# Artessay/RAGraph

Hardware: AMD Instinct MI355X
Metric: retrieved-queries/sec (RAGraph_node forward: GCN encode + cosine/top-k retrieval + 3-hop propagate + decode) (higher is better)
Workload: dtype f32 (exact results; candidates pre-filtered on bf16 / int8 MFMA with proven bounds)

## Files before the change

### include/ragraph_hip.h

```cpp
#ifndef RAGRAPH_HIP_H
#define RAGRAPH_HIP_H

#include <stddef.h>
#include <stdint.h>

#ifdef __cplusplus
extern "C" {
#endif

#define RAGRAPH_ABI_VERSION 1

#define RAGRAPH_OK 0
#define RAGRAPH_EINVAL (-1)
#define RAGRAPH_EUNSUPPORTED (-2)
#define RAGRAPH_EWORKSPACE (-3)
#define RAGRAPH_EDEVICE (-4)

#define RAGRAPH_ACT_NONE 0
#define RAGRAPH_ACT_RELU 1
#define RAGRAPH_ACT_PRELU 2
#define RAGRAPH_ACT_LEAKY 3
#define RAGRAPH_ACT_ELU 4

int ragraph_abi_version(void);
const char* ragraph_last_error(void);
int ragraph_device_check(void);

int ragraph_normalize_rows_f32(const float* X, int64_t n, int D, float* out, void* stream);

#define RAGRAPH_TOPK_MAX 64
size_t ragraph_topk_cosine_workspace_bytes(int64_t B, int64_t N, int D, int k);
int ragraph_topk_cosine_f32(const float* Q, int64_t B, const float* Kn, int64_t N, int D, int k, int64_t idx_base,
                            float* out_scores, int64_t* out_idx, void* ws, size_t ws_bytes, void* stream);

int ragraph_pack_keys_f32(const float* Kn, int64_t N, int D, float* Kp, void* stream);
int ragraph_topk_cosine_bank_f32(const float* Q, int64_t B, const float* Kn, const float* Kp, int64_t N, int D, int k,
                                 int64_t idx_base, float* out_scores, int64_t* out_idx, void* ws, size_t ws_bytes,
                                 void* stream);

size_t ragraph_topk_cosine_mix_workspace_bytes(int64_t B, int64_t N, int D, int A, int k);
int ragraph_topk_cosine_mix_f32(const float* Q, int64_t B, const float* Kn, int64_t N, int D, const float* Pq,
                                const float* Pn, int A, float w_struct, float w_sem, int k, int64_t idx_base,
                                float* out_scores, int64_t* out_idx, void* ws, size_t ws_bytes, void* stream);

int64_t ragraph_keys_bf16_rows(int64_t N);
int ragraph_keys_to_bf16(const float* Kn, int64_t N, int D, uint16_t* Kb, void* stream);
int ragraph_topk_cosine_filtered_cap(int k);
size_t ragraph_topk_cosine_filtered_workspace_bytes(int64_t B, int64_t N, int D, int k);
size_t ragraph_topk_cosine_filtered_stats_offset(size_t ws_bytes);
int ragraph_topk_cosine_filtered_plan(int64_t B, int64_t N, int D, int k, int64_t plan[7]);
int ragraph_topk_cosine_filtered_i8_levels(int64_t B, int64_t N, int D, int k);
int ragraph_topk_cosine_filtered_max_i8_levels(int n);
float ragraph_topk_cosine_filtered_set_prior(float theta_prior);
int ragraph_topk_cosine_filtered_f32(const float* Q, int64_t B, const float* Kn, const float* Kp, const uint16_t* Kb,
                                     int64_t N, int D, int k, int64_t idx_base, float* out_scores, int64_t* out_idx,
                                     int* overflow, int64_t* overflow_idx, void* ws, size_t ws_bytes, void* stream);

typedef void (*ragraph_exchange_fn)(void* ctx, int phase);
int ragraph_verify_merged_prior_f32(const float* merged_scores, int64_t R, int k, float prior, int speculative,
                                    const int* stats_words, const int* overflow, float* out5, void* stream);
int ragraph_topk_cosine_filtered_sharded_speculates(int64_t B, int64_t plan_N, int D, int k, int n_shards);
size_t ragraph_topk_cosine_filtered_sharded_workspace_bytes(int64_t B, int64_t plan_N, int D, int k, int n_shards);
int ragraph_topk_cosine_filtered_sharded_f32(const float* Q, int64_t B, const float* Kn, const float* Kp, const uint16_t* Kb,
                                             int64_t N, int D, int k, int64_t idx_base, float* out_scores, int64_t* out_idx,
                                             int* overflow, int64_t* overflow_idx, void* ws, size_t ws_bytes, void* stream,
                                             int64_t plan_N, float* theta, ragraph_exchange_fn exchange, void* ctx,
                                             int n_shards);

int ragraph_topk_cosine_small_ok(int64_t B, int64_t N, int D, int k);
size_t ragraph_topk_cosine_small_state_bytes(void);
int64_t ragraph_topk_cosine_small_prefix_keys(int64_t B, int64_t N, int D, int* i8);
size_t ragraph_topk_cosine_small_workspace_bytes(int64_t B, int D, int k);
int ragraph_topk_cosine_small_f32(const float* Q, int64_t B, const float* Kn, const uint16_t* Kb, int64_t N, int D, int k,
                                  int64_t idx_base, float* out_scores, int64_t* out_idx, int* overflow, int* state, void* ws,
                                  size_t ws_bytes, void* stream);

int ragraph_topk_cosine_fused_ok(int64_t B, int64_t N, int D, int k);
size_t ragraph_topk_cosine_fused_workspace_bytes(int64_t B, int64_t N, int D, int k);
int ragraph_topk_cosine_fused_f32(const float* Q, int64_t B, const float* Kn, const uint16_t* Kb, int64_t N, int D, int k,
                                  int64_t idx_base, float* out_scores, int64_t* out_idx, int* tickets, void* ws,
                                  size_t ws_bytes, void* stream);

int ragraph_theta_sharpen_f32(const float* gathered, int G, int64_t B, int m, int k, float* theta, void* stream);

typedef struct ragraph_filter_profile ragraph_filter_profile;
ragraph_filter_profile* ragraph_filter_profile_create(void);
void ragraph_filter_profile_destroy(ragraph_filter_profile* p);
ragraph_filter_profile* ragraph_filter_profile_attach(ragraph_filter_profile* p);
float ragraph_filter_profile_last_ms(ragraph_filter_profile* p);
int ragraph_filter_profile_levels(ragraph_filter_profile* p, float* ms_host, int* i8_host, int64_t* keys_host);

int ragraph_topk_merge_f32(const float* scores, const int64_t* idx, int G, int64_t B, int k, float* out_scores,
                           int64_t* out_idx, void* stream);

size_t ragraph_dedup_rows_workspace_bytes(int64_t N);
int ragraph_dedup_rows_f32(const float* Kn, int64_t N, int D, int64_t* stats, int64_t* uniq_row, int32_t* group_ptr,
                           int32_t* members, void* ws, size_t ws_bytes, void* stream);
int ragraph_topk_expand_groups_f32(const float* scores_u, const int64_t* idx_u, int ku, int64_t idx_base_u,
                                   const int32_t* group_ptr, const int32_t* members, int64_t U, int64_t B, int k,
                                   int64_t idx_base, float* out_scores, int64_t* out_idx, void* stream);

int ragraph_gather_rows_f32(const float* V, int64_t N, int D, const int64_t* idx, int64_t M, int64_t idx_base,
                            float* out, void* stream);

int ragraph_gather_reduce_f32(const float* V, int D, const float* L, int C, int64_t N, const int64_t* idx, int64_t B,
                              int k, int64_t idx_base, float v_scale, float* sum_V, float* mean_L, void* stream);

int ragraph_gather_reduce_mix_f32(const float* V, int D, const float* L, int C, int64_t N, const int64_t* idx, int64_t B,
                                  int k, int64_t idx_base, float v_scale, const float* A, float wa, float wb, float* out,
                                  float* mean_L, void* stream);

int ragraph_linear_f32(const float* X, int64_t M, int K, const float* W, int64_t N, const float* bias, int act,
                       float alpha, float* Y, void* stream);

size_t ragraph_linear_tn_workspace_bytes(int64_t n, int M, int N);
int ragraph_linear_tn_f32(const float* A, const float* B, int64_t n, int M, int N, float* C, void* ws, size_t ws_bytes,
                          void* stream);

int ragraph_spmm_csr_f32(const int64_t* rowptr, const int32_t* col, const float* val, int64_t n, const float* X, int D,
                         const float* bias, int act, float alpha, float beta, const float* Y_in, float* Y,
                         void* stream);
size_t ragraph_sparse_workspace_bytes(int64_t nnz, int D);
int ragraph_spmm_csr_ws_f32(const int64_t* rowptr, const int32_t* col, const float* val, int64_t n, const float* X, int D,
                            const float* bias, int act, float alpha, float beta, const float* Y_in, float* Y, int64_t nnz,
                            void* ws, size_t ws_bytes, void* stream);
size_t ragraph_spmm_csr_rows_workspace_bytes(int64_t nnz, int64_t R, int D);
int ragraph_spmm_csr_rows_f32(const int64_t* rowptr, const int32_t* col, const float* val, int64_t n, const float* X, int D,
                              const int64_t* rows, int64_t R, float* Y, int64_t nnz, void* ws, size_t ws_bytes,
                              void* stream);
size_t ragraph_csr_rows_offsets_workspace_bytes(int64_t R);
int ragraph_csr_rows_offsets_i64(const int64_t* rowptr, int64_t n, const int64_t* rows, int64_t R, int64_t* off, void* ws,
                                 size_t ws_bytes, void* stream);
int ragraph_csr_rows_edges_f32(const int64_t* rowptr, const int32_t* col, const float* val, const int64_t* rows, int64_t R,
                               const int64_t* off, int64_t E, int64_t* out_col, int64_t* out_r, float* out_val,
                               void* stream);
int ragraph_spmm_csr_prelu_dev_f32(const int64_t* rowptr, const int32_t* col, const float* val, int64_t n, const float* X,
                                   int D, const float* bias, const float* alpha, float* Y, float* Z, int64_t nnz, void* ws,
                                   size_t ws_bytes, void* stream);
int ragraph_act_grad_prelu_dev_f32(const float* z, const float* gy, int64_t n, const float* alpha, float* gz,
                                   float* alpha_terms, void* stream);

size_t ragraph_radix_sort_workspace_bytes(int64_t n, int val_bytes);
int ragraph_radix_sort_u64(const uint64_t* keys_in, uint64_t* keys_out, const void* vals_in, void* vals_out, int val_bytes,
                           int64_t n, int bits, void* ws, size_t ws_bytes, void* stream);
size_t ragraph_scan_workspace_bytes(int64_t n);
int ragraph_scan_sum_i32(const int* in, int* out, int64_t n, int inclusive, void* ws, size_t ws_bytes, void* stream);

size_t ragraph_coo_to_csr_workspace_bytes(int64_t E, int64_t n);
int ragraph_coo_to_csr_i64(const int64_t* row, const int64_t* col, int64_t E, int64_t n, int sort_cols, int64_t* rowptr,
                           int64_t* perm, int32_t* out_col, void* ws, size_t ws_bytes, void* stream);
int ragraph_csr_row_ids_i64(const int64_t* rowptr, int64_t n, int64_t nnz, int64_t* rows, void* stream);

size_t ragraph_mask_positions_workspace_bytes(int64_t E);
int ragraph_mask_positions_i64(const unsigned char* mask, int64_t E, int64_t* pos, int64_t* count, void* ws, size_t ws_bytes,
                               void* stream);

int ragraph_spmm_csr_panels_f32(const int64_t* rowptr, const int32_t* col, const float* val, int64_t n, const float* X,
                                int64_t x_rows, int x_panels, int D, int act, float alpha, float* Y, int y_panels, void* stream);

int ragraph_spmm_linear_f32(const int64_t* rowptr, const int32_t* col, const float* val, int64_t M, const float* X, int K,
                            const float* W, int64_t N, const float* bias, int act, float alpha, float* Y, void* stream);

int ragraph_spmm_csr_tiled_f32(const int* wp, const int* col3, const float* val3, const unsigned short* row3, int RG, int C,
                               int64_t n, const float* X, int64_t x_rows, int x_panels, int D, int act, float alpha, float* Y,
                               int y_panels, void* stream);

int ragraph_csr_row_normalize_f32(const int64_t* rowptr, const float* val, int64_t n, float* val_out, void* stream);

int ragraph_segment_softmax_f32(const int64_t* rowptr, const float* x, int64_t n, float* out, void* stream);
int ragraph_segment_softmax_ws_f32(const int64_t* rowptr, const float* x, int64_t n, int64_t nnz, float* out, void* ws,
                                   size_t ws_bytes, void* stream);

int ragraph_axpby_f32(const float* a, float wa, const float* b, float wb, int64_t n, float* out, void* stream);

int ragraph_fuse_decode_f32(const float* query, const float* rag, int64_t n, int D, float wq, float wr, const float* W1,
                            const float* b1, int H, float slope, const float* W2, const float* b2, int C,
                            const float* rag_label, float lambda, float* out, void* stream);

int ragraph_softmax_mix_f32(const float* logits, const float* rag_label, int64_t B, int C, float lambda, int log_mode,
                            float* out, void* stream);

int ragraph_segment_reduce_f32(const float* X, int D, const int64_t* seg_ptr, int64_t G, const float* w, int mean_mode,
                               float* out, void* stream);

int ragraph_proto_cosine_f32(const float* emb, int64_t G, int D, const float* proto, int C, int mode, float* out,
                             void* stream);

int ragraph_sigmoid_gate_f32(const float* x, const float* z, int64_t n, float* out, void* stream);

int ragraph_time_rescale_f32(const int64_t* t, int64_t n, float t_min, float t_max, float* out, void* stream);

int ragraph_topk_rows_f32(const float* S, int64_t B, int64_t N, int64_t ld, int k, float* out_scores,
                          int64_t* out_idx, void* stream);

int ragraph_topk_select_rows_f32(const float* S, int64_t B, int64_t N, int64_t ld, int64_t k, float* out_kth,
                                 int64_t* out_idx, void* stream);
size_t ragraph_topk_select_rows_workspace_bytes(int64_t B, int64_t N);
int ragraph_topk_select_rows_ws_f32(const float* S, int64_t B, int64_t N, int64_t ld, int64_t k, float* out_kth,
                                    int64_t* out_idx, void* ws, size_t ws_bytes, void* stream);

#define RAGRAPH_TOPK_ORDERED_MAX 4096
size_t ragraph_topk_rows_large_workspace_bytes(int64_t B, int64_t N, int64_t k);
int ragraph_topk_rows_large_f32(const float* S, int64_t B, int64_t N, int64_t ld, int64_t k, float* out_scores,
                                int64_t* out_idx, void* ws, size_t ws_bytes, void* stream);

int ragraph_scatter_fill_f32(float* S, int64_t B, int64_t N, int64_t ld, const int64_t* rowptr, const int64_t* col,
// ... 104 lines not shown
```

### ragraph_amd/_native.py

```python
from __future__ import annotations

import ctypes
import os
import subprocess

import torch

_HERE = os.path.dirname(os.path.abspath(__file__))
CSRC = os.path.join(_HERE, "csrc")
SO_PATH = os.environ.get("RAGRAPH_HIP_SO", os.path.join(CSRC, "libragraph_hip.so"))

OK, EINVAL, EUNSUPPORTED, EWORKSPACE, EDEVICE = 0, -1, -2, -3, -4
ACT_NONE, ACT_RELU, ACT_PRELU, ACT_LEAKY, ACT_ELU = 0, 1, 2, 3, 4
TOPK_MAX = 64
TOPK_ORDERED_MAX = 4096
POSITION_CODES_LDS_MAX = 40000
POSITION_CODES_LONG_ROW = 512

_vp, _i64, _i32, _f32, _sz = ctypes.c_void_p, ctypes.c_int64, ctypes.c_int, ctypes.c_float, ctypes.c_size_t

SIGNATURES = {
    "ragraph_abi_version": (_i32, []),
    "ragraph_last_error": (ctypes.c_char_p, []),
    "ragraph_device_check": (_i32, []),
    "ragraph_normalize_rows_f32": (_i32, [_vp, _i64, _i32, _vp, _vp]),
    "ragraph_topk_cosine_workspace_bytes": (_sz, [_i64, _i64, _i32, _i32]),
    "ragraph_topk_cosine_f32": (_i32, [_vp, _i64, _vp, _i64, _i32, _i32, _i64, _vp, _vp, _vp, _sz, _vp]),
    "ragraph_pack_keys_f32": (_i32, [_vp, _i64, _i32, _vp, _vp]),
    "ragraph_keys_bf16_rows": (_i64, [_i64]),
    "ragraph_keys_to_bf16": (_i32, [_vp, _i64, _i32, _vp, _vp]),
    "ragraph_filter_profile_create": (_vp, []),
    "ragraph_filter_profile_destroy": (None, [_vp]),
    "ragraph_filter_profile_attach": (_vp, [_vp]),
    "ragraph_filter_profile_last_ms": (ctypes.c_float, [_vp]),
    "ragraph_topk_cosine_filtered_set_prior": (ctypes.c_float, [_f32]),
    "ragraph_filter_profile_levels": (_i32, [_vp, _vp, _vp, _vp]),
    "ragraph_topk_cosine_filtered_cap": (_i32, [_i32]),
    "ragraph_topk_cosine_filtered_workspace_bytes": (_sz, [_i64, _i64, _i32, _i32]),
    "ragraph_topk_cosine_filtered_stats_offset": (_sz, [_sz]),
    "ragraph_topk_cosine_filtered_sharded_workspace_bytes": (_sz, [_i64, _i64, _i32, _i32, _i32]),
    "ragraph_topk_cosine_filtered_plan": (_i32, [_i64, _i64, _i32, _i32, _vp]),
    "ragraph_topk_cosine_filtered_i8_levels": (_i32, [_i64, _i64, _i32, _i32]),
    "ragraph_topk_cosine_filtered_sharded_speculates": (_i32, [_i64, _i64, _i32, _i32, _i32]),
    "ragraph_verify_merged_prior_f32": (_i32, [_vp, _i64, _i32, _f32, _i32, _vp, _vp, _vp, _vp]),
    "ragraph_topk_cosine_filtered_max_i8_levels": (_i32, [_i32]),
    "ragraph_topk_cosine_filtered_f32": (_i32, [_vp, _i64, _vp, _vp, _vp, _i64, _i32, _i32, _i64, _vp, _vp, _vp, _vp, _vp,
                                                _sz, _vp]),
    "ragraph_topk_cosine_filtered_sharded_f32": (_i32, [_vp, _i64, _vp, _vp, _vp, _i64, _i32, _i32, _i64, _vp, _vp, _vp, _vp,
                                                        _vp, _sz, _vp, _i64, _vp, _vp, _vp, _i32]),
    "ragraph_topk_cosine_small_ok": (_i32, [_i64, _i64, _i32, _i32]),
    "ragraph_topk_cosine_small_state_bytes": (_sz, []),
    "ragraph_topk_cosine_small_prefix_keys": (_i64, [_i64, _i64, _i32, _vp]),
    "ragraph_topk_cosine_small_workspace_bytes": (_sz, [_i64, _i32, _i32]),
    "ragraph_topk_cosine_small_f32": (_i32, [_vp, _i64, _vp, _vp, _i64, _i32, _i32, _i64, _vp, _vp, _vp, _vp, _vp, _sz, _vp]),
    "ragraph_topk_cosine_fused_ok": (_i32, [_i64, _i64, _i32, _i32]),
    "ragraph_topk_cosine_fused_workspace_bytes": (_sz, [_i64, _i64, _i32, _i32]),
    "ragraph_topk_cosine_fused_f32": (_i32, [_vp, _i64, _vp, _vp, _i64, _i32, _i32, _i64, _vp, _vp, _vp, _vp, _sz, _vp]),
    "ragraph_theta_sharpen_f32": (_i32, [_vp, _i32, _i64, _i32, _i32, _vp, _vp]),
    "ragraph_topk_cosine_bank_f32": (_i32, [_vp, _i64, _vp, _vp, _i64, _i32, _i32, _i64, _vp, _vp, _vp, _sz, _vp]),
    "ragraph_topk_cosine_mix_workspace_bytes": (_sz, [_i64, _i64, _i32, _i32, _i32]),
    "ragraph_topk_cosine_mix_f32": (_i32, [_vp, _i64, _vp, _i64, _i32, _vp, _vp, _i32, _f32, _f32, _i32, _i64, _vp, _vp, _vp,
                                          _sz, _vp]),
    "ragraph_topk_merge_f32": (_i32, [_vp, _vp, _i32, _i64, _i32, _vp, _vp, _vp]),
    "ragraph_dedup_rows_workspace_bytes": (_sz, [_i64]),
    "ragraph_dedup_rows_f32": (_i32, [_vp, _i64, _i32, _vp, _vp, _vp, _vp, _vp, _sz, _vp]),
    "ragraph_topk_expand_groups_f32": (_i32, [_vp, _vp, _i32, _i64, _vp, _vp, _i64, _i64, _i32, _i64, _vp, _vp, _vp]),
    "ragraph_gather_rows_f32": (_i32, [_vp, _i64, _i32, _vp, _i64, _i64, _vp, _vp]),
    "ragraph_gather_reduce_f32": (_i32, [_vp, _i32, _vp, _i32, _i64, _vp, _i64, _i32, _i64, _f32, _vp, _vp, _vp]),
    "ragraph_gather_reduce_mix_f32": (_i32, [_vp, _i32, _vp, _i32, _i64, _vp, _i64, _i32, _i64, _f32, _vp, _f32, _f32, _vp, _vp, _vp]),
    "ragraph_linear_f32": (_i32, [_vp, _i64, _i32, _vp, _i64, _vp, _i32, _f32, _vp, _vp]),
    "ragraph_linear_tn_workspace_bytes": (_sz, [_i64, _i32, _i32]),
    "ragraph_linear_tn_f32": (_i32, [_vp, _vp, _i64, _i32, _i32, _vp, _vp, _sz, _vp]),
    "ragraph_spmm_csr_f32": (_i32, [_vp, _vp, _vp, _i64, _vp, _i32, _vp, _i32, _f32, _f32, _vp, _vp, _vp]),
    "ragraph_radix_sort_workspace_bytes": (_sz, [_i64, _i32]),
    "ragraph_radix_sort_u64": (_i32, [_vp, _vp, _vp, _vp, _i32, _i64, _i32, _vp, _sz, _vp]),
    "ragraph_scan_workspace_bytes": (_sz, [_i64]),
    "ragraph_scan_sum_i32": (_i32, [_vp, _vp, _i64, _i32, _vp, _sz, _vp]),
    "ragraph_coo_to_csr_workspace_bytes": (_sz, [_i64, _i64]),
    "ragraph_coo_to_csr_i64": (_i32, [_vp, _vp, _i64, _i64, _i32, _vp, _vp, _vp, _vp, _sz, _vp]),
    "ragraph_csr_row_ids_i64": (_i32, [_vp, _i64, _i64, _vp, _vp]),
    "ragraph_mask_positions_workspace_bytes": (_sz, [_i64]),
    "ragraph_mask_positions_i64": (_i32, [_vp, _i64, _vp, _vp, _vp, _sz, _vp]),
    "ragraph_spmm_csr_panels_f32": (_i32, [_vp, _vp, _vp, _i64, _vp, _i64, _i32, _i32, _i32, _f32, _vp, _i32, _vp]),
    "ragraph_spmm_linear_f32": (_i32, [_vp, _vp, _vp, _i64, _vp, _i32, _vp, _i64, _vp, _i32, _f32, _vp, _vp]),
    "ragraph_spmm_csr_tiled_f32": (_i32, [_vp, _vp, _vp, _vp, _i32, _i32, _i64, _vp, _i64, _i32, _i32, _i32, _f32, _vp, _i32, _vp]),
    "ragraph_csr_row_normalize_f32": (_i32, [_vp, _vp, _i64, _vp, _vp]),
    "ragraph_segment_softmax_f32": (_i32, [_vp, _vp, _i64, _vp, _vp]),
    "ragraph_segment_softmax_ws_f32": (_i32, [_vp, _vp, _i64, _i64, _vp, _vp, _sz, _vp]),
    "ragraph_sparse_workspace_bytes": (_sz, [_i64, _i32]),
    "ragraph_spmm_csr_ws_f32": (_i32, [_vp, _vp, _vp, _i64, _vp, _i32, _vp, _i32, _f32, _f32, _vp, _vp, _i64, _vp, _sz,
                                       _vp]),
    "ragraph_spmm_csr_rows_workspace_bytes": (_sz, [_i64, _i64, _i32]),
    "ragraph_spmm_csr_rows_f32": (_i32, [_vp, _vp, _vp, _i64, _vp, _i32, _vp, _i64, _vp, _i64, _vp, _sz, _vp]),
    "ragraph_csr_rows_offsets_workspace_bytes": (_sz, [_i64]),
    "ragraph_csr_rows_offsets_i64": (_i32, [_vp, _i64, _vp, _i64, _vp, _vp, _sz, _vp]),
    "ragraph_csr_rows_edges_f32": (_i32, [_vp, _vp, _vp, _vp, _i64, _vp, _i64, _vp, _vp, _vp, _vp]),
    "ragraph_axpby_f32": (_i32, [_vp, _f32, _vp, _f32, _i64, _vp, _vp]),
    "ragraph_softmax_mix_f32": (_i32, [_vp, _vp, _i64, _i32, _f32, _i32, _vp, _vp]),
    "ragraph_fuse_decode_f32": (_i32, [_vp, _vp, _i64, _i32, _f32, _f32, _vp, _vp, _i32, _f32, _vp, _vp, _i32, _vp, _f32,
                                       _vp, _vp]),
    "ragraph_segment_reduce_f32": (_i32, [_vp, _i32, _vp, _i64, _vp, _i32, _vp, _vp]),
    "ragraph_proto_cosine_f32": (_i32, [_vp, _i64, _i32, _vp, _i32, _i32, _vp, _vp]),
    "ragraph_sigmoid_gate_f32": (_i32, [_vp, _vp, _i64, _vp, _vp]),
    "ragraph_time_rescale_f32": (_i32, [_vp, _i64, _f32, _f32, _vp, _vp]),
    "ragraph_topk_rows_f32": (_i32, [_vp, _i64, _i64, _i64, _i32, _vp, _vp, _vp]),
    "ragraph_topk_select_rows_f32": (_i32, [_vp, _i64, _i64, _i64, _i64, _vp, _vp, _vp]),
    "ragraph_topk_select_rows_workspace_bytes": (_sz, [_i64, _i64]),
    "ragraph_topk_select_rows_ws_f32": (_i32, [_vp, _i64, _i64, _i64, _i64, _vp, _vp, _vp, _sz, _vp]),
    "ragraph_topk_rows_large_workspace_bytes": (_sz, [_i64, _i64, _i64]),
    "ragraph_topk_rows_large_f32": (_i32, [_vp, _i64, _i64, _i64, _i64, _vp, _vp, _vp, _sz, _vp]),
    "ragraph_scatter_fill_f32": (_i32, [_vp, _i64, _i64, _i64, _vp, _vp, _f32, _vp]),
    "ragraph_floyd_warshall_f32": (_i32, [_vp, _i32, _vp, _vp]),
    "ragraph_position_code_f32": (_i32, [_vp, _i32, _vp, _i32, _f32, _vp, _vp]),
    "ragraph_position_codes_csr_f32": (_i32, [_vp, _vp, _vp, _i64, _vp, _i32, _f32, _vp, _vp, _vp]),
    "ragraph_position_codes_csr_global_workspace_bytes": (_sz, [_i64, _i32]),
    "ragraph_position_codes_csr_global_f32": (_i32, [_vp, _vp, _vp, _i64, _vp, _i32, _f32, _vp, _vp, _i32, _i32, _vp, _vp, _sz,
                                                     _vp]),
    "ragraph_act_grad_f32": (_i32, [_vp, _vp, _i64, _i32, _f32, _vp, _vp, _vp]),
    "ragraph_spmm_csr_prelu_dev_f32": (_i32, [_vp, _vp, _vp, _i64, _vp, _i32, _vp, _vp, _vp, _vp, _i64, _vp, _sz, _vp]),
    "ragraph_act_grad_prelu_dev_f32": (_i32, [_vp, _vp, _i64, _vp, _vp, _vp, _vp]),
    "ragraph_sigmoid_gate_grad_f32": (_i32, [_vp, _vp, _vp, _i64, _vp, _vp, _vp]),
    "ragraph_softmax_grad_f32": (_i32, [_vp, _vp, _i64, _i32, _f32, _vp, _vp]),
    "ragraph_mul_cols_f32": (_i32, [_vp, _vp, _i64, _i32, _vp, _vp]),
    "ragraph_mul_cols_act_f32": (_i32, [_vp, _vp, _i64, _i32, _i32, _f32, _vp, _vp]),
    "ragraph_mul_f32": (_i32, [_vp, _vp, _i64, _vp, _vp]),
    "ragraph_proto_cosine_grad_f32": (_i32, [_vp, _i64, _i32, _vp, _i32, _i32, _vp, _vp, _vp, _vp]),
    "ragraph_proto_cosine_grad_proto_workspace_bytes": (_sz, [_i64, _i32, _i32]),
    "ragraph_proto_cosine_grad_proto_f32": (_i32, [_vp, _i64, _i32, _vp, _i32, _i32, _vp, _vp, _vp, _vp, _sz, _vp]),
    "ragraph_axpby_dev_f32": (_i32, [_vp, _vp, _vp, _i32, _i32, _i64, _vp, _vp]),
    "ragraph_ingest_workspace_bytes": (_sz, [_i64, _i64]),
    "ragraph_csr_sym_normalized_f32": (_i32, [_vp, _vp, _i64, _i64, _vp, _vp, _vp, _vp, _vp, _sz, _vp]),
    "ragraph_binorm_edges_f32": (_i32, [_vp, _vp, _vp, _i64, _i64, _i64, _vp, _vp, _vp, _vp, _vp, _sz, _vp]),
    "ragraph_pagerank_workspace_bytes": (_sz, [_i64, _i64]),
    "ragraph_pagerank_f32": (_i32, [_vp, _vp, _vp, _vp, _vp, _vp, _i64, _i64, _f32, _f32, _i32, _vp, _vp, _vp, _sz, _vp]),
    "ragraph_sample_prob_f32": (_i32, [_vp, _vp, _vp, _i64, _f32, _f32, _vp, _vp]),
    "ragraph_csr_row_sums_f32": (_i32, [_vp, _vp, _i64, _vp, _vp]),
    "ragraph_position_codes_batch_f32": (_i32, [_vp, _i64, _i32, _vp, _i32, _f32, _vp, _vp, _vp]),
    "ragraph_topk_dot_masked_workspace_bytes": (_sz, [_i64, _i64, _i32, _i32, _i64]),
    "ragraph_topk_dot_masked_f32": (_i32, [_vp, _i64, _vp, _i64, _vp, _i64, _i32, _i32, _vp, _vp, _i64, _f32, _vp, _vp, _vp,
                                          _sz, _vp]),
    "ragraph_rank_metrics_workspace_bytes": (_sz, [_i64, _i32, _i64]),
    "ragraph_rank_metrics_f64": (_i32, [_vp, _i64, _i32, _vp, _vp, _vp, _i32, _i64, _vp, _vp, _sz, _vp]),
    "ragraph_lp_workspace_bytes": (_sz, []),
    "ragraph_lp_sample_i64": (_i32, [_vp, _vp, _i64, _i64, _i32, _vp, _vp, _vp, _sz, _vp]),
    "ragraph_lp_compare_loss_fwd_f32": (_i32, [_vp, _i64, _i32, _vp, _i32, _f32, _vp, _vp, _vp, _vp, _vp, _vp, _vp, _sz, _vp]),
    "ragraph_lp_combine_f32": (_i32, [_vp, _vp, _vp, _vp, _vp, _f32, _i64, _i32, _vp, _vp]),
    "ragraph_edge_hist_check_i64": (_i32, [_vp, _vp, _i64, _i64, _i64, _vp, _sz, _vp]),
    "ragraph_edge_neg_sample_i64": (_i32, [_vp, _vp, _i64, _i64, _vp, _i64, _i32, _i32, _vp, _vp, _vp, _sz, _vp]),
    "ragraph_noise_rows_i64": (_i32, [_vp, _vp, _i64, _i64, _i32, _i64, _vp, _i64, _vp]),
    "ragraph_gather_reduce_noisy_f32": (_i32, [_vp, _i32, _vp, _i32, _i64, _vp, _i64, _i32, _i64, _f32, _vp, _vp, _i64, _i32, _i64,
                                               _vp, _f32, _f32, _vp, _vp, _vp]),
    "ragraph_add_normal_noise_f32": (_i32, [_vp, _i64, _i64, _i32, _f32, _vp, _vp, _i64, _vp, _vp]),
    "ragraph_edge_rewrite_workspace_bytes": (_sz, [_i64]),
    "ragraph_edge_rewrite_csr": (_i32, [_vp, _vp, _vp, _i64, _i64, _vp, _vp, _vp, _vp, _i64, _vp, _sz, _vp]),
    "ragraph_multinomial_segments_workspace_bytes": (_sz, [_i64]),
    "ragraph_multinomial_segments_i64": (_i32, [_vp, _vp, _i64, _vp, _i64, _i32, _vp, _vp, _sz, _vp]),
    "ragraph_csr_induced_blocks_f32": (_i32, [_vp, _vp, _vp, _i64, _i64, _vp, _i64, _i32, _vp, _vp]),
    "ragraph_blocks_to_csr_workspace_bytes": (_sz, [_i64, _i32]),
    "ragraph_blocks_to_csr_f32": (_i32, [_vp, _i64, _i32, _vp, _vp, _vp, _vp, _vp, _sz, _vp]),
    "ragraph_augment_features_f32": (_i32, [_vp, _i64, _i32, _vp, _f32, _f32, _vp, _vp, _vp, _i64, _vp, _vp]),
}


class RagraphNativeError(RuntimeError):
    """The HIP library is missing, has no usable device, or a call returned an error code."""


_lib = None


def build(verbose: bool = False) -> str:
    cmd = ["make", "-C", CSRC, "-j4"]
    if not verbose:
        cmd.append("-s")
    subprocess.check_call(cmd)
    return SO_PATH


def lib() -> ctypes.CDLL:
    global _lib
    if _lib is None:
        if not os.path.exists(SO_PATH):
            raise RagraphNativeError(
                f"{SO_PATH} not found: build it with `python -c 'import __graft_entry__ as g; g.build()'` "
                "(ragraph_amd has no CPU fallback)")
        cdll = ctypes.CDLL(SO_PATH)
        for name, (res, args) in SIGNATURES.items():
            fn = getattr(cdll, name)
# ... 22 lines not shown
```

### ragraph_amd/csrc/filter_common.h

```cpp
#pragma once
#include "common.h"
#include <climits>

namespace ragraph {

typedef __bf16 bf16x8 __attribute__((ext_vector_type(8)));

constexpr float FILTER_EPS_SLACK = 0.000244140625f;

constexpr int FILTER_STAGE_BYTES = 32 * 1024;
constexpr int FILTER_PAD_KEYS = 256;

__host__ __device__ constexpr int64_t filter_block_offset(int64_t subtile, int D, int t, int h) {
  return (subtile * (D / 16) + 2 * t + h) * 1024;
}

__host__ __device__ constexpr int64_t filter_i8_block_offset(int64_t subtile, int D, int t, int h) {
  return (subtile * (D / 32) + 2 * t + h) * 1024;
}
__host__ __device__ constexpr int filter_i8_granule_keys(int D) { return FILTER_STAGE_BYTES / D; }
__host__ __device__ constexpr int64_t filter_pad_keys(int64_t n) { return (n + FILTER_PAD_KEYS - 1) / FILTER_PAD_KEYS * FILTER_PAD_KEYS; }
struct FilterI8View {
  const signed char* K8;
  const unsigned* tail8;
  const float* gmax;
  const unsigned* cls;
  int64_t granules;
};
inline int64_t filter_i8_granules(int64_t N, int D) {
  const int gk = filter_i8_granule_keys(D);
  return (filter_pad_keys(N) + gk - 1) / gk;
}
inline size_t filter_i8_table_bytes(int64_t N, int D) {
  const int64_t g = filter_i8_granules(N, D);
  return (size_t)((g * 4 + 15) / 16 * 16) + (size_t)((g + 31) / 32 * 4) + 16;
}
inline FilterI8View filter_i8_view(const uint16_t* Kb, int64_t N, int D) {
  const int64_t npad = filter_pad_keys(N);
  FilterI8View v;
  v.K8 = reinterpret_cast<const signed char*>(Kb + (npad + 1) * D);
  v.tail8 = reinterpret_cast<const unsigned*>(v.K8 + npad * D);
  v.granules = filter_i8_granules(N, D);
  v.gmax = reinterpret_cast<const float*>(reinterpret_cast<const char*>(v.tail8) + (size_t)D * 2);
  v.cls = reinterpret_cast<const unsigned*>(reinterpret_cast<const char*>(v.gmax) + (v.granules * 4 + 15) / 16 * 16);
  return v;
}

__device__ __forceinline__ int quantize_i8(float x, float inv_scale) {
  return (int)fminf(fmaxf(__builtin_rintf(__fmul_rn(x, inv_scale)), -127.f), 127.f);
}

int filter_thread_i8_cap();
float filter_thread_prior();
int launch_overflow_fixup(int D, const float* Qn, const float* Kn, int64_t N, int k, int64_t idx_base, const int* count,
                          const int* list, float* out_s, int64_t* out_i, int* done, float* part_s, int64_t* part_i, int64_t B,
                          void* stream);

__device__ __forceinline__ int f2ord(float f) {
  const int b = __float_as_int(f);
  return b >= 0 ? b : b ^ 0x7FFFFFFF;
}
__device__ __forceinline__ float ord2f(int o) { return __int_as_float(o >= 0 ? o : o ^ 0x7FFFFFFF); }

struct FilterThr {
  const float* theta;
  const float* prev_scores;
  const int* gmax;
  const float* eq;
  const unsigned* max_kerr2;
  int k, ngroups;
  int ablate;
  const float* eq8;
  const float* qscale;
  const unsigned* tail8;
  const unsigned* cls8;
  const unsigned char* flag;
};

__device__ __forceinline__ float filter_eps(const FilterThr& t, int64_t q) {
  const float ek = sqrtf(__uint_as_float(*t.max_kerr2));
  const float e = t.eq[q];
  return fmaf(fmaf(e, ek, e + ek), 1.0009765625f, FILTER_EPS_SLACK);
}

__device__ __forceinline__ float filter_theta(const FilterThr& t, int64_t q) {
  if (t.theta) return t.theta[q];
  if (t.gmax) {
    int m = t.gmax[q * t.ngroups];
    for (int g = 1; g < t.ngroups; ++g) m = min(m, t.gmax[q * t.ngroups + g]);
    return __fsub_rn(ord2f(m), filter_eps(t, q));
  }
  return t.prev_scores[q * t.k + t.k - 1];
}

__device__ __forceinline__ float filter_threshold(const FilterThr& t, int64_t q) {
  const unsigned char fl = t.flag ? t.flag[q] : 0;
  const float thr = __fsub_rn(filter_theta(t, q), filter_eps(t, q));
  return (t.ablate == 1 || fl) ? __builtin_huge_valf() : thr;
}

__device__ __forceinline__ int filter_threshold_i8_of(float theta, float e, float ek, float sc) {
  const float eps = fmaf(fmaf(e, ek, e + ek), 1.0009765625f, FILTER_EPS_SLACK);
  if (!(sc > 0.f)) return INT_MIN;
  const float x = __fsub_rn(theta, eps) / sc;
  if (!(x > -8.4e6f)) return INT_MIN;
  if (x > 8.4e6f) return INT_MAX;
  return (int)floorf(x) - 2;
}
__device__ __forceinline__ int filter_threshold_i8_at(const FilterThr& t, int64_t q, float theta, int heavy) {
  return filter_threshold_i8_of(theta, t.eq8[q], sqrtf(__uint_as_float(t.tail8[heavy ? 3 : 0])),
                                t.qscale[q] * __uint_as_float(t.tail8[heavy ? 4 : 1]));
}
__device__ __forceinline__ int filter_threshold_i8(const FilterThr& t, int64_t q, int heavy) {
  const unsigned char fl = t.flag ? t.flag[q] : 0;
  const int thr = filter_threshold_i8_at(t, q, filter_theta(t, q), heavy);
  return (t.ablate == 1 || fl) ? INT_MAX : thr;
}
__device__ __forceinline__ int filter_i8_class(const unsigned* cls, int64_t granule) {
  return (int)((cls[granule >> 5] >> (granule & 31)) & 1u);
}

constexpr int FILTER_COUNT_STRIDE = 32;
constexpr int FILTER_TICKET_SLOT = 16;
__host__ __device__ constexpr int filter_count_stride(int64_t B) { return B < 2048 ? FILTER_COUNT_STRIDE : 1; }

struct DirectArgs {
  const uint16_t* Qb;
  const uint16_t* Kb;
  int64_t B, key0, key1;
  FilterThr thr;
  int* count;
  int* cand;
  int cap;
  int nsub;
  int* gmax_out;
  int bound_groups;
  int scored;
  int i8;
};
template <int D>
int launch_filter_direct(const DirectArgs& a, hipStream_t st);

}
```

### ragraph_amd/csrc/filter_ring.h

```cpp

#ifdef RG_RING_STAMPS
__device__ unsigned long long g_ring_t[2][2][8];
__device__ unsigned long long g_ring_span[2][2];
__device__ unsigned long long g_ring_max[2][8];
#define RG_RSTAMP(i_)                                                                                     \
  if (threadIdx.x == 0 && first_seg) {                                                                    \
    const unsigned long long now_ = wall_clock64();                                                       \
    if (blockIdx.x == 0 || blockIdx.x == gridDim.x - 1) g_ring_t[BOUND][blockIdx.x != 0][i_] = now_;      \
    if ((i_) == 0) atomicMin(&g_ring_span[BOUND][0], now_);                                               \
    else atomicMax(&g_ring_max[BOUND][i_], now_ - rs_prev);                                               \
    rs_prev = now_;                                                                                       \
  }
static void ring_stamps_report(bool BOUND, bool I8) {
  (void)hipDeviceSynchronize();
  unsigned long long t[2][2][8];
  (void)hipMemcpyFromSymbol(t, HIP_SYMBOL(g_ring_t), sizeof(t));
  for (int b = 0; b < 2; ++b)
    fprintf(stderr, "[ring stamps, %s%s launch, %s workgroup, 10 ns ticks] operands %lld thresholds %lld ring primed %lld stages %lld "
            "flush %lld (entered %lld after workgroup 0)\n", BOUND ? "bound" : "filter", I8 ? " int8" : "", b ? "last" : "first",
            (long long)(t[BOUND][b][1] - t[BOUND][b][0]), (long long)(t[BOUND][b][2] - t[BOUND][b][1]),
            (long long)(t[BOUND][b][3] - t[BOUND][b][2]), (long long)(t[BOUND][b][4] - t[BOUND][b][3]),
            (long long)(t[BOUND][b][5] - t[BOUND][b][4]), (long long)(t[BOUND][b][0] - t[BOUND][0][0]));
  unsigned long long span[2][2], mx[2][8];
  (void)hipMemcpyFromSymbol(span, HIP_SYMBOL(g_ring_span), sizeof(span));
  (void)hipMemcpyFromSymbol(mx, HIP_SYMBOL(g_ring_max), sizeof(mx));
  fprintf(stderr, "[ring stamps, all workgroups] first entry to last exit %lld; longest first-segment phases: operands %lld thresholds %lld "
          "ring primed %lld stages %lld flush %lld\n", (long long)(span[BOUND][1] - span[BOUND][0]), (long long)mx[BOUND][1],
          (long long)mx[BOUND][2], (long long)mx[BOUND][3], (long long)mx[BOUND][4], (long long)mx[BOUND][5]);
  unsigned long long init_span[2][2] = {{~0ull, 0ull}, {~0ull, 0ull}}, zero[2][8] = {};
  (void)hipMemcpyToSymbol(HIP_SYMBOL(g_ring_span), init_span, sizeof(init_span));
  (void)hipMemcpyToSymbol(HIP_SYMBOL(g_ring_max), zero, sizeof(zero));
}
#else
#define RG_RSTAMP(i_)
static void ring_stamps_report(bool, bool) {}
#endif
#ifdef RG_TOPK_TIMING
__device__ unsigned long long g_filter_timing[8];
#define RG_FT(var_) const unsigned long long var_ = __builtin_amdgcn_s_memtime()
static void ring_timing_report(int prof_slot, int D) {
  (void)hipDeviceSynchronize();
  unsigned long long t[8];
  (void)hipMemcpyFromSymbol(t, HIP_SYMBOL(g_filter_timing), sizeof(t));
  const double n = (double)t[5];
  if (n > 0)
    fprintf(stderr, "[filter timing] slot %d D=%d wave-stages=%.0f ticks/stage: wait_full %.1f compute %.1f signal+vmcnt "
            "%.1f wait_free %.1f dma_issue %.1f total %.1f; flushes in the loop: %.0f, %.1f ticks each = %.1f per stage\n",
            prof_slot, D, n, t[0] / n, t[1] / n, t[2] / n, t[3] / n, t[4] / n, (t[0] + t[1] + t[2] + t[3] + t[4]) / n, (double)t[7],
            t[7] ? (double)t[6] / (double)t[7] : 0.0, t[6] / n);
  unsigned long long zero[8] = {0, 0, 0, 0, 0, 0, 0, 0};
  (void)hipMemcpyToSymbol(HIP_SYMBOL(g_filter_timing), zero, sizeof(zero));
}
#else
#define RG_FT(var_)
static void ring_timing_report(int, int) {}
#endif

#ifndef RG_RING_FOLD
#define RG_RING_FOLD 1
#endif
template <int D, int QW, bool BOUND = false, bool I8 = false, bool SCORED = false, bool PIPE = false>
__global__ void __launch_bounds__(512, 2) topk_filter_kernel(FilterParams p) {
  using C = FilterCfg<I8 ? D / 2 : D>;
  static_assert(!PIPE || (I8 && !BOUND && C::KSTEPS >= QW / 16 + 2), "PIPE: int8 filter levels, one step per query group + 2");
  static_assert(!(I8 && BOUND), "the bound pass runs on the bf16 copy");
  static_assert(I8 || !SCORED, "scored lists carry the int8 levels' integer sums");
  static_assert(QW == 32 || QW == 64 || QW == 96 || QW == 128, "two, four, six or eight query groups of 16 per wave");
  constexpr int QT = C::WAVES * QW;
  constexpr int NG = QW / 16;
  constexpr bool FOLD = RG_RING_FOLD && I8 && !PIPE && !BOUND && D == 64;
  extern __shared__ float4 fsmem4[];
  char* smem = reinterpret_cast<char*>(fsmem4);
  unsigned* full = reinterpret_cast<unsigned*>(smem + C::SLOTS * C::STAGE_BYTES);
  unsigned* freec = full + C::SLOTS;
  const unsigned lds_base = (unsigned)(size_t)(lds_void_f*)smem;

  const int tid = threadIdx.x;
  const int lane = tid & 63;
  const int wave = __builtin_amdgcn_readfirstlane(tid >> 6);
  const int j = lane & 15, g = lane >> 4;

  unsigned voff[C::DMAS];
#pragma unroll
  for (int i = 0; i < C::DMAS; ++i) voff[i] = (unsigned)(i * 1024 + lane * 16);
  auto dma_stage = [&](int64_t stage_abs, int slot) {
    const uint64_t goff = (uint64_t)stage_abs * C::STAGE_BYTES + (uint64_t)(C::DMAS * wave * 1024);
    const char* gbase = reinterpret_cast<const char*>(p.Kb) +
                        (((uint64_t)(unsigned)__builtin_amdgcn_readfirstlane((int)(goff >> 32)) << 32) |
                         (uint64_t)(unsigned)__builtin_amdgcn_readfirstlane((int)(unsigned)goff));
#pragma unroll
    for (int i = 0; i < C::DMAS; ++i) {
      const unsigned dst = lds_base + (unsigned)(slot * C::STAGE_BYTES + (C::DMAS * wave + i) * 1024);
      unsigned keep;
      asm volatile(
          "s_mov_b32 %0, m0\n\ts_mov_b32 m0, %2\n\ts_nop 0\n\tglobal_load_lds_dwordx4 %1, %3\n\ts_mov_b32 m0, %0"
          : "=&s"(keep)
          : "v"(voff[i]), "s"(dst), "s"(gbase)
          : "memory");
    }
  };
  const unsigned apos = lds_base + (unsigned)lane * 16u;

  const int x = p.xcd_map ? (int)(blockIdx.x & 7) : 0;
  const int64_t nq = p.xcd_map ? ((p.qtiles - x + 7) >> 3) : p.qtiles;
  const int64_t nq0 = p.xcd_map ? ((p.qtiles + 7) >> 3) : p.qtiles;
  SegmentWalker walker(nq, p.nstages_total, p.wgs_per_group, p.lb_min, 0, p.depth[nq != nq0],
                       p.xcd_map ? (int)(blockIdx.x >> 3) : (int)blockIdx.x);
  Segment seg;
  [[maybe_unused]] bool first_seg = true;
#ifdef RG_RING_STAMPS
  unsigned long long rs_prev = 0;
#endif
  RG_RSTAMP(0);
  while (walker.next(seg)) {
    const int64_t qtile = p.xcd_map ? x + 8 * seg.tile : seg.tile;
    const int64_t q_lo = qtile * QT + wave * QW + j;
    const int64_t st0 = seg.st0;
    const int nstages = (int)(seg.st1 - seg.st0);

    bf16x8 bq[I8 ? 1 : NG][I8 ? 1 : C::KS32];
    i32x4 bqi[I8 ? NG : 1][I8 ? C::KS32 : 1];
    constexpr int TB = C::KS32 < 4 ? C::KS32 : 4;
    if constexpr (I8) {
      if (p.Qb) {
        const int64_t qg0 = (qtile * QT + wave * QW) >> 4;
        const int64_t ngroups16 = ((p.B + 31) / 32 * 32) >> 4;
#pragma unroll
        for (int gq = 0; gq < NG; ++gq) {
          const bool have = qg0 + gq < ngroups16;
          const i32x4* src = reinterpret_cast<const i32x4*>(p.Qb) + ((qg0 + gq) * C::KS32) * 64 + lane;
#pragma unroll
          for (int t = 0; t < C::KS32; ++t) {
            i32x4 z = {0, 0, 0, 0};
            bqi[gq][t] = have ? src[t * 64] : z;
          }
        }
      } else
#pragma unroll
      for (int gq = 0; gq < NG; ++gq) {
        const int64_t qq = q_lo + 16 * gq;
        const int64_t qr = qq < p.B ? qq : p.B - 1;
        const float sq = p.thr.qscale[qr];
        const float inv_sq = sq > 0.f ? 1.f / sq : 0.f;
        const float* r0 = p.Qn + qr * D + 16 * g;
#pragma unroll
        for (int t = 0; t < C::KS32; ++t) {
          float4 u[4];
#pragma unroll
          for (int c = 0; c < 4; ++c) u[c] = *reinterpret_cast<const float4*>(r0 + 64 * t + 4 * c);
#pragma unroll
          for (int c = 0; c < 4; ++c) {
            unsigned w = 0u;
            if (sq > 0.f)
              w = ((unsigned)quantize_i8(u[c].x, inv_sq) & 0xFFu) | (((unsigned)quantize_i8(u[c].y, inv_sq) & 0xFFu) << 8) |
                  (((unsigned)quantize_i8(u[c].z, inv_sq) & 0xFFu) << 16) | (((unsigned)quantize_i8(u[c].w, inv_sq) & 0xFFu) << 24);
            bqi[gq][t][c] = (int)w;
          }
          asm volatile("" : "+v"(bqi[gq][t]));
        }
        asm volatile("" ::: "memory");
      }
    } else if (p.Qb) {
      const int64_t qg0 = (qtile * QT + wave * QW) >> 4;
      const int64_t ngroups16 = ((p.B + 31) / 32 * 32) >> 4;
#pragma unroll
      for (int gq = 0; gq < NG; ++gq) {
        const bool have = qg0 + gq < ngroups16;
        const bf16x8* src = reinterpret_cast<const bf16x8*>(p.Qb) + ((qg0 + gq) * C::KS32) * 64 + lane;
#pragma unroll
        for (int t = 0; t < C::KS32; ++t) {
          bf16x8 z;
#pragma unroll
          for (int e = 0; e < 8; ++e) z[e] = (__bf16)0.f;
          bq[gq][t] = have ? src[t * 64] : z;
        }
      }
    } else
#pragma unroll
    for (int gq = 0; gq < NG; ++gq) {
      const int64_t qq = q_lo + 16 * gq;
      const float* r0 = p.Qn + (qq < p.B ? qq : p.B - 1) * D + 8 * g;
#pragma unroll
      for (int t0 = 0; t0 < C::KS32; t0 += TB) {
#pragma unroll
        for (int t = t0; t < t0 + TB; ++t) {
          const float4 u0 = *reinterpret_cast<const float4*>(r0 + 32 * t), u1 = *reinterpret_cast<const float4*>(r0 + 32 * t + 4);
          bq[gq][t][0] = (__bf16)u0.x; bq[gq][t][1] = (__bf16)u0.y; bq[gq][t][2] = (__bf16)u0.z; bq[gq][t][3] = (__bf16)u0.w;
          bq[gq][t][4] = (__bf16)u1.x; bq[gq][t][5] = (__bf16)u1.y; bq[gq][t][6] = (__bf16)u1.z; bq[gq][t][7] = (__bf16)u1.w;
        }
#pragma unroll
        for (int t = t0; t < t0 + TB; ++t) asm volatile("" : "+v"(bq[gq][t]));
        asm volatile("" ::: "memory");
      }
    }
    RG_RSTAMP(1);
    float thr[NG];
    int thr8[NG], thr8h[NG];
#pragma unroll
    for (int gq = 0; gq < NG; ++gq) {
      thr[gq] = (!BOUND && !I8 && q_lo + 16 * gq < p.B) ? filter_threshold(p.thr, q_lo + 16 * gq) : __builtin_huge_valf();
      thr8[gq] = (I8 && q_lo + 16 * gq < p.B) ? filter_threshold_i8(p.thr, q_lo + 16 * gq, 0) : INT_MAX;
      thr8h[gq] = (I8 && q_lo + 16 * gq < p.B) ? filter_threshold_i8(p.thr, q_lo + 16 * gq, 1) : INT_MAX;
    }
    float gm[NG];
#pragma unroll
    for (int gq = 0; gq < NG; ++gq) gm[gq] = RG_NEG_INF;
    int grp = 0;
    int64_t grp_end = 0;
    auto group_of = [&](int64_t t) { return (int)(t * p.ngroups / p.nstages_total); };
    auto flush_max = [&]() {
#pragma unroll
      for (int gq = 0; gq < NG; ++gq) {
        float v = gm[gq];
        v = fmaxf(v, __shfl_xor(v, 16));
        v = fmaxf(v, __shfl_xor(v, 32));
        if (g == 0 && q_lo + 16 * gq < p.B) atomicMax(p.gmax + (q_lo + 16 * gq) * p.ngroups + grp, f2ord(v));
        gm[gq] = RG_NEG_INF;
      }
    };
    if constexpr (BOUND) {
      grp = group_of(st0);
      grp_end = ((int64_t)(grp + 1) * p.nstages_total + p.ngroups - 1) / p.ngroups;
    }
// ... 434 lines not shown
```

### ragraph_amd/csrc/filter_schedule.h

```cpp

constexpr int FILTER_MAX_LEVELS = 3;
static int64_t filter_round_up(int64_t n) { return (n + FILTER_PAD_KEYS - 1) / FILTER_PAD_KEYS * FILTER_PAD_KEYS; }

struct FilterSchedule {
  int64_t bound_keys;
  int64_t n0;
  int slab0;
  int nlev;
  int64_t ends[FILTER_MAX_LEVELS];
  int i8_levels;
};

constexpr int64_t FILTER_SLAB_MAX_B = 16384;
constexpr int64_t FILTER_QB_MAX_B = 262144;
constexpr int64_t FILTER_SLAB_MAX_SCORES = (int64_t)1 << 26;

struct FilterEnv {
  int i8;
  int scored;
  int pipe;
  int partner_lead;
  int i8_qw;
  int scored_shards;
  int spec_two_shards;
};
static int filter_env_int(const char* name, int dflt) {
  const char* e = getenv(name);
  return e ? atoi(e) : dflt;
}
static FilterEnv filter_env() {
  static const int scored_shards = filter_env_int("RAGRAPH_FILTER_SCORED_SHARDS", 2);
  static const int spec_two_shards = filter_env_int("RAGRAPH_FILTER_SPEC_SHARDS_TWO_LEVELS", 2);
  return {filter_env_int("RAGRAPH_FILTER_I8", -1), filter_env_int("RAGRAPH_FILTER_SCORED", -1), filter_env_int("RAGRAPH_FILTER_PIPE", 1),
          filter_env_int("RAGRAPH_FILTER_PARTNER_LEAD", 1), filter_env_int("RAGRAPH_FILTER_I8_QW", 0), scored_shards, spec_two_shards};
}

static bool filter_scored_lists(int64_t B, int D, int k, const FilterEnv& env) {
  if (B < 65) return false;
  if (env.scored >= 0) return env.scored != 0;
  return D == 256 && k <= 16;
}

static int rescore_slices(int64_t B, int k) {
  int S = B <= 16 ? 8 : (B <= 32 ? 4 : (B <= 64 ? 2 : 1));
  while (S > 1 && S * k > 256) S >>= 1;
  return S;
}
constexpr int FILTER_LIST_CAP = 2048;
static int filter_cap(int64_t B, int k) { return FILTER_LIST_CAP * (B <= 64 ? rescore_slices(B, k) : 1); }

constexpr int64_t FILTER_BOUND_MIN_KEYS = 8192;

static int filter_bound_parts(int k, int64_t bound_keys, int D, int64_t B = 1 << 20, int n_shards = 1) {
  if (B <= 64) return k;
  int64_t g = 4 * (int64_t)k;
  if (g > 128) g = 128;
  if (n_shards > 1) g = (g + n_shards - 1) / n_shards;
  const int64_t avail = bound_keys == INT64_MAX ? g : bound_keys / (FILTER_STAGE_BYTES / (2 * D));
  if (g > avail) g = avail;
  return (int)(g < k ? k : g);
}
static double filter_bound_eff(int k, int parts) {
  if (parts >= 4 * k || parts >= 128) return 1.2;
  if (parts >= 2 * k) return 1.5;
  return log((double)k) + 1.0;
}

static void filter_align_ends(FilterSchedule& sc, int D) {
  if (D != 64) return;
  for (int l = 0; l + 1 < sc.nlev; ++l) {
    const int64_t e = sc.ends[l] / 512 * 512;
    if (e >= 512 && (l == 0 || e > sc.ends[l - 1])) sc.ends[l] = e;
  }
  if (sc.bound_keys > sc.ends[0]) sc.bound_keys = sc.ends[0] / FILTER_PAD_KEYS * FILTER_PAD_KEYS;
}

struct FilterShape {
  int64_t B, N, plan_N;
  int D, k, n_shards;
  bool exchange;
  float prior;
  int i8_cap;
  bool exact_level0;
  FilterEnv env;
  int cus;
};

static FilterSchedule filter_schedule(const FilterShape& in) {
  const int64_t B = in.B, N = in.plan_N;
  const int D = in.D, k = in.k, n_shards = in.exchange ? in.n_shards : 1, cus = in.cus;
  const FilterEnv& env = in.env;
  FilterSchedule sc{};
  const int cap = 2048;
  const bool scored = (n_shards == 1 || n_shards <= env.scored_shards) && B >= 2048 && filter_scored_lists(B, D, k, env);
  constexpr double scored_cand = 0.6;
  const bool bound = N >= FILTER_BOUND_MIN_KEYS;
  const bool i8_ok = (D == 64 || D == 128 || D == 256) && B > 256 &&
                     (N * n_shards >= 65536 || (D == 256 && B >= 2048 && N * n_shards >= 32768));
  const bool mid_i8 = i8_ok && N * n_shards < 65536;
  static const bool i8_direct_env = [] { const char* e = getenv("RAGRAPH_FILTER_I8_DIRECT"); return !e || atoi(e) != 0; }();
  static const bool i8_direct_d64 = [] { const char* e = getenv("RAGRAPH_FILTER_I8_DIRECT_D64"); return !e || atoi(e) != 0; }();
  const bool i8_direct = (D == 128 || D == 256 || (D == 64 && i8_direct_d64)) && B <= 256 && N * n_shards >= 65536 && i8_direct_env;
  const double eff_div = filter_bound_eff(k, B <= 64 ? k : 4 * k);
  auto prefix_for = [&](int64_t n0) {
    int64_t nA = filter_round_up((int64_t)((double)n0 * eff_div));
    const int parts = filter_bound_parts(k, nA, D, B);
    if (parts < 4 * k && parts < 128) nA = filter_round_up((int64_t)((double)n0 * filter_bound_eff(k, parts)));
    return nA;
  };
  if (B > FILTER_SLAB_MAX_B || N < 4 * 4096) {
    static const int64_t n0div = [] { const char* e = getenv("RAGRAPH_FILTER_N0DIV"); return e ? (int64_t)atoll(e) : (int64_t)64; }();
    int64_t n0 = N * n_shards / n0div;
    if (n0 < 4096) n0 = 4096;
    int64_t nA = bound ? prefix_for(n0) : 0;
    if (n_shards > 1) {
      n0 /= n_shards;
      nA = filter_round_up(nA / n_shards);
      const int64_t min_keys = filter_round_up((int64_t)k * (FILTER_STAGE_BYTES / (2 * D)));
      if (nA < min_keys) nA = min_keys;
    }
    if (n0 > N) n0 = N;
    if (n0 < k) n0 = k < N ? k : N;
    if (bound) {
      if (nA > N / 4) nA = N / 4 / FILTER_PAD_KEYS * FILTER_PAD_KEYS;
      sc.bound_keys = nA;
    }
    sc.n0 = n0;
    sc.slab0 = 0;
    sc.nlev = 0;
    int64_t prev = n0;
    int64_t fracs[2] = {32, 4};
    int nfr = 2;
    if (const char* fe = getenv("RAGRAPH_FILTER_FRACS")) {
      long long a = 0, b = 0;
      nfr = sscanf(fe, "%lld,%lld", &a, &b);
      if (nfr < 1 || a < 2) nfr = 0;
      fracs[0] = a;
      fracs[1] = b;
      if (nfr == 2 && b < 2) nfr = 1;
    }
    for (int fi = 0; fi < nfr; ++fi) {
      const int64_t frac = fracs[fi];
      int64_t e = filter_round_up(N / frac);
      if (e < 4 * prev) e = filter_round_up(4 * prev);
      if (e * 2 >= N) break;
      sc.ends[sc.nlev++] = e;
      prev = e;
    }
    sc.ends[sc.nlev++] = N;
    if (sc.bound_keys > sc.ends[0]) sc.bound_keys = sc.ends[0] / FILTER_PAD_KEYS * FILTER_PAD_KEYS;
    if (sc.bound_keys / (FILTER_STAGE_BYTES / (2 * D)) < k) sc.bound_keys = 0;
    sc.i8_levels = i8_ok && B >= 1024 ? (scored ? 3 : 2) : 0;
    filter_align_ends(sc, D);
    return sc;
  }
  double best = 1e30;
  int64_t best_n0 = 4096, best_nA = 0;
  int best_L = FILTER_MAX_LEVELS, best_i8 = 0;
  static const int64_t force_n0 = [] { const char* e = getenv("RAGRAPH_FILTER_FORCE_N0"); return e ? (int64_t)atoll(e) : (int64_t)0; }();
  static const int force_L = [] { const char* e = getenv("RAGRAPH_FILTER_FORCE_L"); return e ? atoi(e) : 0; }();
  const int stage_keys = FILTER_STAGE_BYTES / (2 * D);
  const double tiles = (double)((B + 511) / 512);
  for (int64_t n0 = 4096; n0 * 4 <= N; n0 *= 2) {
    if (force_n0 > 0 && n0 != force_n0) continue;
    double first;
    int64_t nA = 0;
    if (bound) {
      nA = prefix_for(n0);
      if (nA * 4 > N) break;
      if (B <= 256)
        first = 6.0 + (double)nA * 2.0 * D / 5.0e6 * (1.0 + (double)B / 320.0);
      else
        first = 35.0 + (double)nA * 2.0 * D / 3.0e6 + tiles * (double)(nA / stage_keys) * 3.1 / 256.0;
    } else {
      if (B * n0 > FILTER_SLAB_MAX_SCORES) break;
      first = 30.0 + (double)B * (double)n0 * (2.0 * D / 1.0e8 + 4.0 / 3.0e6);
    }
    for (int L = 1; L <= FILTER_MAX_LEVELS; ++L) {
      if (force_L > 0 && L != force_L) continue;
      const double r = pow((double)N / (double)n0, 1.0 / L);
      if (1.3 * k * r > cap / 2 && !(force_n0 > 0 && force_L > 0)) continue;
      if (B <= 256) {
        for (int q8 = i8_direct ? 1 : 0; q8 <= (i8_direct ? 1 : 0); ++q8) {
          const double cands = 1.3 * k * r * (q8 ? 3.0 : 1.0);
          if (cands > cap * (q8 ? rescore_slices(B, k) : 1) / 2 && !(force_n0 > 0 && force_L > 0)) continue;
          const double cost = first + L * (25.0 + (double)B * cands * (q8 ? 2.0e-3 : 0.5e-3)) + (L - 1) * (q8 ? 30.0 : 15.0)
                              - (q8 ? 32.0 + 0.08 * (double)B : 0.0);
          if (cost < best) {
            best = cost;
            best_n0 = n0;
            best_nA = nA;
            best_L = L;
            best_i8 = q8 ? L : 0;
          }
        }
        continue;
      }
      const double per_cand = 0.18e-3 + 0.22e-3 * (B <= 1024 ? 1.0 : 1024.0 / (double)B);
      static const double i8_candf = [] { const char* e = getenv("RAGRAPH_FILTER_I8_CANDF"); return e ? atof(e) : 2.0; }();
      for (int i8 = 0; i8 <= (i8_ok && !mid_i8 ? (L < 2 || scored ? L : 2) : 0); ++i8) {
        double cost = first, e_prev = 0.0, e = (double)n0;
        bool fits = true;
        for (int l = 0; l < L; ++l) {
          e = l + 1 == L ? (double)N : e * r;
          const bool q8 = l >= L - i8;
          const double cands = 1.3 * k * r * (q8 ? i8_candf : 1.0);
          if (cands > cap / 2 && !(force_n0 > 0 && force_L > 0)) fits = false;
          cost += 60.0 + (e - e_prev) * (double)B * 2.0 * D / (q8 ? 2.4e9 : 1.25e9) +
                  (double)B * cands * per_cand * (q8 && scored ? scored_cand : 1.0);
          e_prev = e;
        }
        if (fits && cost < best) {
          best = cost;
          best_n0 = n0;
          best_nA = nA;
          best_L = L;
          best_i8 = i8;
        }
      }
    }
  }
  sc.bound_keys = bound ? (best_nA ? best_nA : prefix_for(4096)) : 0;
  if (bound && B > 128 && B <= 256 && n_shards == 1) {
    const int64_t round_keys = (int64_t)8 * cus * (16384 / (2 * D));
    int64_t r = (sc.bound_keys + round_keys / 2) / round_keys;
    if (r < 1) r = 1;
    if (r * round_keys * 4 <= N && r * round_keys >= (int64_t)k * 4 * (FILTER_STAGE_BYTES / (2 * D))) sc.bound_keys = r * round_keys;
  }
  sc.n0 = best_n0;
  sc.i8_levels = mid_i8 ? best_L : best_i8;
  sc.slab0 = 1;
  sc.nlev = 0;
  const double r = pow((double)N / (double)best_n0, 1.0 / best_L);
  double e = (double)best_n0;
  for (int l = 0; l + 1 < best_L; ++l) {
    e *= r;
    const int64_t ei = filter_round_up((int64_t)e);
    if (ei * 2 >= N) break;
    sc.ends[sc.nlev++] = ei;
  }
  sc.ends[sc.nlev++] = N;
  if (sc.bound_keys > sc.ends[0]) sc.bound_keys = sc.ends[0] / FILTER_PAD_KEYS * FILTER_PAD_KEYS;
  if (sc.bound_keys / stage_keys < k) sc.bound_keys = 0;
  if (sc.bound_keys == 0 && B * sc.n0 > FILTER_SLAB_MAX_SCORES) sc.slab0 = 0;
  filter_align_ends(sc, D);
  return sc;
}

static int filter_i8_levels(const FilterSchedule& sc, int64_t B, int i8_cap, const FilterEnv& env) {
  if (B <= 256) {
    if (i8_cap == 0 || sc.i8_levels == 0) return 0;
    return sc.nlev;
  }
  if (env.i8 >= 0) return env.i8 < sc.nlev ? env.i8 : sc.nlev;
  if (i8_cap == 0) return 0;
  int n = sc.i8_levels < sc.nlev ? sc.i8_levels : sc.nlev;
  if (i8_cap > 0 && n > i8_cap) n = i8_cap;
  return n;
}

enum FilterLevel0 {
  FILTER_L0_NONE,
  FILTER_L0_BOUND,
  FILTER_L0_SLAB,
  FILTER_L0_TILE
};
struct FilterLevel {
  int64_t key0, key1;
  bool int8, scored;
};
struct FilterCall {
  int cap;
  bool scored_slots;
  bool exact_participant;
  bool spec;
  FilterLevel0 level0;
  size_t level0_bytes;
  int64_t n0, bound_keys;
  int parts;
  int nlev, i8_levels;
  FilterLevel level[FILTER_MAX_LEVELS];
  bool bf16_image;
  int first_phase;
};

static void filter_drop_first_level(FilterSchedule& sc) {
  for (int l = 0; l + 1 < sc.nlev; ++l) sc.ends[l] = sc.ends[l + 1];
  --sc.nlev;
  if (sc.i8_levels > sc.nlev) sc.i8_levels = sc.nlev;
}

static FilterCall filter_call_plan(const FilterShape& in, FilterSchedule sc) {
  const int64_t B = in.B, N = in.N, plan_N = in.plan_N;
  const int D = in.D, k = in.k, ns = in.exchange ? in.n_shards : 1;
  const int stage_keys = FILTER_STAGE_BYTES / (2 * D);
  FilterCall c{};
  c.cap = filter_cap(B, k);
  c.scored_slots = filter_scored_lists(B, D, k, in.env);
  const bool prior_ok = in.prior == in.prior && in.prior > -2.f && in.prior < 2.f;
  const int spec_two = in.env.spec_two_shards;
  auto drop_first_level_under_prior = [&] {
    if ((sc.nlev == 2 && B <= 4096) || (in.exchange && sc.nlev == 3 && spec_two > 0 && in.n_shards >= spec_two))
      filter_drop_first_level(sc);
  };
  if (in.exchange) {
    c.spec = prior_ok && sc.bound_keys > 0;
    if (c.spec) drop_first_level_under_prior();
    if (plan_N - N > 1024) {
      int64_t prev = 0;
      for (int l = 0; l + 1 < sc.nlev; ++l) {
        int64_t e = (int64_t)((double)sc.ends[l] * (double)N / (double)plan_N) / 512 * 512;
        if (e < prev + 512 || e + 512 > N) c.exact_participant = true;
        sc.ends[l] = e;
        prev = e;
      }
      sc.bound_keys = (int64_t)((double)sc.bound_keys * (double)N / (double)plan_N) / FILTER_PAD_KEYS * FILTER_PAD_KEYS;
      if (sc.nlev > 1 && sc.bound_keys > sc.ends[0]) sc.bound_keys = sc.ends[0];
      if (sc.bound_keys / stage_keys < (int64_t)filter_bound_parts(k, sc.bound_keys, D, B, in.n_shards)) sc.bound_keys = 0;
      if (sc.n0 > N) sc.n0 = N;
      if (N < 16384 || N * 8 < plan_N) c.exact_participant = true;
    }
  }
  c.first_phase = c.spec ? 1 : 0;
  c.nlev = sc.nlev;
  if (c.exact_participant) return c;
  sc.ends[sc.nlev - 1] = N;
  if (sc.bound_keys > N / 2 || in.exact_level0) {
    sc.bound_keys = 0;
    if (sc.n0 > N) sc.n0 = N;
  }
  if (in.exchange && in.n_shards > 1 && sc.bound_keys > 0 && B <= FILTER_SLAB_MAX_B && plan_N >= 4 * 4096) {
    const int64_t min_keys = filter_round_up((int64_t)k * stage_keys);
    const int64_t bk = filter_round_up(sc.bound_keys / in.n_shards);
    sc.bound_keys = bk < min_keys ? (min_keys < sc.bound_keys ? min_keys : sc.bound_keys) : bk;
  }
  if (!in.exchange) {
    c.spec = prior_ok && sc.bound_keys > 0 && N == plan_N;
    if (c.spec) drop_first_level_under_prior();
  }
  const bool bound = sc.bound_keys > 0 && !c.spec;
  c.level0 = c.spec ? FILTER_L0_NONE : (bound ? FILTER_L0_BOUND : (sc.slab0 ? FILTER_L0_SLAB : FILTER_L0_TILE));
  c.level0_bytes = sc.bound_keys > 0 ? 0
                   : sc.slab0        ? align_up((size_t)(B < FILTER_SLAB_MAX_B ? B : FILTER_SLAB_MAX_B) * (size_t)sc.n0 * sizeof(float), 256)
                                     : ragraph_topk_cosine_workspace_bytes(B, sc.n0, D, k);
  c.n0 = sc.n0;
  c.bound_keys = sc.bound_keys;
  c.parts = bound ? filter_bound_parts(k, sc.bound_keys, D, B, ns) : k;
  c.nlev = sc.nlev;
  c.i8_levels = filter_i8_levels(sc, B, in.i8_cap, in.env);
  c.bf16_image = B <= FILTER_QB_MAX_B && (B <= 256 || bound || c.nlev > c.i8_levels);
  for (int l = 0; l < c.nlev; ++l) {
    FilterLevel& lv = c.level[l];
    lv.key0 = l ? sc.ends[l - 1] : 0;
    lv.key1 = sc.ends[l];
    lv.int8 = l >= c.nlev - c.i8_levels;
    lv.scored = lv.int8 && (!in.exchange || in.n_shards <= in.env.scored_shards) && c.scored_slots;
  }
  return c;
}
```

### ragraph_amd/csrc/filter_verify_fixup.h

```cpp

__global__ void __launch_bounds__(256) filter_verify_prior_kernel(const float* __restrict__ out_s, int64_t B, int k, float prior,
                                                                  int speculative, const unsigned char* __restrict__ flag,
                                                                  int* __restrict__ overflow, int* __restrict__ overflow_list,
                                                                  int* __restrict__ stats) {
  const int64_t q = (int64_t)blockIdx.x * 256 + threadIdx.x;
  int lo = INT_MAX, hi = INT_MIN, failed = 0;
  if (q < B && flag[q] != 2) {
    const float kth = out_s[q * k + k - 1];
    if (speculative && flag[q] == 0 && !(kth >= prior)) {
      overflow_list[atomicAdd(overflow, 1)] = (int)q;
      failed = 1;
    } else if (kth > RG_NEG_INF) {
      lo = hi = f2ord(kth);
    }
  }
#pragma unroll
  for (int off = 32; off >= 1; off >>= 1) {
    lo = min(lo, __shfl_xor(lo, off));
    hi = max(hi, __shfl_xor(hi, off));
    failed += __shfl_xor(failed, off);
  }
  __shared__ int red[3][4];
  const int w = threadIdx.x >> 6;
  if ((threadIdx.x & 63) == 0) {
    red[0][w] = lo;
    red[1][w] = hi;
    red[2][w] = failed;
  }
  __syncthreads();
  if (threadIdx.x == 0 && stats) {
    lo = min(min(red[0][0], red[0][1]), min(red[0][2], red[0][3]));
    hi = max(max(red[1][0], red[1][1]), max(red[1][2], red[1][3]));
    failed = red[2][0] + red[2][1] + red[2][2] + red[2][3];
    if (lo != INT_MAX) atomicMin(stats + 18, lo);
    if (hi != INT_MIN) atomicMax(stats + 19, hi);
    if (failed) atomicAdd(stats + 17, failed);
  }
}

__global__ void __launch_bounds__(256) verify_merged_prior_kernel(const float* __restrict__ s, int64_t R, int k, float prior,
                                                                  int speculative, const int* __restrict__ words,
                                                                  const int* __restrict__ overflow, float* __restrict__ out) {
  __shared__ float red[3][4];
  float miss = 0.f, neg_lo = RG_NEG_INF, hi = RG_NEG_INF;
  for (int64_t q = threadIdx.x; q < R; q += 256) {
    const float top = s[q * k], kth = s[q * k + k - 1];
    const bool zero = top == 0.f && kth == 0.f;
    const bool ok = zero || !speculative || kth >= prior;
    if (!ok) miss += 1.f;
    else if (!zero && kth > RG_NEG_INF) {
      neg_lo = fmaxf(neg_lo, -kth);
      hi = fmaxf(hi, kth);
    }
  }
#pragma unroll
  for (int off = 32; off >= 1; off >>= 1) {
    miss += __shfl_xor(miss, off);
    neg_lo = fmaxf(neg_lo, __shfl_xor(neg_lo, off));
    hi = fmaxf(hi, __shfl_xor(hi, off));
  }
  const int w = threadIdx.x >> 6;
  if ((threadIdx.x & 63) == 0) {
    red[0][w] = miss;
    red[1][w] = neg_lo;
    red[2][w] = hi;
  }
  __syncthreads();
  if (threadIdx.x == 0) {
    out[0] = red[0][0] + red[0][1] + red[0][2] + red[0][3];
    out[1] = fmaxf(fmaxf(red[1][0], red[1][1]), fmaxf(red[1][2], red[1][3]));
    out[2] = fmaxf(fmaxf(red[2][0], red[2][1]), fmaxf(red[2][2], red[2][3]));
    float cand = -1.f;
    if (words && words[0] == FILTER_STATS_MAGIC) {
      cand = 0.f;
      for (int l = 0; l < 3; ++l)
        if (words[5 + l] > 0) cand += (float)words[2 + l] / (float)words[5 + l];
    }
    out[3] = cand;
    out[4] = overflow ? (float)*overflow : 0.f;
  }
}

template <int D>
__global__ void __launch_bounds__(256) topk_overflow_fixup_kernel(const float* __restrict__ Qn, const float* __restrict__ Kn,
                                                                  int64_t N, int k, int64_t idx_base,
                                                                  const int* __restrict__ overflow,
                                                                  const int* __restrict__ overflow_list,
                                                                  int64_t* __restrict__ overflow_idx_out,
                                                                  float* __restrict__ out_s, int64_t* __restrict__ out_i,
                                                                  int* __restrict__ done, float* __restrict__ part_s,
                                                                  int64_t* __restrict__ part_i, int64_t B,
                                                                  const unsigned char* __restrict__ flag,
                                                                  int* __restrict__ stats) {
  __shared__ float4 qs[D / 4];
  __shared__ __attribute__((aligned(16))) float tile[4][64 * RESCORE_LD];
  __shared__ float ps[4][32];
  __shared__ int64_t pi[4][32];
  __shared__ int ticket_s;
  const int n_over = *overflow;
  if (stats && blockIdx.x == 0 && threadIdx.x == 0) stats[20] = n_over;
  if (stats && stats[16] == 0) {
    int lo = INT_MAX, hi = INT_MIN;
    for (int64_t q = (int64_t)blockIdx.x * 256 + threadIdx.x; q < B; q += (int64_t)gridDim.x * 256) {
      const float kth = flag[q] != 0 ? RG_NEG_INF : out_s[q * k + k - 1];
      if (kth > RG_NEG_INF) {
        lo = min(lo, f2ord(kth));
        hi = max(hi, f2ord(kth));
      }
    }
#pragma unroll
    for (int off = 32; off >= 1; off >>= 1) {
      lo = min(lo, __shfl_xor(lo, off));
      hi = max(hi, __shfl_xor(hi, off));
    }
    if ((threadIdx.x & 63) == 0) {
      if (lo != INT_MAX) atomicMin(stats + 18, lo);
      if (hi != INT_MIN) atomicMax(stats + 19, hi);
    }
  }
  if (n_over <= 0) return;
  int SL = 1;
  if (n_over <= FILTER_FIX_MAX_Q)
    while (SL < FILTER_FIX_SLICES && 2 * SL * n_over <= (int)gridDim.x) SL *= 2;
  const int64_t chunk = ((N + SL - 1) / SL + 63) / 64 * 64;
  const int lane = threadIdx.x & 63, w = threadIdx.x >> 6;
  for (int64_t item = blockIdx.x; item < (int64_t)n_over * SL; item += gridDim.x) {
    const int o = (int)(item / SL), sl = (int)(item % SL);
    const int64_t b = overflow_list[o];
    if (overflow_idx_out && threadIdx.x == 0 && sl == 0) overflow_idx_out[o] = b;
    __syncthreads();
    if (threadIdx.x < D / 4) qs[threadIdx.x] = reinterpret_cast<const float4*>(Qn + b * D)[threadIdx.x];
    __syncthreads();
    if (SL == 1) {
      exact_scan_query<D>(qs, Kn, N, k, idx_base, tile, ps, pi, out_s + b * k, out_i + b * k);
      continue;
    }
    const int64_t lo = sl * chunk, hi = lo + chunk < N ? lo + chunk : N;
    float* my_s = part_s + ((int64_t)o * SL + sl) * 32;
    int64_t* my_i = part_i + ((int64_t)o * SL + sl) * 32;
    if (lo < hi) {
      exact_scan_query<D>(qs, Kn + lo * D, hi - lo, k, lo, tile, ps, pi, my_s, my_i);
    } else if (threadIdx.x < k) {
      my_s[threadIdx.x] = RG_NEG_INF;
      my_i[threadIdx.x] = INT64_MAX;
    }
    __threadfence();
    __syncthreads();
    if (threadIdx.x == 0) ticket_s = atomicAdd(done + o, 1);
    __syncthreads();
    if (ticket_s != SL - 1) continue;
    __threadfence();
    if (w == 0) {
      float s8[8];
      int id8[8];
#pragma unroll
      for (int u = 0; u < 8; ++u) {
        const int e = lane + 64 * u;
        s8[u] = RG_NEG_INF;
        id8[u] = INT_MAX;
        if (e < SL * k) {
          const int64_t at = ((int64_t)o * SL + e / k) * 32 + e % k;
          const int64_t pv = __builtin_nontemporal_load(part_i + at);
          if (pv < INT_MAX) {
            s8[u] = __builtin_nontemporal_load(part_s + at);
            id8[u] = (int)pv;
          }
        }
      }
      wave_select<8>(s8, id8, k, lane, idx_base, out_s + b * k, out_i + b * k);
    }
  }
}
```

### ragraph_amd/csrc/topk_filter.hip

```cpp
#include "filter_common.h"
#include "rescore_common.h"
#include <new>
#include "segment_plan.h"
#include <cmath>
#include <type_traits>

namespace ragraph {

typedef __attribute__((address_space(3))) void lds_void_f;
typedef int i32x4 __attribute__((ext_vector_type(4)));

template <int D_>
struct FilterCfg {
  static constexpr int D = D_;
  static constexpr int WAVES = 8, THREADS = 512;
  static constexpr int ROW_BYTES = D * 2;
  static constexpr int CR = D / 8;
  static constexpr int KSTEPS = D / 16;
  static constexpr int KS32 = D / 32;
  static constexpr int STAGE_BYTES = FILTER_STAGE_BYTES;
  static constexpr int STAGE_KEYS = STAGE_BYTES / ROW_BYTES;
  static constexpr int SUBS = STAGE_KEYS / 32;
  static constexpr int NSTEP = SUBS * KSTEPS;
  static constexpr int SLOTS = 4;
  static constexpr int DMAS = STAGE_BYTES / 1024 / WAVES;
  static constexpr int RPI = 1024 / ROW_BYTES;
  static constexpr int CAND_BUF = 480;
  static constexpr size_t LDS_BYTES = (size_t)SLOTS * STAGE_BYTES + 64 + (size_t)WAVES * CAND_BUF * 8;
};
static_assert(FilterCfg<256>::NSTEP == 32 && FilterCfg<128>::NSTEP == 32 && FilterCfg<64>::NSTEP == 32, "32 steps per stage");

struct FilterParams {
  const float* Qn;
  const uint16_t* Kb;
  FilterThr thr;
  int* count;
  int cstride;
  const uint16_t* Qb;
  int* cand;
  int64_t B, N;
  int cap;
  int64_t stage_base;
  int64_t qtiles, nstages_total;
  int xcd_map, wgs_per_group, lb_min, depth[2];
  int partner_lead;
  int* gmax;
  int ngroups;
};

__device__ __forceinline__ void fring_wait(unsigned* ctr, unsigned target) {
  while (__hip_atomic_load(ctr, __ATOMIC_ACQUIRE, __HIP_MEMORY_SCOPE_WORKGROUP) < target) __builtin_amdgcn_s_sleep(1);
}
#ifndef RG_RING_RELAXED
#define RG_RING_RELAXED 1
#endif
__device__ __forceinline__ void fring_signal(unsigned* ctr, int lane) {
  asm volatile("" ::: "memory");
  if (lane == 0) __hip_atomic_fetch_add(ctr, 1u, RG_RING_RELAXED ? __ATOMIC_RELAXED : __ATOMIC_RELEASE, __HIP_MEMORY_SCOPE_WORKGROUP);
}

#include "filter_copies.h"

#include "filter_prepare.h"

#include "filter_ring.h"

#include "filter_rescore.h"

#include "filter_verify_fixup.h"

static int filter_device_cus() { return device_cus_multiple_of_8(); }

}

using namespace ragraph;

struct ragraph_filter_profile {
  hipEvent_t ev[2 * 4];
  int have, bound;
  int i8[4];
  int64_t keys[4];
};
static thread_local ragraph_filter_profile* t_prof = nullptr;
extern "C" ragraph_filter_profile* ragraph_filter_profile_create(void) {
  ragraph_filter_profile* p = new (std::nothrow) ragraph_filter_profile();
  if (!p) {
    set_error("profile: out of memory");
    return nullptr;
  }
  for (int i = 0; i < 2 * 4; ++i)
    if (hipEventCreate(&p->ev[i]) != hipSuccess) {
      for (int j = 0; j < i; ++j) (void)hipEventDestroy(p->ev[j]);
      delete p;
      set_error("profile: cannot create events");
      return nullptr;
    }
  return p;
}
extern "C" void ragraph_filter_profile_destroy(ragraph_filter_profile* p) {
  if (!p) return;
  if (t_prof == p) t_prof = nullptr;
  for (int i = 0; i < 2 * 4; ++i) (void)hipEventDestroy(p->ev[i]);
  delete p;
}
extern "C" ragraph_filter_profile* ragraph_filter_profile_attach(ragraph_filter_profile* p) {
  ragraph_filter_profile* old = t_prof;
  t_prof = p;
  if (p) p->have = p->bound = 0;
  return old;
}
extern "C" float ragraph_filter_profile_last_ms(ragraph_filter_profile* p) {
  if (!p || !p->have) return -1.f;
  float total = 0.f;
  if (p->bound) {
    float ms = 0.f;
    if (hipEventSynchronize(p->ev[7]) != hipSuccess || hipEventElapsedTime(&ms, p->ev[6], p->ev[7]) != hipSuccess) return -1.f;
    total += ms;
  }
  for (int l = 0; l < p->have; ++l) {
    float ms = 0.f;
    if (hipEventSynchronize(p->ev[2 * l + 1]) != hipSuccess || hipEventElapsedTime(&ms, p->ev[2 * l], p->ev[2 * l + 1]) != hipSuccess)
      return -1.f;
    total += ms;
  }
  return total;
}

extern "C" int ragraph_filter_profile_levels(ragraph_filter_profile* p, float* ms_host, int* i8_host, int64_t* keys_host) {
  RG_REQUIRE(p && ms_host && i8_host && keys_host, RAGRAPH_EINVAL, "profile: null pointer");
  for (int s_ = 0; s_ < 4; ++s_) {
    ms_host[s_] = -1.f;
    i8_host[s_] = p->i8[s_];
    keys_host[s_] = p->keys[s_];
    const bool have = s_ == 3 ? p->bound != 0 : s_ < p->have;
    if (!have) continue;
    float ms = 0.f;
    if (hipEventSynchronize(p->ev[2 * s_ + 1]) == hipSuccess && hipEventElapsedTime(&ms, p->ev[2 * s_], p->ev[2 * s_ + 1]) == hipSuccess)
      ms_host[s_] = ms;
  }
  return RAGRAPH_OK;
}

#include "filter_schedule.h"

static thread_local int t_max_i8_levels = -1;
static thread_local float t_prior = __builtin_nanf("");
extern "C" float ragraph_topk_cosine_filtered_set_prior(float theta_prior) {
  const float old = t_prior;
  t_prior = theta_prior;
  return old;
}
extern "C" int ragraph_topk_cosine_filtered_max_i8_levels(int n) {
  const int old = t_max_i8_levels;
  t_max_i8_levels = n < 0 ? -1 : n;
  return old;
}
int ragraph::filter_thread_i8_cap() { return t_max_i8_levels; }
float ragraph::filter_thread_prior() { return t_prior; }
int ragraph::launch_overflow_fixup(int D, const float* Qn, const float* Kn, int64_t N, int k, int64_t idx_base, const int* count,
                                   const int* list, float* out_s, int64_t* out_i, int* done, float* part_s, int64_t* part_i,
                                   int64_t B, void* stream) {
  hipStream_t st = as_stream(stream);
#define RG_FIX(D_)                                                                                                          \
  hipLaunchKernelGGL(topk_overflow_fixup_kernel<D_>, dim3(256), dim3(256), 0, st, Qn, Kn, N, k, idx_base, count, list,       \
                     (int64_t*)nullptr, out_s, out_i, done, part_s, part_i, B, (const unsigned char*)nullptr, (int*)nullptr)
  if (D == 256) RG_FIX(256);
  else if (D == 128) RG_FIX(128);
  else RG_FIX(64);
#undef RG_FIX
  RG_CHECK_LAUNCH("overflow fixup");
  return RAGRAPH_OK;
}

static bool filter_dim_ok(int D) { return D == 64 || D == 128 || D == 256; }

extern "C" int ragraph_keys_to_bf16(const float* Kn, int64_t N, int D, uint16_t* Kb, void* stream) {
  RG_REQUIRE(Kn && Kb, RAGRAPH_EINVAL, "keys_to_bf16: null pointer");
  RG_REQUIRE(N >= 1, RAGRAPH_EINVAL, "keys_to_bf16: N=%lld must be >= 1", (long long)N);
  RG_REQUIRE(filter_dim_ok(D), RAGRAPH_EUNSUPPORTED, "keys_to_bf16: D=%d not in {64,128,256}", D);
  RG_REQUIRE(aligned16(Kn) && aligned16(Kb), RAGRAPH_EINVAL, "keys_to_bf16: pointers must be 16-B aligned");
  const int64_t npad = filter_round_up(N);
  unsigned* tail = reinterpret_cast<unsigned*>(Kb + npad * D);
  hipStream_t st = as_stream(stream);
  if (hipMemsetAsync(tail, 0, (size_t)D * sizeof(uint16_t), st) != hipSuccess) {
    set_error("keys_to_bf16: memset failed");
    return RAGRAPH_EDEVICE;
  }
  const dim3 grid((unsigned)cdiv(npad * (D / 8), 256));
  if (D == 256) hipLaunchKernelGGL(keys_to_bf16_kernel<256>, grid, dim3(256), 0, st, Kn, N, npad, Kb, tail);
  else if (D == 128) hipLaunchKernelGGL(keys_to_bf16_kernel<128>, grid, dim3(256), 0, st, Kn, N, npad, Kb, tail);
  else hipLaunchKernelGGL(keys_to_bf16_kernel<64>, grid, dim3(256), 0, st, Kn, N, npad, Kb, tail);
  RG_CHECK_LAUNCH("keys_to_bf16");
  const FilterI8View v8 = filter_i8_view(Kb, N, D);
  signed char* Kb8 = const_cast<signed char*>(v8.K8);
  unsigned* tail8 = const_cast<unsigned*>(v8.tail8);
  if (hipMemsetAsync(tail8, 0, (size_t)D * sizeof(uint16_t) + filter_i8_table_bytes(N, D), st) != hipSuccess) {
    set_error("keys_to_bf16: memset failed");
    return RAGRAPH_EDEVICE;
  }
  float* gmax = const_cast<float*>(v8.gmax);
  unsigned* cls = const_cast<unsigned*>(v8.cls);
  const dim3 gridg((unsigned)v8.granules);
  if (D == 256) hipLaunchKernelGGL(i8_granule_absmax_kernel<256>, gridg, dim3(256), 0, st, Kn, N, gmax, tail8);
  else if (D == 128) hipLaunchKernelGGL(i8_granule_absmax_kernel<128>, gridg, dim3(256), 0, st, Kn, N, gmax, tail8);
  else hipLaunchKernelGGL(i8_granule_absmax_kernel<64>, gridg, dim3(256), 0, st, Kn, N, gmax, tail8);
  static const float lambda = [] {
    const char* e = getenv("RAGRAPH_I8_ONE_SCALE");
    if (e && e[0] == '1') return 0.f;
    const char* l = getenv("RAGRAPH_I8_CUT_LAMBDA");
    return l ? (float)atof(l) : 60.f;
  }();
  hipLaunchKernelGGL(i8_cut_kernel, dim3(1), dim3(1024), 0, st, gmax, v8.granules, D, lambda, tail8);
  const dim3 grid8((unsigned)cdiv(npad * (D / 16), 256));
  if (D == 256) hipLaunchKernelGGL(keys_to_i8_kernel<256>, grid8, dim3(256), 0, st, Kn, N, npad, Kb8, tail8, gmax, cls);
  else if (D == 128) hipLaunchKernelGGL(keys_to_i8_kernel<128>, grid8, dim3(256), 0, st, Kn, N, npad, Kb8, tail8, gmax, cls);
  else hipLaunchKernelGGL(keys_to_i8_kernel<64>, grid8, dim3(256), 0, st, Kn, N, npad, Kb8, tail8, gmax, cls);
  RG_CHECK_LAUNCH("keys_to_bf16(int8 copy)");
  return RAGRAPH_OK;
}

constexpr int64_t FILTER_COPY_SLACK_ROWS = 256;
extern "C" int64_t ragraph_keys_bf16_rows(int64_t N) {
  if (N < 1) return 0;
  const int64_t npad = filter_round_up(N);
  return npad + 1 + npad / 2 + 1 + (npad / 4096 + 8) + FILTER_COPY_SLACK_ROWS;
}

extern "C" int ragraph_topk_cosine_filtered_cap(int k) { return FILTER_LIST_CAP; }

constexpr size_t FILTER_STATS_BYTES = 256;
extern "C" size_t ragraph_topk_cosine_filtered_stats_offset(size_t ws_bytes) {
  return ws_bytes < FILTER_STATS_INTS * sizeof(int) ? 0 : (ws_bytes - FILTER_STATS_INTS * sizeof(int)) & ~(size_t)15;
}

struct FilterWs {
  float* Qn;
  uint16_t* Qb;
  float* eq;
  int* count;
  unsigned char* flag;
  int* cand;
  int* gmax;
  float* theta;
  int* overflow_list;
  int* fix_done;
  float* fix_s;
  int64_t* fix_i;
  float* part_s;
  int* part_i;
  float* eq8;
  float* qscale;
  signed char* Qb8;
};

static size_t filter_ws_carve(char* w, const FilterShape& in, const FilterCall& c, FilterWs* out) {
  const int64_t B = in.B;
  const int D = in.D, k = in.k;
  size_t off = 0;
  auto take = [&](size_t bytes) {
    char* ptr = w ? w + off : nullptr;
    off += align_up(bytes, 256);
    return ptr;
  };
  FilterWs f;
  f.Qn = reinterpret_cast<float*>(take((size_t)B * D * sizeof(float)));
  f.Qb = B <= FILTER_QB_MAX_B ? reinterpret_cast<uint16_t*>(take((size_t)((B + 31) / 32 * 32) * D * sizeof(uint16_t))) : nullptr;
  f.eq = reinterpret_cast<float*>(take((size_t)B * sizeof(float)));
  f.count = reinterpret_cast<int*>(take((size_t)B * filter_count_stride(B) * sizeof(int)));
  f.flag = reinterpret_cast<unsigned char*>(take((size_t)B));
  f.cand = reinterpret_cast<int*>(take((size_t)B * c.cap * (c.scored_slots ? sizeof(int2) : sizeof(int))));
  f.gmax = reinterpret_cast<int*>(take((size_t)B * filter_bound_parts(k, INT64_MAX, 256) * sizeof(int)));
  f.theta = reinterpret_cast<float*>(take((size_t)B * sizeof(float)));
  f.overflow_list = reinterpret_cast<int*>(take((size_t)B * sizeof(int)));
  f.fix_done = reinterpret_cast<int*>(take((size_t)FILTER_FIX_MAX_Q * sizeof(int)));
  f.fix_s = reinterpret_cast<float*>(take((size_t)FILTER_FIX_MAX_Q * FILTER_FIX_SLICES * 32 * sizeof(float)));
  f.fix_i = reinterpret_cast<int64_t*>(take((size_t)FILTER_FIX_MAX_Q * FILTER_FIX_SLICES * 32 * sizeof(int64_t)));
  f.part_s = B <= 64 ? reinterpret_cast<float*>(take((size_t)B * 8 * k * sizeof(float))) : nullptr;
  f.part_i = B <= 64 ? reinterpret_cast<int*>(take((size_t)B * 8 * k * sizeof(int))) : nullptr;
  f.eq8 = reinterpret_cast<float*>(take((size_t)B * sizeof(float)));
  f.qscale = reinterpret_cast<float*>(take((size_t)B * sizeof(float)));
  f.Qb8 = B <= FILTER_QB_MAX_B ? reinterpret_cast<signed char*>(take((size_t)((B + 31) / 32 * 32) * D)) : nullptr;
  if (out) *out = f;
  return off;
}

static int filter_shape_code(int64_t B, int64_t N, int D, int k) {
  if (!filter_dim_ok(D)) return RAGRAPH_EUNSUPPORTED;
  return B >= 1 && N >= 1 && k >= 1 && k <= 32 && k <= N ? RAGRAPH_OK : RAGRAPH_EINVAL;
}
#define RG_REQUIRE_FILTER_SHAPE(who, B, N, D, k)                                                                      \
  do {                                                                                                                \
    const int code__ = filter_shape_code(B, N, D, k);                                                                 \
    RG_REQUIRE(code__ != RAGRAPH_EUNSUPPORTED, RAGRAPH_EUNSUPPORTED, who ": D=%d not in {64,128,256}", D);           \
    RG_REQUIRE(code__ == RAGRAPH_OK, RAGRAPH_EINVAL, who ": bad B/N/k");                                              \
  } while (0)

static FilterShape filter_query_shape(int64_t B, int64_t N, int D, int k, int n_shards, bool exchange) {
  return {B, N, N, D, k, n_shards, exchange, __builtin_nanf(""), -1, false, filter_env(), filter_device_cus()};
}

static size_t filter_workspace_bytes(FilterShape in, const FilterSchedule& sc) {
  const FilterCall planned = filter_call_plan(in, sc);
  in.exact_level0 = true;
  const FilterCall exact0 = filter_call_plan(in, sc);
  return (planned.level0_bytes > exact0.level0_bytes ? planned.level0_bytes : exact0.level0_bytes) +
         filter_ws_carve(nullptr, in, planned, nullptr) + FILTER_STATS_BYTES;
}
static size_t filter_workspace_bytes(int64_t B, int64_t N, int D, int k, int n_shards) {
  if (B < 1 || N < 1 || k < 1 || n_shards < 1 || !filter_dim_ok(D)) return 0;
  const FilterShape in = filter_query_shape(B, N, D, k, n_shards, n_shards > 1);
  return filter_workspace_bytes(in, filter_schedule(in));
}

extern "C" size_t ragraph_topk_cosine_filtered_workspace_bytes(int64_t B, int64_t N, int D, int k) {
  return filter_workspace_bytes(B, N, D, k, 1);
}
extern "C" size_t ragraph_topk_cosine_filtered_sharded_workspace_bytes(int64_t B, int64_t plan_N, int D, int k, int n_shards) {
  if (!filter_dim_ok(D)) return 0;
  const size_t a = filter_workspace_bytes(B, plan_N, D, k, n_shards), b = filter_workspace_bytes(B, plan_N, D, k, 1);
  const size_t c = ragraph_topk_cosine_workspace_bytes(B, plan_N, D, k);
  const size_t ab = a > b ? a : b;
  return ab > c ? ab : c;
}

extern "C" int ragraph_topk_cosine_filtered_i8_levels(int64_t B, int64_t N, int D, int k) {
  if (filter_shape_code(B, N, D, k) != RAGRAPH_OK) return 0;
  FilterShape in = filter_query_shape(B, N, D, k, 1, false);
  in.i8_cap = t_max_i8_levels;
  return filter_call_plan(in, filter_schedule(in)).i8_levels;
}

extern "C" int ragraph_topk_cosine_filtered_plan(int64_t B, int64_t N, int D, int k, int64_t plan[7]) {
  RG_REQUIRE(plan, RAGRAPH_EINVAL, "topk_cosine_filtered_plan: null pointer");
  RG_REQUIRE_FILTER_SHAPE("topk_cosine_filtered_plan", B, N, D, k);
  const FilterShape in = filter_query_shape(B, N, D, k, 1, false);
  const FilterCall c = filter_call_plan(in, filter_schedule(in));
  plan[0] = c.n0;
  plan[1] = c.level0 == FILTER_L0_BOUND ? 2 : (c.level0 == FILTER_L0_SLAB ? 1 : 0);
  plan[2] = c.nlev;
  for (int l = 0; l < FILTER_MAX_LEVELS; ++l) plan[3 + l] = l < c.nlev ? c.level[l].key1 : 0;
  plan[6] = c.bound_keys;
  return c.nlev;
}

extern "C" int ragraph_topk_cosine_filtered_sharded_speculates(int64_t B, int64_t plan_N, int D, int k, int n_shards) {
  if (filter_shape_code(B, plan_N, D, k) != RAGRAPH_OK || n_shards < 1) return 0;
  FilterShape in = filter_query_shape(B, plan_N, D, k, n_shards, true);
  in.prior = 0.f;
  return filter_call_plan(in, filter_schedule(in)).spec ? 1 : 0;
}

template <int D, int QW, bool BOUND, bool I8 = false, bool SCORED = false, bool PIPE = false>
static int launch_ring(FilterParams p, int64_t B, int CUS, int prof_slot, hipStream_t st) {
  using C = FilterCfg<I8 ? D / 2 : D>;
  p.qtiles = cdiv(B, (int64_t)C::WAVES * QW);
  p.xcd_map = p.qtiles >= 64 ? 1 : 0;
  p.wgs_per_group = CUS / (p.xcd_map ? 8 : 1);
  {
    const int64_t per_wg = p.qtiles * p.nstages_total / CUS;
    p.lb_min = per_wg >= 16 ? 8 : (per_wg >= 8 ? 4 : (per_wg >= 3 ? 2 : 1));
  }
  const int64_t nq0 = p.xcd_map ? (p.qtiles + 7) / 8 : p.qtiles;
  for (int v = 0; v < 2; ++v) {
    const int64_t nq = nq0 - v;
    p.depth[v] = 0;
    if (nq < 1 || (v == 1 && (!p.xcd_map || p.qtiles % 8 == 0))) continue;
    p.depth[v] = SegmentWalker::choose_depth(nq, p.nstages_total, p.wgs_per_group, p.lb_min, 0).depth;
    if (p.qtiles * p.nstages_total / CUS < 16) p.depth[v] = 0;
  }
  static DeviceOnce lds_once;
  if (hipError_t e = raise_dynamic_lds(lds_once, &topk_filter_kernel<D, QW, BOUND, I8, SCORED, PIPE>, (int)C::LDS_BYTES); e != hipSuccess) {
    set_error("topk_cosine_filtered: cannot raise dynamic LDS limit: %s", hipGetErrorString(e));
    return RAGRAPH_EDEVICE;
  }
  if (t_prof) (void)hipEventRecord(t_prof->ev[2 * prof_slot], st);
  hipLaunchKernelGGL((topk_filter_kernel<D, QW, BOUND, I8, SCORED, PIPE>), dim3((unsigned)CUS), dim3(C::THREADS), C::LDS_BYTES, st, p);
  if (t_prof) (void)hipEventRecord(t_prof->ev[2 * prof_slot + 1], st);
  RG_CHECK_LAUNCH("topk_cosine_filtered(filter)");
  ring_stamps_report(BOUND, I8);
  ring_timing_report(prof_slot, D);
  return RAGRAPH_OK;
}

struct PassVariant {
  bool direct;
  int qw;
  bool bound, i8, scored, pipe;
};
static PassVariant filter_pass_variant(int D, int64_t B, int64_t key0, int64_t key1, bool bound, bool int8, bool scored, int cus,
                                       const FilterEnv& env) {
  PassVariant v{};
  v.qw = 64;
  v.bound = bound;
  v.i8 = int8;
  v.scored = int8 && scored;
  if (B <= 256) {
    v.direct = true;
    return v;
  }
  const int64_t nstages = cdiv(key1 - key0, FILTER_STAGE_BYTES / ((int8 ? 1 : 2) * D));
  auto long_stream = [&](int64_t tile) { return cdiv(B, tile) * nstages >= 32 * (int64_t)cus; };
  if (!int8) {
    if (!bound && D == 64 && B >= 1024 && long_stream(1024)) v.qw = 128;
    return v;
  }
  const int64_t pad64 = cdiv(B, (int64_t)512) * 512 - B;
  auto fits = [&](int64_t tile) {
    return long_stream(tile) && (cdiv(B, tile) * tile - B - pad64) * 50 <= B;
  };
  const int qw = env.i8_qw ? env.i8_qw : (D == 64 && fits(1024) ? 128 : (fits(768) ? 96 : 64));
  const bool long128 = qw == 128 && long_stream(1024), long96 = qw == 96 && long_stream(768);
  if (D == 256 && ((env.pipe == 1 && !long128 && !long96) || env.pipe == 2)) v.pipe = true;
  else v.qw = long128 ? 128 : (long96 ? 96 : 64);
  return v;
}

template <int D>
static int launch_ring_variant(const PassVariant& v, const FilterParams& p, int64_t B, int cus, int prof_slot, hipStream_t st) {
  RG_REQUIRE(!v.direct && (v.qw == 64 || (v.i8 ? !v.pipe && (v.qw == 96 || v.qw == 128) : D == 64 && !v.bound && v.qw == 128)) &&
             (!v.pipe || (D == 256 && v.i8)), RAGRAPH_EINVAL, "topk_cosine_filtered: no ring kernel for D=%d qw=%d bound=%d int8=%d pipe=%d",
             D, v.qw, (int)v.bound, (int)v.i8, (int)v.pipe);
  if (v.bound) return launch_ring<D, 64, true>(p, B, cus, prof_slot, st);
  if (!v.i8) {
    if constexpr (D == 64)
      if (v.qw == 128) return launch_ring<D, 128, false>(p, B, cus, prof_slot, st);
    return launch_ring<D, 64, false>(p, B, cus, prof_slot, st);
  }
  if constexpr (D == 256)
    if (v.pipe)
      return v.scored ? launch_ring<D, 64, false, true, true, true>(p, B, cus, prof_slot, st)
                      : launch_ring<D, 64, false, true, false, true>(p, B, cus, prof_slot, st);
#define RG_RING_I8(QW_) \
  return v.scored ? launch_ring<D, QW_, false, true, true>(p, B, cus, prof_slot, st) : launch_ring<D, QW_, false, true>(p, B, cus, prof_slot, st)
  if (v.qw == 128) RG_RING_I8(128);
  if (v.qw == 96) RG_RING_I8(96);
  RG_RING_I8(64);
#undef RG_RING_I8
}

template <int D>
static int run_pass(const FilterWs& f, const uint16_t* Kb, const signed char* Kb8, int64_t B, int64_t key0, int64_t key1,
                    const FilterThr& thr, int cap, int bound_groups, bool int8, bool scored, const FilterEnv& env, int cus,
                    int prof_slot, hipStream_t st) {
  const PassVariant v = filter_pass_variant(D, B, key0, key1, bound_groups > 0, int8, scored, cus, env);
  const uint16_t* keys = v.i8 ? reinterpret_cast<const uint16_t*>(Kb8) : Kb;
  const uint16_t* Qimg = v.i8 ? reinterpret_cast<const uint16_t*>(f.Qb8) : f.Qb;
  if (v.direct) {
    DirectArgs a{};
    a.Qb = Qimg;
    a.Kb = keys;
    a.i8 = v.i8;
    a.scored = v.scored;
    a.B = B;
    a.key0 = key0;
    a.key1 = key1;
    a.thr = thr;
    a.count = f.count;
    a.cand = f.cand;
    a.cap = cap;
    a.nsub = rescore_slices(B, thr.k);
    a.gmax_out = f.gmax;
    a.bound_groups = bound_groups;
    if (t_prof) (void)hipEventRecord(t_prof->ev[2 * prof_slot], st);
    const int rc = launch_filter_direct<D>(a, st);
    if (t_prof) (void)hipEventRecord(t_prof->ev[2 * prof_slot + 1], st);
    return rc;
  }
  const int stage_keys = FILTER_STAGE_BYTES / ((v.i8 ? 1 : 2) * D);
  RG_REQUIRE(!v.i8 || key0 % stage_keys == 0, RAGRAPH_EINVAL, "topk_cosine_filtered: an int8 level must start at a whole stage "
             "(key %lld, %d keys per stage)", (long long)key0, stage_keys);
  FilterParams p{};
  p.Qn = f.Qn;
  p.Kb = keys;
  p.thr = thr;
  p.count = f.count;
  p.cstride = filter_count_stride(B);
  p.Qb = Qimg;
  p.cand = f.cand;
  p.gmax = bound_groups > 0 ? f.gmax : nullptr;
  p.ngroups = bound_groups;
  p.B = B;
  p.N = key1;
  p.cap = cap;
  p.stage_base = key0 / stage_keys;
  p.nstages_total = cdiv(key1 - key0, stage_keys);
  p.partner_lead = env.partner_lead;
  return launch_ring_variant<D>(v, p, B, cus, prof_slot, st);
}

enum RescoreKind {
  RESCORE_SCORED_SMALL,
  RESCORE_SCORED,
  RESCORE_WIDE_SLICED,
  RESCORE_WIDE_COOP,
  RESCORE_WIDE,
  RESCORE_COOP_FEW,
  RESCORE_COOP
};
static RescoreKind rescore_kind(int64_t B, int k, bool scored, bool few) {
  if (scored) return B >= 8192 ? RESCORE_SCORED_SMALL : RESCORE_SCORED;
  if (B < 2048) return rescore_slices(B, k) > 1 ? RESCORE_WIDE_SLICED : (B <= 256 ? RESCORE_WIDE_COOP : RESCORE_WIDE);
  return few ? RESCORE_COOP_FEW : RESCORE_COOP;
}

template <int D>
static int run_rescore(const FilterWs& f, const float* Kn, int64_t N, int64_t B, int cap, int k, int64_t idx_base, int merge,
                       int final_level, float* out_scores, int64_t* out_idx, int* overflow, RescoreKind kind, const FilterThr& thr,
                       int* cstat, hipStream_t st) {
  const float* ps = merge ? out_scores : nullptr;
  const int64_t* pi = merge ? out_idx : nullptr;
  const int cs = filter_count_stride(B);
  const int64_t scan_n = 0;
#define RG_SCORED(SMALL_)                                                                                                        \
  hipLaunchKernelGGL((topk_rescore_scored_kernel<D, SMALL_>), dim3((unsigned)cdiv(B, 2)), dim3(128), 0, st, f.Qn, Kn, f.count,    \
                     reinterpret_cast<const int2*>(f.cand), B, cap, cs, k, idx_base, ps, pi, final_level, out_scores, out_idx,   \
                     overflow, f.overflow_list, f.flag, scan_n, thr, cstat)
#define RG_WIDE(SLICED_, COOP_, GRID_, PART_S_, PART_I_)                                                                         \
  hipLaunchKernelGGL((topk_rescore_wide_kernel<D, SLICED_, COOP_>), GRID_, dim3(256), 0, st, f.Qn, Kn, f.count, f.cand, B, N,    \
                     cap, cs, k, idx_base, ps, pi, final_level, out_scores, out_idx, overflow, f.overflow_list, f.flag, PART_S_, \
                     PART_I_, cstat)
#define RG_COOP(FEW_)                                                                                                            \
  hipLaunchKernelGGL((topk_rescore_coop_kernel<D, 32, FEW_>), dim3((unsigned)cdiv(B, 2)), dim3(128), 0, st, f.Qn, Kn, f.count,    \
                     f.cand, B, cap, cs, k, idx_base, ps, pi, final_level, out_scores, out_idx, overflow, f.overflow_list,       \
                     f.flag, scan_n, cstat)
  switch (kind) {
    case RESCORE_SCORED_SMALL: RG_SCORED(true); break;
    case RESCORE_SCORED: RG_SCORED(false); break;
    case RESCORE_WIDE_SLICED:
      RG_WIDE(true, true, dim3((unsigned)B, (unsigned)rescore_slices(B, k)), f.part_s, f.part_i);
      wide_timing_report();
      break;
    case RESCORE_WIDE_COOP: RG_WIDE(false, true, dim3((unsigned)B), (float*)nullptr, (int*)nullptr); break;
    case RESCORE_WIDE: RG_WIDE(false, false, dim3((unsigned)B), (float*)nullptr, (int*)nullptr); break;
    case RESCORE_COOP_FEW: RG_COOP(true); break;
    case RESCORE_COOP: RG_COOP(false); break;
  }
#undef RG_SCORED
#undef RG_WIDE
#undef RG_COOP
  RG_CHECK_LAUNCH("topk_cosine_filtered(rescore)");
  return RAGRAPH_OK;
}

struct FilteredArgs {
  const float* Q;
  int64_t B;
  const float *Kn, *Kp;
  const uint16_t* Kb;
  int64_t N;
  int D, k;
  int64_t idx_base;
  float* out_scores;
  int64_t* out_idx;
  int* overflow;
  int64_t* overflow_idx;
  void* ws;
  size_t ws_bytes;
  void* stream;
  int64_t plan_N;
  float* theta;
  ragraph_exchange_fn exchange;
  void* ctx;
  int n_shards;
};

static int launch_theta(FilterThr thr, int64_t B, int first, float* theta, hipStream_t st) {
  thr.gmax = nullptr;
  thr.theta = nullptr;
  hipLaunchKernelGGL(filter_theta_kernel, dim3((unsigned)cdiv(B, 256)), dim3(256), 0, st, thr, B, first, theta);
  RG_CHECK_LAUNCH("topk_cosine_filtered(theta)");
  return RAGRAPH_OK;
}

static int run_exact_participant(const FilteredArgs& a, const FilterCall& c) {
  hipStream_t st = as_stream(a.stream);
  RG_REQUIRE(a.ws_bytes >= ragraph_topk_cosine_workspace_bytes(a.B, a.N, a.D, a.k), RAGRAPH_EWORKSPACE,
             "topk_cosine_filtered: workspace too small for a short shard's exact top-k");
  int rc = ragraph_topk_cosine_bank_f32(a.Q, a.B, a.Kn, a.D == 256 ? a.Kp : nullptr, a.N, a.D, a.k, a.idx_base, a.out_scores,
                                        a.out_idx, a.ws, a.ws_bytes, a.stream);
  if (rc != RAGRAPH_OK) return rc;
  if (hipMemsetAsync(a.overflow, 0, sizeof(int), st) != hipSuccess) {
    set_error("topk_cosine_filtered: memset failed");
    return RAGRAPH_EDEVICE;
  }
  FilterThr t0{};
  t0.prev_scores = a.out_scores;
  t0.k = a.k;
  for (int ph = c.first_phase; ph < c.nlev; ++ph) {
    if ((rc = launch_theta(t0, a.B, ph == c.first_phase, a.theta, st)) != RAGRAPH_OK) return rc;
    a.exchange(a.ctx, ph);
  }
  return RAGRAPH_OK;
}

template <int D>
static int run_filtered(const FilteredArgs& a, const FilterCall& c, const FilterShape& in) {
  hipStream_t st = as_stream(a.stream);
  const int64_t B = a.B, N = a.N;
  const int k = a.k;
  float* const out_scores = a.out_scores;
  int64_t* const out_idx = a.out_idx;
  const bool sharded = a.exchange != nullptr, bound = c.level0 == FILTER_L0_BOUND;
  static const int ablate = [] {
    const char* e = getenv("RAGRAPH_FILTER_ABLATE");
    return e ? atoi(e) : 0;
  }();
  if (t_prof) t_prof->have = t_prof->bound = 0;

  char* w = static_cast<char*>(a.ws);
  FilterWs f;
  const size_t used = c.level0_bytes + filter_ws_carve(w + c.level0_bytes, in, c, &f) + FILTER_STATS_BYTES;
  RG_REQUIRE(used <= a.ws_bytes, RAGRAPH_EWORKSPACE, "topk_cosine_filtered: the schedule of this call needs %zu bytes of workspace, "
             "%zu given", used, a.ws_bytes);
  int* stats = reinterpret_cast<int*>(w + ragraph_topk_cosine_filtered_stats_offset(a.ws_bytes));
  const unsigned* max_kerr2 = reinterpret_cast<const unsigned*>(a.Kb + filter_round_up(N) * D);
  const FilterI8View v8 = filter_i8_view(a.Kb, N, D);

  FilterStatsInit stats_init{};
  stats_init.nlev = c.nlev;
  for (int l = 0; l < c.nlev; ++l) {
    stats_init.i8[l] = c.level[l].int8;
    const int64_t lk = c.level[l].key1 - c.level[l].key0;
    stats_init.keys[l] = lk > INT_MAX ? INT_MAX : (int)lk;
  }
#define RG_PREP(R_)                                                                                                                     \
  hipLaunchKernelGGL((filter_prep_kernel<D, R_>), dim3((unsigned)cdiv(B <= FILTER_QB_MAX_B ? (B + 31) / 32 * 32 : B, 4 * (R_))), dim3(256), 0, st, a.Q, B, \
                     f.Qn, f.eq, f.count, f.flag, a.overflow, bound ? f.gmax : nullptr, c.parts, c.bf16_image ? f.Qb : nullptr,         \
                     filter_count_stride(B), c.i8_levels > 0 ? f.eq8 : nullptr, f.qscale, B <= FILTER_QB_MAX_B ? f.Qb8 : nullptr, f.fix_done, \
                     stats, stats_init, c.spec ? (sharded ? a.theta : f.theta) : nullptr, in.prior)
  if (B >= 8192) RG_PREP(4);
  else RG_PREP(1);
#undef RG_PREP
  RG_CHECK_LAUNCH("topk_cosine_filtered(prepare)");

  FilterThr thr{};
  thr.eq = f.eq;
  thr.max_kerr2 = max_kerr2;
  thr.eq8 = f.eq8;
  thr.qscale = f.qscale;
  thr.tail8 = v8.tail8;
  thr.cls8 = v8.cls;
  thr.flag = f.flag;
  thr.k = k;
  thr.ngroups = c.parts;
  thr.ablate = ablate;
  int rc = RAGRAPH_OK;
  switch (c.level0) {
    case FILTER_L0_NONE: break;
    case FILTER_L0_BOUND:
      rc = run_pass<D>(f, a.Kb, v8.K8, B, 0, c.bound_keys, thr, c.cap, c.parts, false, false, in.env, in.cus, 3, st);
      if (t_prof) {
        t_prof->bound = 1;
        t_prof->i8[3] = 0;
        t_prof->keys[3] = c.bound_keys;
      }
      break;
    case FILTER_L0_SLAB: {
      float* S = reinterpret_cast<float*>(w);
      for (int64_t b0 = 0; b0 < B && rc == RAGRAPH_OK; b0 += FILTER_SLAB_MAX_B) {
        const int64_t nb = B - b0 < FILTER_SLAB_MAX_B ? B - b0 : FILTER_SLAB_MAX_B;
        rc = ragraph_linear_f32(f.Qn + b0 * D, nb, D, a.Kn, c.n0, nullptr, RAGRAPH_ACT_NONE, 0.f, S, a.stream);
        if (rc == RAGRAPH_OK)
          rc = ragraph_topk_rows_f32(S, nb, c.n0, c.n0, k, out_scores + b0 * k, out_idx + b0 * k, a.stream);
      }
      break;
    }
    case FILTER_L0_TILE:
      rc = ragraph_topk_cosine_bank_f32(a.Q, B, a.Kn, D == 256 ? a.Kp : nullptr, c.n0, D, k, 0, out_scores, out_idx, a.ws,
                                        c.level0_bytes, a.stream);
      break;
  }
  if (rc != RAGRAPH_OK) return rc;
  if (sharded && c.spec) {
    thr.theta = a.theta;
  } else if (sharded) {
    thr.gmax = bound ? f.gmax : nullptr;
    thr.prev_scores = out_scores;
    if (bound) {
      hipLaunchKernelGGL(filter_bound_scores_kernel, dim3((unsigned)cdiv(B, 4)), dim3(256), 0, st, thr, B, out_scores, a.theta);
      RG_CHECK_LAUNCH("topk_cosine_filtered(theta)");
    } else if ((rc = launch_theta(thr, B, 1, a.theta, st)) != RAGRAPH_OK) {
      return rc;
    }
    a.exchange(a.ctx, 0);
    thr.theta = a.theta;
  } else if (bound && c.parts > k) {
    thr.gmax = f.gmax;
    hipLaunchKernelGGL(filter_bound_scores_kernel, dim3((unsigned)cdiv(B, 4)), dim3(256), 0, st, thr, B, (float*)nullptr, f.theta);
    RG_CHECK_LAUNCH("topk_cosine_filtered(theta)");
  }

  for (int l = 0; l < c.nlev; ++l) {
    const FilterLevel& lv = c.level[l];
    thr.gmax = (l == 0 && bound && !sharded && c.parts == k) ? f.gmax : nullptr;
    if (!sharded) thr.theta = (c.spec || (l == 0 && bound && c.parts > k)) ? f.theta : nullptr;
    thr.prev_scores = out_scores;
    rc = run_pass<D>(f, a.Kb, v8.K8, B, lv.key0, lv.key1, thr, c.cap, 0, lv.int8, lv.scored, in.env, in.cus, l, st);
    if (t_prof) {
      t_prof->i8[l] = lv.int8;
      t_prof->keys[l] = lv.key1 - lv.key0;
    }
    if (rc != RAGRAPH_OK) return rc;
    if (t_prof) t_prof->have = l + 1;
    rc = run_rescore<D>(f, a.Kn, N, B, c.cap, k, a.idx_base, l > 0, l == c.nlev - 1, out_scores, out_idx, a.overflow,
                        rescore_kind(B, k, lv.scored, sharded && l > 0), thr, stats + 2 + l, st);
    if (rc != RAGRAPH_OK) return rc;
    if (l + 1 == c.nlev) break;
    if (sharded) {
      if ((rc = launch_theta(thr, B, 0, a.theta, st)) != RAGRAPH_OK) return rc;
      a.exchange(a.ctx, 1 + l);
    } else if (c.spec) {
      if ((rc = launch_theta(thr, B, 0, f.theta, st)) != RAGRAPH_OK) return rc;
    }
  }

  if (c.spec && !sharded) {
    hipLaunchKernelGGL(filter_verify_prior_kernel, dim3((unsigned)cdiv(B, 256)), dim3(256), 0, st, out_scores, B, k, in.prior, 1, f.flag,
                       a.overflow, f.overflow_list, stats);
    RG_CHECK_LAUNCH("topk_cosine_filtered(verify)");
  }
  hipLaunchKernelGGL(topk_overflow_fixup_kernel<D>, dim3(256), dim3(256), 0, st, f.Qn, a.Kn, N, k, a.idx_base,
                     a.overflow, f.overflow_list, a.overflow_idx, out_scores, out_idx, f.fix_done, f.fix_s, f.fix_i, B, f.flag,
                     sharded ? nullptr : stats);
  RG_CHECK_LAUNCH("topk_cosine_filtered(overflow fallback)");
  return RAGRAPH_OK;
}

static int filtered_entry(const FilteredArgs& a) {
  const int64_t B = a.B, N = a.N, plan_N = a.plan_N;
  const int D = a.D, k = a.k;
  RG_REQUIRE(a.Q && a.Kn && a.Kb && a.out_scores && a.out_idx && a.overflow && a.ws, RAGRAPH_EINVAL, "topk_cosine_filtered: null pointer");
  RG_REQUIRE(a.n_shards >= 1, RAGRAPH_EINVAL, "topk_cosine_filtered: n_shards=%d", a.n_shards);
  RG_REQUIRE_FILTER_SHAPE("topk_cosine_filtered", B, N, D, k);
  RG_REQUIRE(N < (int64_t)INT_MAX - 1024, RAGRAPH_EUNSUPPORTED, "topk_cosine_filtered: shard rows must fit int32");
  RG_REQUIRE(plan_N >= N && (a.exchange || plan_N - N <= 1024), RAGRAPH_EINVAL, "topk_cosine_filtered: plan_N must be the largest shard's size");
  RG_REQUIRE(!a.exchange || a.theta, RAGRAPH_EINVAL, "topk_cosine_filtered: an exchange needs the theta buffer");
  RG_REQUIRE(aligned16(a.Q) && aligned16(a.Kn) && aligned16(a.Kb) && aligned16(a.ws), RAGRAPH_EINVAL,
             "topk_cosine_filtered: pointers must be 16-B aligned");
  const FilterShape one = filter_query_shape(B, plan_N, D, k, 1, false);
  const FilterSchedule sc_one = filter_schedule(one);
  const size_t need = filter_workspace_bytes(one, sc_one);
  RG_REQUIRE(a.ws_bytes >= need, RAGRAPH_EWORKSPACE, "topk_cosine_filtered: workspace %zu < %zu", a.ws_bytes, need);
  const FilterShape in{B, N, plan_N, D, k, a.n_shards, a.exchange != nullptr, t_prior, t_max_i8_levels, false, one.env, one.cus};
  const FilterCall c = filter_call_plan(in, a.exchange && a.n_shards > 1 ? filter_schedule(in) : sc_one);
  if (c.exact_participant) return run_exact_participant(a, c);
  if (D == 256) return run_filtered<256>(a, c, in);
  if (D == 128) return run_filtered<128>(a, c, in);
  return run_filtered<64>(a, c, in);
}

extern "C" int ragraph_topk_cosine_filtered_f32(const float* Q, int64_t B, const float* Kn, const float* Kp,
                                                const uint16_t* Kb, int64_t N, int D, int k, int64_t idx_base,
                                                float* out_scores, int64_t* out_idx, int* overflow,
                                                int64_t* overflow_idx, void* ws, size_t ws_bytes, void* stream) {
  return filtered_entry({Q, B, Kn, Kp, Kb, N, D, k, idx_base, out_scores, out_idx, overflow, overflow_idx, ws, ws_bytes, stream,
                         N, nullptr, nullptr, nullptr, 1});
}

extern "C" int ragraph_topk_cosine_filtered_sharded_f32(const float* Q, int64_t B, const float* Kn, const float* Kp,
                                                        const uint16_t* Kb, int64_t N, int D, int k, int64_t idx_base,
                                                        float* out_scores, int64_t* out_idx, int* overflow,
                                                        int64_t* overflow_idx, void* ws, size_t ws_bytes, void* stream,
                                                        int64_t plan_N, float* theta, ragraph_exchange_fn exchange,
                                                        void* ctx, int n_shards) {
  return filtered_entry({Q, B, Kn, Kp, Kb, N, D, k, idx_base, out_scores, out_idx, overflow, overflow_idx, ws, ws_bytes, stream,
                         plan_N, theta, exchange, ctx, n_shards});
}

extern "C" int ragraph_verify_merged_prior_f32(const float* merged_scores, int64_t R, int k, float prior, int speculative,
                                               const int* stats_words, const int* overflow, float* out5, void* stream) {
  RG_REQUIRE(out5 && (merged_scores || R == 0), RAGRAPH_EINVAL, "verify_merged_prior: null pointer");
  RG_REQUIRE(R >= 0 && k >= 1, RAGRAPH_EINVAL, "verify_merged_prior: bad R/k");
  hipLaunchKernelGGL(verify_merged_prior_kernel, dim3(1), dim3(256), 0, as_stream(stream), merged_scores, R, k, prior, speculative,
                     stats_words, overflow, out5);
  RG_CHECK_LAUNCH("verify_merged_prior");
  return RAGRAPH_OK;
}

extern "C" int ragraph_theta_sharpen_f32(const float* gathered, int G, int64_t B, int m, int k, float* theta, void* stream) {
  RG_REQUIRE(gathered && theta, RAGRAPH_EINVAL, "theta_sharpen: null pointer");
  RG_REQUIRE(G >= 1 && m >= 1 && k >= 1 && G * m <= 64 && G * m >= k, RAGRAPH_EINVAL,
             "theta_sharpen: need k <= G*m <= 64 (G=%d m=%d k=%d)", G, m, k);
  if (B <= 0) return RAGRAPH_OK;
  if (G * m <= 32 && B >= 4096)
    hipLaunchKernelGGL(theta_sharpen2_kernel, dim3((unsigned)cdiv(B, 8)), dim3(256), 0, as_stream(stream), gathered, G, B, m, k,
                       theta);
  else
    hipLaunchKernelGGL(theta_sharpen_kernel, dim3((unsigned)cdiv(B, 4)), dim3(256), 0, as_stream(stream), gathered, G, B, m, k,
                       theta);
  RG_CHECK_LAUNCH("theta_sharpen");
  return RAGRAPH_OK;
}
```

### ragraph_amd/csrc/topk_filter_direct.hip

```cpp
#include "filter_common.h"
#include <type_traits>

namespace ragraph {

template <int D_>
struct DirectCfg {
  static constexpr int D = D_;
  static constexpr int WAVES = 8, THREADS = 512;
  static constexpr int KSTEPS = D / 16;
  static constexpr int KS32 = D / 32;
  static constexpr int UNIT_BLOCKS = 16;
  static constexpr int SUBS = UNIT_BLOCKS / KSTEPS;
  static constexpr int UNIT_KEYS = 32 * SUBS;
  static constexpr int CAND_BUF = SUBS == 1 ? 256 : (SUBS <= 4 ? 512 : 128 * SUBS + 64);
  static constexpr int GROUP_BYTES = KS32 * 1024;
#ifndef RG_DIRECT_LA
#define RG_DIRECT_LA 4
#endif
  static constexpr int LA = KS32 < RG_DIRECT_LA ? KS32 : RG_DIRECT_LA;
  static constexpr size_t lds_bytes(int groups_in_lds) {
    return (size_t)groups_in_lds * GROUP_BYTES + (size_t)WAVES * CAND_BUF * 8 + 512 * sizeof(float) + WAVES * sizeof(int);
  }
};

struct DirectParams {
  const uint16_t* Qb;
  const uint16_t* Kb;
  int64_t B;
  int64_t unit0, nunits;
  int64_t key_end;
  FilterThr thr;
  int* count;
  int* cand;
  int cap, nsub, subcap;
  int scored;
  int* gmax;
  int ngroups;
  int qgroups;
};

#ifdef RG_DIRECT_TIMING
__device__ unsigned long long g_direct_t[2][2][8];
#define RG_DSTAMP(i_)                                                                       \
  if (threadIdx.x == 0 && (blockIdx.x == 0 || blockIdx.x == gridDim.x - 1))                \
  g_direct_t[BOUND][blockIdx.x != 0][i_] = wall_clock64()
#else
#define RG_DSTAMP(i_)
#endif

typedef int i32x4 __attribute__((ext_vector_type(4)));

template <int D, bool QREG, bool BOUND, bool I8 = false>
__global__ void __launch_bounds__(512, 2) topk_filter_direct_kernel(DirectParams p) {
  using C = DirectCfg<I8 ? D / 2 : D>;
  static_assert(!(I8 && BOUND), "the bound pass runs on the bf16 copy");
  using acc_t = typename std::conditional<I8, i32x4, f32x4>::type;
  RG_DSTAMP(0);
  extern __shared__ float4 dsmem4[];
  char* smem = reinterpret_cast<char*>(dsmem4);
  const int ngl = QREG ? 0 : p.qgroups;
  char* qlds = smem;
  uint2* wbuf_all = reinterpret_cast<uint2*>(smem + (size_t)ngl * C::GROUP_BYTES);
  float* thr_lds = reinterpret_cast<float*>(wbuf_all + C::WAVES * C::CAND_BUF);

  const int tid = threadIdx.x;
  const int lane = tid & 63;
  const int wave = __builtin_amdgcn_readfirstlane(tid >> 6);
  const int j = lane & 15, g = lane >> 4;

  if (tid < (I8 ? 512 : 256)) {
    if constexpr (I8) {
      int t = INT_MAX;
      if ((tid & 255) < p.B) t = filter_threshold_i8(p.thr, tid & 255, tid >> 8);
      thr_lds[tid] = __int_as_float(t);
    } else {
      float t = __builtin_huge_valf();
      if (!BOUND && tid < p.B) t = filter_threshold(p.thr, tid);
      thr_lds[tid] = t;
    }
  }
  if constexpr (!QREG) {
    const int pieces = ngl * C::KS32 * 64;
    for (int i = tid; i < pieces; i += C::THREADS)
      *reinterpret_cast<f32x4*>(qlds + (size_t)i * 16) = reinterpret_cast<const f32x4*>(p.Qb)[i];
  }
  bf16x8 bq[QREG ? C::KSTEPS : 1];
  if constexpr (QREG) {
#pragma unroll
    for (int t = 0; t < C::KSTEPS; ++t) bq[t] = reinterpret_cast<const bf16x8*>(p.Qb)[t * 64 + lane];
  }
  __syncthreads();
  asm volatile("s_waitcnt vmcnt(0) lgkmcnt(0)" ::: "memory");
  RG_DSTAMP(1);

  const int64_t W = (int64_t)gridDim.x * C::WAVES;
  const int64_t gw = (int64_t)blockIdx.x * C::WAVES + wave;
  const int64_t chunk = (p.nunits + W - 1) / W;
  const int64_t ubase = BOUND ? gw * chunk : gw;
  const int64_t ustride = BOUND ? 1 : W;
  const int64_t n_mine = BOUND ? (ubase < p.nunits ? (p.nunits - ubase < chunk ? p.nunits - ubase : chunk) : 0)
                               : (gw < p.nunits ? (p.nunits - gw + W - 1) / W : 0);
  uint2* wbuf = wbuf_all + wave * C::CAND_BUF;
  float* gm_lds = reinterpret_cast<float*>(wbuf);
  int cur_part = -1;
  if constexpr (BOUND) {
#pragma unroll
    for (int e = 0; e < 4; ++e) gm_lds[lane + 64 * e] = RG_NEG_INF;
  }
  auto flush_max = [&]() {
    if (cur_part >= 0) {
#pragma unroll
      for (int e = 0; e < 4; ++e) {
        const int qq = lane + 64 * e;
        const float v = gm_lds[qq];
        if (qq < p.B && v > RG_NEG_INF) atomicMax(p.gmax + (int64_t)qq * p.ngroups + cur_part, f2ord(v));
        gm_lds[qq] = RG_NEG_INF;
      }
    }
  };
  int wcnt = 0;
  const unsigned lane16 = (unsigned)lane * 16u;

  const int sub = (int)(gw & (p.nsub - 1));
  auto flush = [&]() {
    for (int i0 = 0; i0 < wcnt; i0 += 64) {
      const int i = i0 + lane;
      if (i < wcnt) {
        const uint2 e = wbuf[i];
        const int64_t q = I8 ? ((e.y >> 8) & 0xFFu) : (e.y >> 16);
        unsigned mk = I8 ? (e.y & 0xFFu) : (e.y & 0xFFFFu);
        int slot = atomicAdd(p.count + q * FILTER_COUNT_STRIDE + sub, __popc(mk));
        asm volatile("s_waitcnt vmcnt(0)" : "+v"(slot) : : "memory");
        while (mk) {
          const int r = __ffs(mk) - 1;
          mk &= mk - 1;
          if (slot < p.subcap) {
            const int64_t at = q * p.cap + sub * p.subcap + slot;
            const int key = (int)e.x + (r & 3) + 16 * (r >> 2);
            if (I8 && p.scored) reinterpret_cast<int2*>(p.cand)[at] = make_int2(key, (((int)e.y >> 17) * 512) | (int)((e.y >> 16) & 1u));
            else p.cand[at] = key;
          }
          ++slot;
        }
      }
    }
    wcnt = 0;
  };

  f32x4 A0[16], A1[16];
#define RG_DLOAD(buf_, u_)                                                                                         \
  {                                                                                                                \
    const char* ub_ = reinterpret_cast<const char*>(p.Kb) + (uint64_t)(u_) * (C::UNIT_BLOCKS * 1024) + lane16;     \
    _Pragma("unroll") for (int b_ = 0; b_ < 16; ++b_)                                                              \
      buf_[b_] = __builtin_nontemporal_load(reinterpret_cast<const f32x4*>(ub_ + b_ * 1024));                      \
  }
#define RG_DWAIT(cnt_, reg_)

  [[maybe_unused]] int cls_unit = 0;
  auto epilogue = [&](const acc_t (&a)[2], int gq, int64_t unit, int sub, int part) {
#if defined(RG_DIRECT_ABL) && (RG_DIRECT_ABL & 1)
    if (a[0][0] + a[1][3] == 123456) wbuf[0] = make_uint2(1u, 2u);
    return;
#endif
    if constexpr (I8) {
      int m = a[0][0];
#pragma unroll
      for (int r = 1; r < 4; ++r) m = max(m, a[0][r]);
#pragma unroll
      for (int r = 0; r < 4; ++r) m = max(m, a[1][r]);
      const int th = __float_as_int(thr_lds[256 * cls_unit + 16 * gq + j]);
      if (__any(m >= th)) {
        unsigned mk = 0;
        const unsigned tm1 = (unsigned)(max(-(1 << 24), min(1 << 24, th)) - 1);
#pragma unroll
        for (int b = 7; b >= 0; --b) mk = __builtin_amdgcn_alignbit(mk, tm1 - (unsigned)a[b >> 2][b & 3], 31);
        const int64_t key_base = (unit * C::SUBS + sub) * 32 + 4 * g;
        if (key_base + 32 > p.key_end) {
          unsigned vm = 0;
#pragma unroll
          for (int r = 0; r < 8; ++r) vm |= (key_base + (r & 3) + 16 * (r >> 2) < p.key_end) ? (1u << r) : 0u;
          mk &= vm;
        }
        const unsigned long long bal = __ballot(mk != 0);
        if (bal) {
          const int pos = wcnt + (int)__builtin_amdgcn_mbcnt_hi((unsigned)(bal >> 32), __builtin_amdgcn_mbcnt_lo((unsigned)bal, 0u));
          if (mk) wbuf[pos] = make_uint2((unsigned)key_base, mk | ((unsigned)(16 * gq + j) << 8) |
                                                             ((unsigned)((((m + 255) >> 8) << 1) | cls_unit) << 16));
          wcnt += __popcll(bal);
        }
      }
      return;
    }
    float m = (float)a[0][0];
#pragma unroll
    for (int r = 1; r < 4; ++r) m = fmaxf(m, (float)a[0][r]);
#pragma unroll
    for (int r = 0; r < 4; ++r) m = fmaxf(m, (float)a[1][r]);
    if constexpr (BOUND) {
      if (part != cur_part) {
        flush_max();
        cur_part = part;
      }
      m = fmaxf(m, __shfl_xor(m, 16));
      m = fmaxf(m, __shfl_xor(m, 32));
      if (g == 0) gm_lds[16 * gq + j] = fmaxf(gm_lds[16 * gq + j], m);
    } else {
      const float th = thr_lds[16 * gq + j];
      if (__any(m >= th)) {
        unsigned mk = 0;
#pragma unroll
// ... 56 lines not shown
            }
          }
#pragma unroll
        for (int gq = 0; gq < 2; ++gq) epilogue(acc[gq], gq, unit, sub, part_of(sub));
      }
    } else {
      f32x4 fr[C::LA];
#if defined(RG_DIRECT_ABL) && (RG_DIRECT_ABL & 2)
#pragma unroll
      for (int t = 0; t < C::LA; ++t) fr[t] = f32x4{1.f, 2.f, 3.f, 4.f};
#define RG_BREAD(slot_, addr_, blk_) asm volatile("" : "+v"(fr[(slot_) % C::LA]))
#define RG_BWAIT(slot_) asm volatile("" : "+v"(fr[(slot_) % C::LA]))
#else
#define RG_BREAD(slot_, addr_, blk_) \
  asm volatile("ds_read_b128 %0, %1 offset:%2" : "=v"(fr[(slot_) % C::LA]) : "v"(addr_), "n"((blk_) * 1024))
#define RG_BWAIT(slot_) asm volatile("s_waitcnt lgkmcnt(%1)" : "+v"(fr[(slot_) % C::LA]) : "n"(C::LA - 1))
#endif
#pragma unroll
      for (int t = 0; t < C::LA; ++t) RG_BREAD(t, qaddr0, t);
      for (int gq = 0; gq < ngl; ++gq) {
        if constexpr (!BOUND) {
          if (wcnt > C::CAND_BUF - 64 * C::SUBS) flush();
        }
        const unsigned cur = qaddr0 + (unsigned)gq * C::GROUP_BYTES;
        acc_t acc[C::SUBS][2];
#pragma unroll
        for (int sub = 0; sub < C::SUBS; ++sub) acc[sub][0] = acc[sub][1] = acc_t{0, 0, 0, 0};
#define RG_GSTEP(t_)                                                                                            \
  if constexpr ((t_) < C::KS32) {                                                                               \
    RG_BWAIT(t_);                                                                                               \
    {                                                                                                           \
      _Pragma("unroll") for (int sub = 0; sub < C::SUBS; ++sub)                                                 \
        _Pragma("unroll") for (int h = 0; h < 2; ++h) {                                                         \
          if constexpr (I8)                                                                                     \
            acc[sub][h] = __builtin_bit_cast(acc_t, __builtin_amdgcn_mfma_i32_16x16x64_i8(                      \
                __builtin_bit_cast(i32x4, A[(sub * C::KS32 + (t_)) * 2 + h]),                                   \
                __builtin_bit_cast(i32x4, fr[(t_) % C::LA]), __builtin_bit_cast(i32x4, acc[sub][h]), 0, 0, 0)); \
          else                                                                                                  \
            acc[sub][h] = __builtin_bit_cast(acc_t, __builtin_amdgcn_mfma_f32_16x16x32_bf16(                    \
                __builtin_bit_cast(bf16x8, A[(sub * C::KS32 + (t_)) * 2 + h]),                                  \
                __builtin_bit_cast(bf16x8, fr[(t_) % C::LA]), __builtin_bit_cast(f32x4, acc[sub][h]), 0, 0, 0)); \
        }                                                                                                       \
    }                                                                                                           \
    RG_BREAD(t_, cur, (t_) + C::LA);                                                                            \
  }
        RG_GSTEP(0) RG_GSTEP(1) RG_GSTEP(2) RG_GSTEP(3) RG_GSTEP(4) RG_GSTEP(5) RG_GSTEP(6) RG_GSTEP(7)
#undef RG_GSTEP
#pragma unroll
        for (int sub = 0; sub < C::SUBS; ++sub) epilogue(acc[sub], gq, unit, sub, part_of(sub));
      }
#pragma unroll
      for (int t = 0; t < C::LA; ++t) asm volatile("s_waitcnt lgkmcnt(0)" : "+v"(fr[t]));
#undef RG_BWAIT
#undef RG_BREAD
    }
  };

  auto cls_word = [&](int64_t u) -> unsigned {
    if constexpr (I8) return p.thr.cls8[__builtin_amdgcn_readfirstlane((int)(u >> 6))];
    else return 0u;
  };
  if (n_mine > 0) {
    const int64_t u0 = p.unit0 + ubase;
    RG_DLOAD(A0, u0);
    unsigned w0 = cls_word(u0), w1 = 0u;
    int64_t i = 0;
    for (; i + 2 <= n_mine; i += 2) {
      RG_DLOAD(A1, u0 + (i + 1) * ustride);
      w1 = cls_word(u0 + (i + 1) * ustride);
      process(A0, u0 + i * ustride, w0, std::true_type{});
      if (i + 2 < n_mine) {
        RG_DLOAD(A0, u0 + (i + 2) * ustride);
        w0 = cls_word(u0 + (i + 2) * ustride);
        process(A1, u0 + (i + 1) * ustride, w1, std::true_type{});
      } else {
        process(A1, u0 + (i + 1) * ustride, w1, std::false_type{});
      }
    }
    if (i < n_mine) process(A0, u0 + i * ustride, w0, std::false_type{});
  }
  RG_DSTAMP(2);
  if constexpr (BOUND) {
    int* wave_part = reinterpret_cast<int*>(thr_lds + 256);
    if (lane == 0) wave_part[wave] = cur_part;
    __syncthreads();
    if (tid < 256 && tid < p.B) {
      const float* all = reinterpret_cast<const float*>(wbuf_all);
      float m = RG_NEG_INF;
      int part = -1;
      for (int w = 0; w < C::WAVES; ++w) {
        const int pw = wave_part[w];
        if (pw < 0) continue;
        if (pw != part) {
          if (part >= 0 && m > RG_NEG_INF) atomicMax(p.gmax + (int64_t)tid * p.ngroups + part, f2ord(m));
          part = pw;
          m = RG_NEG_INF;
        }
        m = fmaxf(m, all[(size_t)w * C::CAND_BUF * 2 + tid]);
      }
      if (part >= 0 && m > RG_NEG_INF) atomicMax(p.gmax + (int64_t)tid * p.ngroups + part, f2ord(m));
    }
  } else {
    flush();
  }
  RG_DSTAMP(3);
#undef RG_DWAIT
#undef RG_DLOAD
}

template <int D, bool QREG, bool BOUND, bool I8 = false>
static int launch_direct(const DirectParams& p, int grid, size_t lds, hipStream_t st) {
  static DeviceOnce lds_once;
  if (hipError_t e = raise_dynamic_lds(lds_once, &topk_filter_direct_kernel<D, QREG, BOUND, I8>, 160 * 1024); e != hipSuccess) {
    set_error("topk_cosine_filtered(direct): cannot raise dynamic LDS limit: %s", hipGetErrorString(e));
    return RAGRAPH_EDEVICE;
  }
  hipLaunchKernelGGL((topk_filter_direct_kernel<D, QREG, BOUND, I8>), dim3((unsigned)grid), dim3(512), lds, st, p);
  RG_CHECK_LAUNCH("topk_cosine_filtered(direct filter)");
#ifdef RG_DIRECT_TIMING
  {
    (void)hipDeviceSynchronize();
    unsigned long long t[2][2][8];
    (void)hipMemcpyFromSymbol(t, HIP_SYMBOL(g_direct_t), sizeof(t));
    for (int b = 0; b < 2; ++b)
      fprintf(stderr, "[direct timing, %s pass, %s block of %d, 10 ns ticks] prologue %lld units %lld tail %lld (started %lld after block 0)\n",
              BOUND ? "bound" : "filter", b ? "last" : "first", grid, (long long)(t[BOUND][b][1] - t[BOUND][b][0]),
              (long long)(t[BOUND][b][2] - t[BOUND][b][1]), (long long)(t[BOUND][b][3] - t[BOUND][b][2]),
              (long long)(t[BOUND][b][0] - t[BOUND][0][0]));
  }
#endif
  return RAGRAPH_OK;
}

template <int D>
static int launch_filter_direct_i8(const DirectArgs& a, hipStream_t st) {
  using C = DirectCfg<D / 2>;
  RG_REQUIRE(a.B >= 1 && a.B <= 256 && a.bound_groups == 0, RAGRAPH_EINVAL, "filter(direct, int8): bad batch / mode");
  RG_REQUIRE(a.key0 % C::UNIT_KEYS == 0 && a.key1 > a.key0, RAGRAPH_EINVAL, "filter(direct, int8): bad key range");
  DirectParams p{};
  p.Qb = a.Qb;
  p.Kb = a.Kb;
  p.B = a.B;
  p.unit0 = a.key0 / C::UNIT_KEYS;
  p.nunits = cdiv(a.key1 - a.key0, (int64_t)C::UNIT_KEYS);
  p.key_end = a.key1;
  p.thr = a.thr;
  p.count = a.count;
  p.cand = a.cand;
  p.cap = a.cap;
  p.nsub = a.nsub < 1 ? 1 : a.nsub;
  RG_REQUIRE((p.nsub & (p.nsub - 1)) == 0 && p.nsub <= FILTER_COUNT_STRIDE, RAGRAPH_EINVAL, "filter(direct): nsub=%d", p.nsub);
  p.subcap = a.cap / p.nsub;
  p.scored = a.scored;
  p.qgroups = 2 * (int)cdiv(a.B, 32);
  const int cus = device_cus_multiple_of_8();
  int64_t grid = cdiv(p.nunits, (int64_t)C::WAVES);
  if (grid > cus) grid = cus;
  const bool qreg = a.B <= 32;
  const size_t lds = C::lds_bytes(qreg ? 0 : p.qgroups);
  return qreg ? launch_direct<D, true, false, true>(p, (int)grid, lds, st) : launch_direct<D, false, false, true>(p, (int)grid, lds, st);
}

template <int D>
int launch_filter_direct(const DirectArgs& a, hipStream_t st) {
  using C = DirectCfg<D>;
  if (a.i8) return launch_filter_direct_i8<D>(a, st);
  RG_REQUIRE(a.B >= 1 && a.B <= 256, RAGRAPH_EINVAL, "filter(direct): B=%lld not in [1,256]", (long long)a.B);
  RG_REQUIRE(a.key0 % C::UNIT_KEYS == 0 && a.key1 > a.key0, RAGRAPH_EINVAL, "filter(direct): bad key range");
  DirectParams p{};
  p.Qb = a.Qb;
  p.Kb = a.Kb;
  p.B = a.B;
  p.unit0 = a.key0 / C::UNIT_KEYS;
  p.nunits = cdiv(a.key1 - a.key0, (int64_t)C::UNIT_KEYS);
  p.key_end = a.key1;
  p.thr = a.thr;
  p.count = a.count;
  p.cand = a.cand;
  p.cap = a.cap;
  p.nsub = a.nsub < 1 ? 1 : a.nsub;
  RG_REQUIRE((p.nsub & (p.nsub - 1)) == 0 && p.nsub <= FILTER_COUNT_STRIDE, RAGRAPH_EINVAL, "filter(direct): nsub=%d", p.nsub);
  p.subcap = a.cap / p.nsub;
  p.gmax = a.gmax_out;
  p.ngroups = a.bound_groups;
  p.qgroups = 2 * (int)cdiv(a.B, 32);
  const bool bound = a.bound_groups > 0;
  if (bound)
    RG_REQUIRE(p.nunits * C::SUBS >= a.bound_groups, RAGRAPH_EINVAL, "filter(direct): bound range shorter than its parts");
  const int cus = device_cus_multiple_of_8();
  int64_t grid = cdiv(p.nunits, (int64_t)C::WAVES);
  if (grid > cus) grid = cus;
  const bool qreg = a.B <= 32;
  const size_t lds = C::lds_bytes(qreg ? 0 : p.qgroups);
  if (qreg) return bound ? launch_direct<D, true, true>(p, (int)grid, lds, st) : launch_direct<D, true, false>(p, (int)grid, lds, st);
  return bound ? launch_direct<D, false, true>(p, (int)grid, lds, st) : launch_direct<D, false, false>(p, (int)grid, lds, st);
}

template int launch_filter_direct<64>(const DirectArgs&, hipStream_t);
template int launch_filter_direct<128>(const DirectArgs&, hipStream_t);
template int launch_filter_direct<256>(const DirectArgs&, hipStream_t);

}
```

### ragraph_amd/kernels.py

```python
from __future__ import annotations

import ctypes
import os

import torch

from . import _native as N
from ._native import ACT_ELU, ACT_LEAKY, ACT_NONE, ACT_PRELU, ACT_RELU, RagraphNativeError

_device_ok = False


def _ready():
    global _device_ok
    if not _device_ok:
        N.require_device()
        _device_ok = True
    return N.lib()


def _f32c(t: torch.Tensor, name: str) -> torch.Tensor:
    if not isinstance(t, torch.Tensor) or not t.is_cuda:
        raise RagraphNativeError(f"{name}: expected a ROCm device tensor (ragraph_amd has no CPU fallback)")
    if t.dtype != torch.float32:
# ... 37 lines not shown
_ws_cache: dict = {}
_WS_CACHE_MAX = 8


def _workspace(nbytes: int, device) -> torch.Tensor:
    dev = device.index if device.index is not None else torch.cuda.current_device()
    stream = _raw_stream(dev) if _raw_stream is not None else torch.cuda.current_stream(dev).cuda_stream
    key = (dev, stream)
    ws = _ws_cache.pop(key, None)
    if ws is None or ws.numel() < nbytes:
        ws = torch.empty(max(nbytes, 1 << 20), dtype=torch.uint8, device=device)
    _ws_cache[key] = ws
    while len(_ws_cache) > _WS_CACHE_MAX:
        _ws_cache.pop(next(iter(_ws_cache)))
    return ws


def pack_keys(keys_normalized: torch.Tensor) -> torch.Tensor:
    L = _ready()
    kn = _f32c(keys_normalized, "pack_keys.keys")
    out = torch.empty_like(kn)
    if kn.shape[0] == 0:
        return out
    N.check(L.ragraph_pack_keys_f32(kn.data_ptr(), kn.shape[0], kn.shape[1], out.data_ptr(), _stream()), "pack_keys")
    return out


def packed_keys_help(B: int, D: int, k: int) -> bool:
    return B > 128 and D == 256 and k <= 14


FUSED_WIDTHS = (64, 128, 256)


def padded_dim(D: int):
    for w in FUSED_WIDTHS:
        if D <= w:
            return w
    return None


def pad_cols(x: torch.Tensor, width: int) -> torch.Tensor:
    x = _f32c(x, "pad_cols.x")
    if x.shape[1] == width:
        return x
    out = x.new_zeros((x.shape[0], width))
    out[:, :x.shape[1]] = x
    return out


def topk_cosine(q: torch.Tensor, keys_normalized: torch.Tensor, k: int, idx_base: int = 0,
                keys_packed: torch.Tensor | None = None):
    L = _ready()
    q = _f32c(q, "topk_cosine.q")
    kn = _f32c(keys_normalized, "topk_cosine.keys")
    kp = 0
    if keys_packed is not None:
        kpt = _f32c(keys_packed, "topk_cosine.keys_packed")
        if kpt.shape != kn.shape:
            raise RagraphNativeError(f"topk_cosine: keys_packed {tuple(kpt.shape)} != keys {tuple(kn.shape)}")
        kp = kpt.data_ptr()
    if q.dim() != 2 or kn.dim() != 2 or q.shape[1] != kn.shape[1]:
        raise RagraphNativeError(f"topk_cosine: bad shapes {tuple(q.shape)} x {tuple(kn.shape)}")
    B, D = q.shape
    Nk = kn.shape[0]
    scores = torch.empty((B, k), dtype=torch.float32, device=q.device)
    idx = torch.empty((B, k), dtype=torch.int64, device=q.device)
    if B == 0:
        return scores, idx
    nbytes = L.ragraph_topk_cosine_workspace_bytes(B, Nk, D, k)
    ws = _workspace(nbytes, q.device)
    N.check(L.ragraph_topk_cosine_bank_f32(q.data_ptr(), B, kn.data_ptr(), kp, Nk, D, k, idx_base, scores.data_ptr(),
                                           idx.data_ptr(), ws.data_ptr(), ws.numel(), _stream()), "topk_cosine")
    return scores, idx


def topk_cosine_mix_workspace_bytes(B: int, n_keys: int, D: int, A: int, k: int) -> int:
    return int(N.lib().ragraph_topk_cosine_mix_workspace_bytes(B, n_keys, D, A, k))


def topk_cosine_mix(q: torch.Tensor, keys_normalized: torch.Tensor, pos_q: torch.Tensor, pos_normalized: torch.Tensor,
                    w_struct: float, w_sem: float, k: int, idx_base: int = 0):
    L = _ready()
    q = _f32c(q, "topk_cosine_mix.q")
    kn = _f32c(keys_normalized, "topk_cosine_mix.keys")
    pq = _f32c(pos_q, "topk_cosine_mix.pos_q")
    pn = _f32c(pos_normalized, "topk_cosine_mix.pos_normalized")
    if q.dim() != 2 or kn.dim() != 2 or q.shape[1] != kn.shape[1]:
        raise RagraphNativeError(f"topk_cosine_mix: bad shapes {tuple(q.shape)} x {tuple(kn.shape)}")
    if pq.dim() != 2 or pn.dim() != 2 or pq.shape[1] != pn.shape[1] or pq.shape[0] != q.shape[0] or pn.shape[0] != kn.shape[0]:
        raise RagraphNativeError(f"topk_cosine_mix: codes {tuple(pq.shape)} x {tuple(pn.shape)} do not match "
                                 f"{tuple(q.shape)} x {tuple(kn.shape)}")
    B, D = q.shape
    Nk, A = pn.shape
    scores = torch.empty((B, k), dtype=torch.float32, device=q.device)
    idx = torch.empty((B, k), dtype=torch.int64, device=q.device)
    if B == 0:
        return scores, idx
    nbytes = L.ragraph_topk_cosine_mix_workspace_bytes(B, Nk, D, A, k)
    ws = _workspace(nbytes, q.device)
    N.check(L.ragraph_topk_cosine_mix_f32(q.data_ptr(), B, kn.data_ptr(), Nk, D, pq.data_ptr(), pn.data_ptr(), A,
                                          float(w_struct), float(w_sem), k, idx_base, scores.data_ptr(), idx.data_ptr(),
                                          ws.data_ptr(), ws.numel(), _stream()), "topk_cosine_mix")
    return scores, idx


def keys_to_bf16(keys_normalized: torch.Tensor) -> torch.Tensor:
    L = _ready()
    kn = _f32c(keys_normalized, "keys_to_bf16.keys")
    rows = L.ragraph_keys_bf16_rows(kn.shape[0])
    out = torch.empty((rows, kn.shape[1]), dtype=torch.int16, device=kn.device)
    if kn.shape[0]:
        N.check(L.ragraph_keys_to_bf16(kn.data_ptr(), kn.shape[0], kn.shape[1], out.data_ptr(), _stream()), "keys_to_bf16")
    return out


def bank_copy_errors(keys_bf16: torch.Tensor, n_keys: int):
    npad = -(-n_keys // 256) * 256
    t16 = keys_bf16[npad, :2].contiguous().view(torch.float32).cpu()
    t8 = keys_bf16[npad + 1 + npad // 2, :4].contiguous().view(torch.float32).cpu()
    return float(t16[0]) ** 0.5, float(t8[0]) ** 0.5, float(t8[1])


def int8_copy_classes(keys_bf16: torch.Tensor, n_keys: int) -> dict:
    npad = -(-n_keys // 256) * 256
    row = keys_bf16[npad + 1 + npad // 2, :16].contiguous()
    f, i = row.view(torch.float32).cpu(), row.view(torch.int32).cpu()
    return {"err": float(f[0]) ** 0.5, "scale": float(f[1]), "max_abs": float(f[2]), "err_heavy": float(f[3]) ** 0.5,
            "scale_heavy": float(f[4]), "cut": float(f[5]), "heavy_granules": int(i[6]), "granules": int(i[7])}


def filtered_i8_levels(B: int, n_keys: int, D: int, k: int) -> int:
    return N.lib().ragraph_topk_cosine_filtered_i8_levels(B, n_keys, D, k)


def sharded_speculates(B: int, plan_n: int, D: int, k: int, n_shards: int) -> bool:
    return bool(N.lib().ragraph_topk_cosine_filtered_sharded_speculates(B, plan_n, D, k, n_shards))


def verify_merged_prior(merged_scores: torch.Tensor, prior, stats=None, overflow=None) -> torch.Tensor:
    L = _ready()
    ms = _f32c(merged_scores, "verify_merged_prior.scores")
    R, k = ms.shape
    out = torch.empty(5, dtype=torch.float32, device=ms.device)
    N.check(L.ragraph_verify_merged_prior_f32(ms.data_ptr() if R else None, R, k, 0.0 if prior is None else float(prior),
                                              0 if prior is None else 1, stats.data_ptr() if stats is not None else None,
                                              overflow.data_ptr() if overflow is not None else None, out.data_ptr(), _stream()),
            "verify_merged_prior")
    return out


def set_filter_prior(theta_prior) -> float:
    return N.lib().ragraph_topk_cosine_filtered_set_prior(float("nan") if theta_prior is None else float(theta_prior))


def ord2f(v: int) -> float:
    import struct

    v = int(v)
    if v < 0:
        v ^= 0x7FFFFFFF
    return struct.unpack("<f", struct.pack("<i", v))[0]


def set_max_i8_levels(n: int) -> int:
    return N.lib().ragraph_topk_cosine_filtered_max_i8_levels(int(n))


def expected_i8_candidates(B: int, n_keys: int, D: int, k: int) -> float:
    L = N.lib()
    plan = (ctypes.c_int64 * 7)()
    if L.ragraph_topk_cosine_filtered_plan(B, n_keys, D, k, plan) <= 0:
        return 0.0
    nlev = int(plan[2])
    n_i8 = L.ragraph_topk_cosine_filtered_i8_levels(B, n_keys, D, k)
    ends = [max(int(plan[0]), 1)] + [int(plan[3 + l]) for l in range(nlev)]
    return sum(3.9 * k * ends[l + 1] / ends[l] for l in range(nlev) if l >= nlev - n_i8)


def filter_helps(B: int, n_keys: int, D: int, k: int) -> bool:
    if os.environ.get("RAGRAPH_EXACT_FP32") == "1":
        return False
    if D not in (64, 128, 256) or k > 32:
        return False
    if n_keys >= 65536:
        return B >= FILTER_MIN_B
    if n_keys >= 32768:
        return B >= 128
    if n_keys < 8192:
        return False
    if D >= 128:
        return B >= 512
    return B >= (2048 if n_keys >= 16384 else 8192)


FILTER_MIN_B = int(os.environ.get("RAGRAPH_FILTER_MIN_B", "1"))


_EXCHANGE_FN = ctypes.CFUNCTYPE(None, ctypes.c_void_p, ctypes.c_int)

FILTER_STATS = True
FILTER_STATS_MAGIC = 0x52414753


def filter_stats_levels(stats) -> list:
    st = [int(x) for x in stats]
    if len(st) < 16 or st[0] != FILTER_STATS_MAGIC:
        return []
    return [("int8" if st[8 + l] else "bf16", st[11 + l], (st[2 + l] / st[5 + l]) if st[5 + l] else None)
            for l in range(min(st[1], 3))]


def topk_cosine_filtered(q: torch.Tensor, keys_normalized: torch.Tensor, keys_bf16: torch.Tensor, k: int,
                         idx_base: int = 0, keys_packed: torch.Tensor | None = None, exchange=None, plan_n: int = 0,
                         return_stats: bool = False):
    L = _ready()
    q = _f32c(q, "topk_cosine_filtered.q")
    kn = _f32c(keys_normalized, "topk_cosine_filtered.keys")
    B, D = q.shape
    Nk = kn.shape[0]
    if keys_bf16.dtype != torch.int16 or not keys_bf16.is_contiguous() or keys_bf16.shape[1] != D or \
            keys_bf16.shape[0] != L.ragraph_keys_bf16_rows(Nk):
        raise RagraphNativeError("topk_cosine_filtered: keys_bf16 must come from keys_to_bf16(keys_normalized)")
    kp = 0
    if keys_packed is not None:
        kpt = _f32c(keys_packed, "topk_cosine_filtered.keys_packed")
        if kpt.shape != kn.shape:
            raise RagraphNativeError("topk_cosine_filtered: keys_packed shape mismatch")
        kp = kpt.data_ptr()
    scores = torch.empty((B, k), dtype=torch.float32, device=q.device)
    idx = torch.empty((B, k), dtype=torch.int64, device=q.device)
    overflow = torch.empty(1, dtype=torch.int32, device=q.device)
    if exchange is None:
        nbytes = L.ragraph_topk_cosine_filtered_workspace_bytes(B, max(plan_n, Nk), D, k)
    else:
        nbytes = L.ragraph_topk_cosine_filtered_sharded_workspace_bytes(B, max(plan_n, Nk), D, k,
                                                                        int(getattr(exchange, "n_shards", 1)))
    if nbytes == 0:
        raise RagraphNativeError(f"topk_cosine_filtered: unsupported shape B={B} N={Nk} D={D} k={k}")
    ws = _workspace(nbytes, q.device)
    off = L.ragraph_topk_cosine_filtered_stats_offset(ws.numel())
    stats = ws[off:off + 128].view(torch.int32)
    if exchange is None:
        N.check(L.ragraph_topk_cosine_filtered_f32(q.data_ptr(), B, kn.data_ptr(), kp, keys_bf16.data_ptr(), Nk, D, k,
                                                   idx_base, scores.data_ptr(), idx.data_ptr(), overflow.data_ptr(), None,
                                                   ws.data_ptr(), ws.numel(), _stream()),
                "topk_cosine_filtered")
        return (scores, idx, overflow, stats) if return_stats else (scores, idx, overflow)
    theta = torch.empty(B, dtype=torch.float32, device=q.device)
    errors = []

    def _cb(_ctx, phase):
        try:
            exchange(int(phase), theta, scores)
        except BaseException as e:
            errors.append(e)

    cb = _EXCHANGE_FN(_cb)
    rc = L.ragraph_topk_cosine_filtered_sharded_f32(q.data_ptr(), B, kn.data_ptr(), kp, keys_bf16.data_ptr(), Nk, D, k,
                                                    idx_base, scores.data_ptr(), idx.data_ptr(), overflow.data_ptr(), None,
                                                    ws.data_ptr(), ws.numel(), _stream(), max(plan_n, Nk),
                                                    theta.data_ptr(), cb, None, int(getattr(exchange, "n_shards", 1)))
    if errors:
        raise errors[0]
    N.check(rc, "topk_cosine_filtered(sharded)")
    return (scores, idx, overflow, stats) if return_stats else (scores, idx, overflow)


def fused_helps(B: int, n_keys: int, D: int, k: int) -> bool:
    if os.environ.get("RAGRAPH_EXACT_FP32") == "1" or os.environ.get("RAGRAPH_TOPK_FUSED", "1") == "0":
        return False
    if D not in (64, 128, 256) or k > 16 or n_keys < 128 * k:
        return False
    if 2 * n_keys * D > FUSED_MAX_COPY_BYTES or (D >= 128 and n_keys >= 8192):
        return False
    return B * n_keys >= FUSED_MIN_SCORES


FUSED_MAX_COPY_BYTES = int(os.environ.get("RAGRAPH_FUSED_MAX_COPY", str(3 << 20)))
FUSED_MIN_SCORES = int(os.environ.get("RAGRAPH_FUSED_MIN_SCORES", "12000000"))


_fused_tickets: dict = {}


def _tickets(n: int, device) -> torch.Tensor:
    dev = device.index if device.index is not None else torch.cuda.current_device()
    key = (dev, _raw_stream(dev) if _raw_stream is not None else torch.cuda.current_stream(dev).cuda_stream)
    t = _fused_tickets.get(key)
    if t is None or t.numel() < n:
        t = torch.zeros(max(n, 1024), dtype=torch.int32, device=device)
        _fused_tickets[key] = t
    return t


def topk_cosine_fused(q: torch.Tensor, keys_normalized: torch.Tensor, keys_bf16: torch.Tensor, k: int, idx_base: int = 0):
    L = _ready()
    q = _f32c(q, "topk_cosine_fused.q")
    kn = _f32c(keys_normalized, "topk_cosine_fused.keys")
    B, D = q.shape
    Nk = kn.shape[0]
    if keys_bf16.dtype != torch.int16 or not keys_bf16.is_contiguous() or keys_bf16.shape[1] != D or \
            keys_bf16.shape[0] != L.ragraph_keys_bf16_rows(Nk):
        raise RagraphNativeError("topk_cosine_fused: keys_bf16 must come from keys_to_bf16(keys_normalized)")
    scores = torch.empty((B, k), dtype=torch.float32, device=q.device)
    idx = torch.empty((B, k), dtype=torch.int64, device=q.device)
# ... 1257 lines not shown
```

### ragraph_amd/kernels_index.py

```python
from __future__ import annotations

import os

import torch

from ._native import TOPK_MAX


class KeyIndex:

    MAX_FILTERED_BATCH = 262144
    I8_MAX_ERR = 0.02
    OVERFLOW_FRACTION = 1.0 / 64
    I8_MAX_CANDIDATES_BASE = 300.0
    I8_MAX_CANDIDATES_PER_KEY = 1.2e-3
    REPROBE_QUERIES = 1 << 20
    REPROBE_MAX_BATCH = 4096
    SPEC_MIN_BATCH = 17
    SPEC_WARM_CALLS = 2
    SPEC_WARM_QUERIES = 64
    SPEC_MARGIN = 0.5
    SPEC_MIN_MARGIN = 0.01
    SPEC_MAX_CANDIDATES = 1.5
    SPEC_HISTORY = 16
    DEDUP_MIN_ROWS = 2048
    DEDUP_MAX_UNIQUE = 0.9
    DEDUP_MAX_GROUP = 64

    def __init__(self, keys_normalized: torch.Tensor, ops=None, dedup: bool = True):
        if ops is None:
            from . import kernels as ops
        self.ops = ops
        self.dim = int(keys_normalized.shape[1])
        pad = getattr(ops, "padded_dim", None)
        self._width = pad(self.dim) if pad is not None else self.dim
        if self._width is not None and self._width != self.dim:
            keys_normalized = ops.pad_cols(keys_normalized, self._width)
        self.keys_normalized = keys_normalized
        self._packed = None
        self._bf16 = None
        self._filter_off = False
        self._i8_off = False
        self.i8_classes = None
        self._pending = None
        self._i8_ok = None
        self._seen_i8, self._seen_bf16 = [0, 0], [0, 0]
        self._queries = 0
        self._demoted = {"i8": None, "filter": None}
        self._reprobe_after = {"i8": self.REPROBE_QUERIES, "filter": self.REPROBE_QUERIES}
        self._probed_at = {"i8": None, "filter": None}
        self._host_word = self._event = None
        self._overflowed = 0
        self.last_i8_candidates = None
        self._spec = {}
        self.spec_enabled = os.environ.get("RAGRAPH_SPEC", "1") != "0"
        self._notes = 0
        self.last_stats = None
        self.last_prior = None
        self.last_over = None
        self._collapsed = None if dedup else False
        self.duplicate_stats = None

    @property
    def overflowed_queries(self) -> int:
        return self._overflowed + (self._collapsed[0].overflowed_queries if self._collapsed else 0)

    @property
    def search_index(self) -> "KeyIndex":
        return self._collapsed[0] if self._collapsed else self

    def search_rows(self, min_unique: int = 0) -> int:
        if self._collapsed is None:
            self._judge_duplicates()
        if self._collapsed and self._collapsed[0].keys_normalized.shape[0] < min_unique:
            self._collapsed = False
        return int(self.search_index.keys_normalized.shape[0])

    def _judge_duplicates(self):
        kn = self.keys_normalized
        dedup = getattr(self.ops, "dedup_rows", None)
        if dedup is None or kn.shape[0] < self.DEDUP_MIN_ROWS:
            self._collapsed = False
            return
        if kn.is_cuda and torch.cuda.is_current_stream_capturing():
            return
        U, largest, uniq_row, group_ptr, members = dedup(kn)
        self.duplicate_stats = (kn.shape[0], U, largest)
        if U > self.DEDUP_MAX_UNIQUE * kn.shape[0] and largest <= self.DEDUP_MAX_GROUP:
            self._collapsed = False
            return
        unique = self.ops.gather_rows(kn, uniq_row)
        self._collapsed = (KeyIndex(unique, self.ops, dedup=False), group_ptr, members)

    def _poll_overflow(self):
        pend = self._pending
        if pend is None or (torch.cuda.is_available() and torch.cuda.is_current_stream_capturing()):
            return
        if not pend[1].query():
            return
        n_over, B = int(pend[0][0]), pend[2]
        if n_over < 0:
            n_over = int(pend[0][21]) if int(pend[0][1]) == 0x52414753 else 0
        self._pending = None
        words = pend[0][1:].tolist()
        speculative = False
        if len(pend) > 4 and pend[4] and len(words) >= 20 and words[0] == 0x52414753:
            speculative = bool(words[16])
            n_over = self._judge_prior(pend[4], B, words, n_over)
        self._overflowed += n_over
        i8_was_off = self._i8_off
        if pend[3] and pend[0].numel() > 16 and not speculative:
            from .kernels import filter_stats_levels
            i8 = [(keys, c) for dt, keys, c in filter_stats_levels(pend[0][1:17].tolist()) if dt == "int8" and c is not None]
            if i8:
                self.last_i8_candidates = sum(c for _, c in i8)
                if self.last_i8_candidates > self.I8_MAX_CANDIDATES_BASE + self.I8_MAX_CANDIDATES_PER_KEY * sum(kk for kk, _ in i8):
                    self._demote("i8")
        acc = self._seen_i8 if pend[3] else self._seen_bf16
        acc[0] += B
        acc[1] += n_over
        if (B >= 64 and n_over >= 2 and n_over > self.OVERFLOW_FRACTION * B) or (acc[0] >= 8 and 4 * acc[1] > acc[0]):
            if pend[3] and not i8_was_off:
                self._demote("i8")
            else:
                self._demote("filter")
            acc[0] = acc[1] = 0
        elif acc[0] >= 4096:
            acc[0] = acc[1] = 0

    def _judge_prior(self, k: int, B: int, words, n_over: int) -> int:
        st = self._spec_state(k)
        spec, failed, lo, hi = words[16], words[17], words[18], words[19]
        lists_over = max(n_over - failed, 0)
        cand = None
        if any(words[5 + l] for l in range(3)):
            cand = sum(words[2 + l] / words[5 + l] for l in range(min(words[1], 3)) if words[5 + l])
        if lists_over:
            st["hist"], st["queries"] = [], 0
        elif lo != 0x7FFFFFFF and hi != -0x80000000 and B - failed > 0:
            from .kernels import ord2f
            st["hist"].append((ord2f(lo), ord2f(hi)))
            del st["hist"][:-self.SPEC_HISTORY]
            st["queries"] += B
        if not spec:
            if cand is not None and not lists_over:
                st["cand"] = cand
            return lists_over
        st["used"] += 1
        st["failed"] += failed
        loose = cand is not None and st["cand"] is not None and cand > self.SPEC_MAX_CANDIDATES * max(st["cand"], 32.0)
        if failed or loose or lists_over:
            probed_at = st.get("probed_at")
            if probed_at is not None and self._queries - probed_at < st["after"]:
                st["after"] = min(st["after"] * 4, 1 << 40)
            st["off_at"] = self._queries
            if failed:
                st["hist"] = []
                st["queries"] = 0
        return 0

    def _demote(self, what: str):
        if what == "i8":
            self._i8_off = True
        else:
            self._filter_off = True
        if self._demoted[what] is None:
            probed_at = self._probed_at[what]
            if probed_at is not None and self._queries - probed_at < self._reprobe_after[what]:
                self._reprobe_after[what] = min(self._reprobe_after[what] * 4, 1 << 40)
            else:
                self._reprobe_after[what] = self.REPROBE_QUERIES
            self._demoted[what] = self._queries

    def _maybe_reprobe(self, B: int):
        if B > self.REPROBE_MAX_BATCH:
            return
        for what in ("filter", "i8"):
            at = self._demoted[what]
            if at is not None and self._queries - at >= self._reprobe_after[what]:
                if what == "i8":
                    self._i8_off = False
                    self._seen_i8 = [0, 0]
                else:
                    self._filter_off = False
                    self._seen_bf16 = [0, 0]
                self._demoted[what] = None
                self._probed_at[what] = self._queries
                return

    def _spec_state(self, k: int) -> dict:
        st = self._spec.get(k)
        if st is None:
            st = self._spec[k] = {"hist": [], "queries": 0, "off_at": None, "after": self.REPROBE_QUERIES, "cand": None,
                                  "failed": 0, "used": 0}
        return st

    def _prior_for(self, B: int, k: int, small: bool = False):
        if not self.spec_enabled or (B < self.SPEC_MIN_BATCH and not small) or getattr(self.ops, "set_filter_prior", None) is None:
            return None
        if torch.cuda.is_available() and torch.cuda.is_current_stream_capturing():
            return None
        st = self._spec_state(k)
        if st["off_at"] is not None:
            if self._queries - st["off_at"] < st["after"] or B > self.REPROBE_MAX_BATCH:
                return None
            st["off_at"] = None
            st["probed_at"] = self._queries
        if len(st["hist"]) < self.SPEC_WARM_CALLS or st["queries"] < self.SPEC_WARM_QUERIES:
            return None
        lo = min(h[0] for h in st["hist"])
        hi = max(h[1] for h in st["hist"])
        return lo - max(self.SPEC_MARGIN * (hi - lo), self.SPEC_MIN_MARGIN)

    def _note_overflow(self, over, B: int, had_i8: bool, stats=None, k: int = 0):
        if not over.is_cuda:
            self._overflowed += int(over)
        elif self._pending is None and not torch.cuda.is_current_stream_capturing():
            self._notes += 1
            if B <= 64 and (self._notes & 3) and self.last_prior is not None:
                return
            if self._host_word is None:
                self._host_word = torch.zeros(33, dtype=torch.int32).pin_memory()
                self._event = torch.cuda.Event()
            if stats is not None and stats.numel() >= 32:
                self._host_word[1:33].copy_(stats[:32], non_blocking=True)
                self._host_word[0] = -1
            else:
                self._host_word[:1].copy_(over, non_blocking=True)
                self._host_word[1:].zero_()
                if stats is not None:
                    self._host_word[1:1 + stats.numel()].copy_(stats, non_blocking=True)
            self._event.record()
            self._pending = (self._host_word, self._event, B, had_i8, k)

    def _cap_i8(self):
        cap = getattr(self.ops, "set_max_i8_levels", None)
        if cap is None:
            return None, False
        if self._i8_ok is None and not (torch.cuda.is_available() and torch.cuda.is_current_stream_capturing()):
            c = self.ops.int8_copy_classes(self._bf16, self.keys_normalized.shape[0])
            many_heavy = 4 * c["heavy_granules"] > c["granules"] and c["err_heavy"] > self.I8_MAX_ERR
            self._i8_ok = c["err"] <= self.I8_MAX_ERR and not many_heavy
            self.i8_classes = c
        allowed = bool(self._i8_ok) and not self._i8_off
        cap(-1 if allowed else 0)
        return cap, allowed

    def sharded_speculates(self, B: int, k: int, plan_n: int, n_shards: int) -> bool:
        ops = self.ops
        if self._width is None or getattr(ops, "set_filter_prior", None) is None or getattr(ops, "sharded_speculates", None) is None:
            return False
        fhelps = getattr(ops, "filter_helps", None)
        if fhelps is None or B > self.MAX_FILTERED_BATCH or not fhelps(B, plan_n, self._width, k):
            return False
        return bool(ops.sharded_speculates(B, plan_n, self._width, k, n_shards))

    def topk(self, q: torch.Tensor, k: int, idx_base: int = 0, exchange=None, plan_n: int = 0, prior=None):
        ops, kn = self.ops, self.keys_normalized
        if q.shape[1] != self.dim:
            raise ValueError(f"KeyIndex.topk: queries of {q.shape[1]} columns against a bank of {self.dim}")
        if k > TOPK_MAX and exchange is None:
            if self._width is not None and self._width != self.dim:
                q = ops.pad_cols(q, self._width)
            return ops.topk_cosine(q, kn, k, idx_base=idx_base)
        if self._width is None:
            return ops.topk_cosine(q, kn, k, idx_base=idx_base)
        if self._width != self.dim:
            q = ops.pad_cols(q, self._width)
        B, D = q.shape
        if self._collapsed is None:
            self._judge_duplicates()
        if self._collapsed:
            inner, group_ptr, members = self._collapsed
            U = inner.keys_normalized.shape[0]
            if exchange is None:
                su, iu = inner.topk(q, min(k, U))
                return ops.topk_expand_groups(su, iu, group_ptr, members, k, idx_base=idx_base)
            if U >= k:
                su, iu = inner.topk(q, k, 0, exchange, plan_n, prior)
                return ops.topk_expand_groups(su, iu, group_ptr, members, k, idx_base=idx_base)
            raise RuntimeError("KeyIndex: a collapsed shard of fewer unique rows than k cannot take part in the exchanges; "
                               "ShardedToyGraphBase keeps such a shard uncollapsed (search_rows(min_unique=k))")
        fhelps = getattr(ops, "filter_helps", None)
        if exchange is not None:
            if fhelps is not None and fhelps(B, max(plan_n, kn.shape[0]), D, k) and B <= self.MAX_FILTERED_BATCH:
                if self._bf16 is None:
                    self._bf16 = ops.keys_to_bf16(kn)
                cap, _ = self._cap_i8()
                if prior is not None:
                    ops.set_filter_prior(prior)
                try:
                    if getattr(ops, "FILTER_STATS", False):
                        s, i, self.last_over, self.last_stats = ops.topk_cosine_filtered(
                            q, kn, self._bf16, k, idx_base=idx_base, exchange=exchange, plan_n=plan_n, return_stats=True)
                    else:
                        s, i, self.last_over = ops.topk_cosine_filtered(q, kn, self._bf16, k, idx_base=idx_base,
                                                                        exchange=exchange, plan_n=plan_n)
                finally:
                    if cap is not None:
                        cap(-1)
                    if prior is not None:
                        ops.set_filter_prior(None)
                self.last_prior = prior
                return s, i
            fhelps = None
        self._poll_overflow()
        self._maybe_reprobe(B)
        self._queries += B
        fused = getattr(ops, "fused_helps", None)
        if fused is not None and not self._filter_off and fused(B, kn.shape[0], D, k):
            if self._bf16 is None:
                self._bf16 = ops.keys_to_bf16(kn)
            return ops.topk_cosine_fused(q, kn, self._bf16, k, idx_base=idx_base)
        small = getattr(ops, "small_helps", None)
        if (small is not None and not self._filter_off and small(B, kn.shape[0], D, k)
                and getattr(ops, "small_state_ready", lambda _d: True)(q.device)):
            if self._bf16 is None:
                self._bf16 = ops.keys_to_bf16(kn)
            cap, had_i8 = self._cap_i8()
            stats = None
            prior = self._prior_for(B, k, small=True)
            if prior is not None:
                ops.set_filter_prior(prior)
            try:
                if getattr(ops, "FILTER_STATS", False):
                    s, i, over, stats = ops.topk_cosine_small(q, kn, self._bf16, k, idx_base=idx_base, return_stats=True)
                else:
                    s, i, over = ops.topk_cosine_small(q, kn, self._bf16, k, idx_base=idx_base)
            finally:
                if cap is not None:
                    cap(-1)
                if prior is not None:
                    ops.set_filter_prior(None)
            self.last_prior = prior
            self._note_overflow(over, B, had_i8 and D in (128, 256), stats, k)
            return s, i
        if fhelps is not None and not self._filter_off and fhelps(B, kn.shape[0], D, k):
            if self._bf16 is None:
                self._bf16 = ops.keys_to_bf16(kn)
            if B > self.MAX_FILTERED_BATCH:
                outs = [self.topk(q[b0:b0 + self.MAX_FILTERED_BATCH], k, idx_base)
                        for b0 in range(0, B, self.MAX_FILTERED_BATCH)]
                return torch.cat([o[0] for o in outs]), torch.cat([o[1] for o in outs])
            cap, had_i8 = self._cap_i8()
            had_i8 = had_i8 and ops.filtered_i8_levels(B, kn.shape[0], D, k) > 0
            stats = None
            prior = self._prior_for(B, k)
            if prior is not None:
                ops.set_filter_prior(prior)
            try:
                if getattr(ops, "FILTER_STATS", False):
                    s, i, over, stats = ops.topk_cosine_filtered(q, kn, self._bf16, k, idx_base=idx_base,
                                                                 keys_packed=self._packed, return_stats=True)
                else:
                    s, i, over = ops.topk_cosine_filtered(q, kn, self._bf16, k, idx_base=idx_base, keys_packed=self._packed)
            finally:
                if cap is not None:
                    cap(-1)
                if prior is not None:
                    ops.set_filter_prior(None)
            self.last_prior = prior
            self._note_overflow(over, B, had_i8, stats, k)
            self.last_stats = stats
            return s, i
        helps = getattr(ops, "packed_keys_help", None)
        if helps is not None and helps(B, D, k):
            if self._packed is None:
                self._packed = ops.pack_keys(kn)
            return ops.topk_cosine(q, kn, k, idx_base=idx_base, keys_packed=self._packed)
        return ops.topk_cosine(q, kn, k, idx_base=idx_base)
```

Baseline: 5.002 million.

## Add tight speculative threshold with gated repair pass for soft queries

Adds a second, tighter speculative threshold derived from the history of observed k-th scores, so the filtered top-k can run a single filter level with fewer candidates. Queries whose k-th score falls below the tight threshold are marked soft and cleared. Up to 256 of them are gathered into a small batch and re-run through the filter and rescore using buffers carved from idle list space. If too many queries are soft, a full-batch fallback pass runs, and device-side gates make those kernels exit early when unused. This trades fewer levels and fewer candidates for extra small launches and the risk of costly fallbacks when the margin is wrong.

```diff
diff --git a/include/ragraph_hip.h b/include/ragraph_hip.h
--- a/include/ragraph_hip.h
+++ b/include/ragraph_hip.h
@@ -52,6 +52,7 @@
 int ragraph_topk_cosine_filtered_i8_levels(int64_t B, int64_t N, int D, int k);
 int ragraph_topk_cosine_filtered_max_i8_levels(int n);
 float ragraph_topk_cosine_filtered_set_prior(float theta_prior);
+float ragraph_topk_cosine_filtered_set_tight_prior(float t);
 int ragraph_topk_cosine_filtered_f32(const float* Q, int64_t B, const float* Kn, const float* Kp, const uint16_t* Kb,
                                      int64_t N, int D, int k, int64_t idx_base, float* out_scores, int64_t* out_idx,
                                      int* overflow, int64_t* overflow_idx, void* ws, size_t ws_bytes, void* stream);
diff --git a/ragraph_amd/_native.py b/ragraph_amd/_native.py
--- a/ragraph_amd/_native.py
+++ b/ragraph_amd/_native.py
@@ -34,6 +34,7 @@
     "ragraph_filter_profile_attach": (_vp, [_vp]),
     "ragraph_filter_profile_last_ms": (ctypes.c_float, [_vp]),
     "ragraph_topk_cosine_filtered_set_prior": (ctypes.c_float, [_f32]),
+    "ragraph_topk_cosine_filtered_set_tight_prior": (ctypes.c_float, [_f32]),
     "ragraph_filter_profile_levels": (_i32, [_vp, _vp, _vp, _vp]),
     "ragraph_topk_cosine_filtered_cap": (_i32, [_i32]),
     "ragraph_topk_cosine_filtered_workspace_bytes": (_sz, [_i64, _i64, _i32, _i32]),
diff --git a/ragraph_amd/csrc/filter_common.h b/ragraph_amd/csrc/filter_common.h
--- a/ragraph_amd/csrc/filter_common.h
+++ b/ragraph_amd/csrc/filter_common.h
@@ -124,6 +124,17 @@
 constexpr int FILTER_TICKET_SLOT = 16;
 __host__ __device__ constexpr int filter_count_stride(int64_t B) { return B < 2048 ? FILTER_COUNT_STRIDE : 1; }
 
+constexpr int FILTER_REPAIR_Q = 256;
+struct FilterGate {
+  const int* word;
+  int lo, hi;
+};
+__device__ __forceinline__ bool filter_gate_closed(const FilterGate& g) {
+  if (!g.word) return false;
+  const int n = *g.word;
+  return n < g.lo || n > g.hi;
+}
+
 struct DirectArgs {
   const uint16_t* Qb;
   const uint16_t* Kb;
@@ -136,6 +147,7 @@
   int* gmax_out;
   int bound_groups;
   int scored;
+  FilterGate gate;
   int i8;
 };
 template <int D>
diff --git a/ragraph_amd/csrc/filter_ring.h b/ragraph_amd/csrc/filter_ring.h
--- a/ragraph_amd/csrc/filter_ring.h
+++ b/ragraph_amd/csrc/filter_ring.h
@@ -69,6 +69,7 @@
   constexpr int QT = C::WAVES * QW;
   constexpr int NG = QW / 16;
   constexpr bool FOLD = RG_RING_FOLD && I8 && !PIPE && !BOUND && D == 64;
+  if (filter_gate_closed(p.gate)) return;
   extern __shared__ float4 fsmem4[];
   char* smem = reinterpret_cast<char*>(fsmem4);
   unsigned* full = reinterpret_cast<unsigned*>(smem + C::SLOTS * C::STAGE_BYTES);
diff --git a/ragraph_amd/csrc/filter_schedule.h b/ragraph_amd/csrc/filter_schedule.h
--- a/ragraph_amd/csrc/filter_schedule.h
+++ b/ragraph_amd/csrc/filter_schedule.h
@@ -23,6 +23,7 @@
   int i8_qw;
   int scored_shards;
   int spec_two_shards;
+  int tight_levels;
 };
 static int filter_env_int(const char* name, int dflt) {
   const char* e = getenv(name);
@@ -32,7 +33,8 @@
   static const int scored_shards = filter_env_int("RAGRAPH_FILTER_SCORED_SHARDS", 2);
   static const int spec_two_shards = filter_env_int("RAGRAPH_FILTER_SPEC_SHARDS_TWO_LEVELS", 2);
   return {filter_env_int("RAGRAPH_FILTER_I8", -1), filter_env_int("RAGRAPH_FILTER_SCORED", -1), filter_env_int("RAGRAPH_FILTER_PIPE", 1),
-          filter_env_int("RAGRAPH_FILTER_PARTNER_LEAD", 1), filter_env_int("RAGRAPH_FILTER_I8_QW", 0), scored_shards, spec_two_shards};
+          filter_env_int("RAGRAPH_FILTER_PARTNER_LEAD", 1), filter_env_int("RAGRAPH_FILTER_I8_QW", 0), scored_shards, spec_two_shards,
+          filter_env_int("RAGRAPH_FILTER_TIGHT_LEVELS", 1)};
 }
 
 static bool filter_scored_lists(int64_t B, int D, int k, const FilterEnv& env) {
@@ -84,6 +86,7 @@
   bool exact_level0;
   FilterEnv env;
   int cus;
+  float tight;
 };
 
 static FilterSchedule filter_schedule(const FilterShape& in) {
@@ -282,7 +285,16 @@
   FilterLevel level[FILTER_MAX_LEVELS];
   bool bf16_image;
   int first_phase;
-};
+  bool tight;
+  bool repair_scored;
+  int level_final;
+};
+
+static size_t filter_repair_bytes(int D, int k, size_t slot_bytes) {
+  const size_t q = FILTER_REPAIR_Q;
+  return q * FILTER_LIST_CAP * slot_bytes + 2 * q * D * sizeof(float) + q * D * sizeof(uint16_t) + q * FILTER_COUNT_STRIDE * sizeof(int) +
+         align_up(q * k * sizeof(float), 256) + align_up(q * k * sizeof(int64_t), 256) + 16 * 1024 ;
+}
 
 static void filter_drop_first_level(FilterSchedule& sc) {
   for (int l = 0; l + 1 < sc.nlev; ++l) sc.ends[l] = sc.ends[l + 1];
@@ -338,6 +350,14 @@
     c.spec = prior_ok && sc.bound_keys > 0 && N == plan_N;
     if (c.spec) drop_first_level_under_prior();
   }
+  {
+    const size_t slot = c.scored_slots ? sizeof(int2) : sizeof(int);
+    const size_t idle = align_up((size_t)B * c.cap * slot, 256) + align_up((size_t)B * filter_bound_parts(k, INT64_MAX, 256) * sizeof(int), 256);
+    c.tight = c.spec && !in.exchange && B > 256 && in.tight == in.tight && in.tight > in.prior && in.tight < 2.f &&
+              idle >= filter_repair_bytes(D, k, slot);
+  }
+  if (c.tight)
+    while (sc.nlev > (in.env.tight_levels == 2 ? 2 : 1)) filter_drop_first_level(sc);
   const bool bound = sc.bound_keys > 0 && !c.spec;
   c.level0 = c.spec ? FILTER_L0_NONE : (bound ? FILTER_L0_BOUND : (sc.slab0 ? FILTER_L0_SLAB : FILTER_L0_TILE));
   c.level0_bytes = sc.bound_keys > 0 ? 0
@@ -356,5 +376,7 @@
     lv.int8 = l >= c.nlev - c.i8_levels;
     lv.scored = lv.int8 && (!in.exchange || in.n_shards <= in.env.scored_shards) && c.scored_slots;
   }
+  c.level_final = c.tight ? -1 : c.nlev - 1;
+  c.repair_scored = c.tight && c.level[c.nlev - 1].scored;
   return c;
 }
diff --git a/ragraph_amd/csrc/filter_verify_fixup.h b/ragraph_amd/csrc/filter_verify_fixup.h
--- a/ragraph_amd/csrc/filter_verify_fixup.h
+++ b/ragraph_amd/csrc/filter_verify_fixup.h
@@ -35,6 +35,68 @@
     if (lo != INT_MAX) atomicMin(stats + 18, lo);
     if (hi != INT_MIN) atomicMax(stats + 19, hi);
     if (failed) atomicAdd(stats + 17, failed);
+  }
+}
+
+__global__ void __launch_bounds__(256) filter_tight_verdict_kernel(float* __restrict__ out_s, int64_t* __restrict__ out_i, int64_t B,
+                                                                   int k, float tight, float prior,
+                                                                   const unsigned char* __restrict__ flag, float* __restrict__ theta,
+                                                                   int* __restrict__ list, int* __restrict__ stats) {
+  const int64_t q = (int64_t)blockIdx.x * 256 + threadIdx.x;
+  const int lane = threadIdx.x & 63;
+  if (q == 0) stats[21] = 1;
+  bool soft = false;
+  float kth = RG_NEG_INF;
+  if (q < B) {
+    kth = out_s[q * k + k - 1];
+    soft = flag[q] == 0 && !(kth >= tight);
+    theta[q] = soft ? fmaxf(prior, kth) : __builtin_huge_valf();
+  }
+  const unsigned long long m = __ballot(soft);
+  if (m == 0ull) return;
+  int base = 0;
+  if (lane == 0) base = atomicAdd(stats + 22, __popcll(m));
+  base = __shfl(base, 0);
+  if (!soft) return;
+  const int pos = base + __popcll(m & ((1ull << lane) - 1ull));
+  if (pos < FILTER_REPAIR_Q) list[pos] = (int)q;
+  for (int j = 0; j < k; ++j) {
+    out_s[q * k + j] = RG_NEG_INF;
+    out_i[q * k + j] = INT64_MAX;
+  }
+}
+
+template <int D>
+__global__ void __launch_bounds__(64) filter_repair_gather_kernel(const float* __restrict__ Q, const float* __restrict__ theta,
+                                                                  const int* __restrict__ list, float* __restrict__ Q2,
+                                                                  float* __restrict__ theta2, int* __restrict__ stats) {
+  const int row = blockIdx.x, lane = threadIdx.x;
+  const int n = stats[22];
+  if (row == 0 && lane == 0) stats[23] = n == 0 ? 0 : (n <= FILTER_REPAIR_Q ? 1 : 2);
+  const bool live = n <= FILTER_REPAIR_Q && row < n;
+  const int64_t q = live ? list[row] : 0;
+  float4 v = make_float4(0.f, 0.f, 0.f, 0.f);
+  if (live && lane < D / 4) v = reinterpret_cast<const float4*>(Q + q * D)[lane];
+  if (lane < D / 4) reinterpret_cast<float4*>(Q2 + (int64_t)row * D)[lane] = v;
+  if (lane == 0) theta2[row] = live ? theta[q] : 0.f;
+}
+
+__global__ void __launch_bounds__(64) filter_repair_scatter_kernel(const int* __restrict__ list, const float* __restrict__ s2,
+                                                                   const int64_t* __restrict__ i2,
+                                                                   const unsigned char* __restrict__ flag2, int k,
+                                                                   float* __restrict__ out_s, int64_t* __restrict__ out_i,
+                                                                   unsigned char* __restrict__ flag, const int* __restrict__ stats) {
+  const int row = blockIdx.x, lane = threadIdx.x;
+  const int n = stats[22];
+  if (n < 1 || n > FILTER_REPAIR_Q || row >= n) return;
+  const int64_t q = list[row];
+  if (flag2[row] != 0) {
+    if (lane == 0) flag[q] = 1;
+    return;
+  }
+  if (lane < k) {
+    out_s[q * k + lane] = s2[(int64_t)row * k + lane];
+    out_i[q * k + lane] = i2[(int64_t)row * k + lane];
   }
 }
 
diff --git a/ragraph_amd/csrc/topk_filter.hip b/ragraph_amd/csrc/topk_filter.hip
--- a/ragraph_amd/csrc/topk_filter.hip
+++ b/ragraph_amd/csrc/topk_filter.hip
@@ -46,6 +46,7 @@
   int partner_lead;
   int* gmax;
   int ngroups;
+  FilterGate gate;
 };
 
 __device__ __forceinline__ void fring_wait(unsigned* ctr, unsigned target) {
@@ -153,6 +154,12 @@
 extern "C" int ragraph_topk_cosine_filtered_max_i8_levels(int n) {
   const int old = t_max_i8_levels;
   t_max_i8_levels = n < 0 ? -1 : n;
+  return old;
+}
+static thread_local float t_tight = __builtin_nanf("");
+extern "C" float ragraph_topk_cosine_filtered_set_tight_prior(float t) {
+  const float old = t_tight;
+  t_tight = t;
   return old;
 }
 int ragraph::filter_thread_i8_cap() { return t_max_i8_levels; }
@@ -296,7 +303,13 @@
   } while (0)
 
 static FilterShape filter_query_shape(int64_t B, int64_t N, int D, int k, int n_shards, bool exchange) {
-  return {B, N, N, D, k, n_shards, exchange, __builtin_nanf(""), -1, false, filter_env(), filter_device_cus()};
+  return {B, N, N, D, k, n_shards, exchange, __builtin_nanf(""), -1, false, filter_env(), filter_device_cus(), __builtin_nanf("")};
+}
+static void filter_query_follow_tight(FilterShape& in) {
+  if (t_prior == t_prior && t_tight == t_tight && t_tight > t_prior) {
+    in.prior = t_prior;
+    in.tight = t_tight;
+  }
 }
 
 static size_t filter_workspace_bytes(FilterShape in, const FilterSchedule& sc) {
@@ -327,13 +340,15 @@
   if (filter_shape_code(B, N, D, k) != RAGRAPH_OK) return 0;
   FilterShape in = filter_query_shape(B, N, D, k, 1, false);
   in.i8_cap = t_max_i8_levels;
+  filter_query_follow_tight(in);
   return filter_call_plan(in, filter_schedule(in)).i8_levels;
 }
 
 extern "C" int ragraph_topk_cosine_filtered_plan(int64_t B, int64_t N, int D, int k, int64_t plan[7]) {
   RG_REQUIRE(plan, RAGRAPH_EINVAL, "topk_cosine_filtered_plan: null pointer");
   RG_REQUIRE_FILTER_SHAPE("topk_cosine_filtered_plan", B, N, D, k);
-  const FilterShape in = filter_query_shape(B, N, D, k, 1, false);
+  FilterShape in = filter_query_shape(B, N, D, k, 1, false);
+  filter_query_follow_tight(in);
   const FilterCall c = filter_call_plan(in, filter_schedule(in));
   plan[0] = c.n0;
   plan[1] = c.level0 == FILTER_L0_BOUND ? 2 : (c.level0 == FILTER_L0_SLAB ? 1 : 0);
@@ -373,12 +388,12 @@
     set_error("topk_cosine_filtered: cannot raise dynamic LDS limit: %s", hipGetErrorString(e));
     return RAGRAPH_EDEVICE;
   }
-  if (t_prof) (void)hipEventRecord(t_prof->ev[2 * prof_slot], st);
+  if (t_prof && prof_slot >= 0) (void)hipEventRecord(t_prof->ev[2 * prof_slot], st);
   hipLaunchKernelGGL((topk_filter_kernel<D, QW, BOUND, I8, SCORED, PIPE>), dim3((unsigned)CUS), dim3(C::THREADS), C::LDS_BYTES, st, p);
-  if (t_prof) (void)hipEventRecord(t_prof->ev[2 * prof_slot + 1], st);
+  if (t_prof && prof_slot >= 0) (void)hipEventRecord(t_prof->ev[2 * prof_slot + 1], st);
   RG_CHECK_LAUNCH("topk_cosine_filtered(filter)");
   ring_stamps_report(BOUND, I8);
-  ring_timing_report(prof_slot, D);
+  if (prof_slot >= 0) ring_timing_report(prof_slot, D);
   return RAGRAPH_OK;
 }
 
@@ -441,7 +456,7 @@
 template <int D>
 static int run_pass(const FilterWs& f, const uint16_t* Kb, const signed char* Kb8, int64_t B, int64_t key0, int64_t key1,
                     const FilterThr& thr, int cap, int bound_groups, bool int8, bool scored, const FilterEnv& env, int cus,
-                    int prof_slot, hipStream_t st) {
+                    int prof_slot, hipStream_t st, FilterGate gate = FilterGate{nullptr, 0, 0}) {
   const PassVariant v = filter_pass_variant(D, B, key0, key1, bound_groups > 0, int8, scored, cus, env);
   const uint16_t* keys = v.i8 ? reinterpret_cast<const uint16_t*>(Kb8) : Kb;
   const uint16_t* Qimg = v.i8 ? reinterpret_cast<const uint16_t*>(f.Qb8) : f.Qb;
@@ -461,9 +476,10 @@
     a.nsub = rescore_slices(B, thr.k);
     a.gmax_out = f.gmax;
     a.bound_groups = bound_groups;
-    if (t_prof) (void)hipEventRecord(t_prof->ev[2 * prof_slot], st);
+    a.gate = gate;
+    if (t_prof && prof_slot >= 0) (void)hipEventRecord(t_prof->ev[2 * prof_slot], st);
     const int rc = launch_filter_direct<D>(a, st);
-    if (t_prof) (void)hipEventRecord(t_prof->ev[2 * prof_slot + 1], st);
+    if (t_prof && prof_slot >= 0) (void)hipEventRecord(t_prof->ev[2 * prof_slot + 1], st);
     return rc;
   }
   const int stage_keys = FILTER_STAGE_BYTES / ((v.i8 ? 1 : 2) * D);
@@ -485,6 +501,7 @@
   p.stage_base = key0 / stage_keys;
   p.nstages_total = cdiv(key1 - key0, stage_keys);
   p.partner_lead = env.partner_lead;
+  p.gate = gate;
   return launch_ring_variant<D>(v, p, B, cus, prof_slot, st);
 }
 
@@ -593,6 +610,93 @@
   return RAGRAPH_OK;
 }
 
+struct FilterRepairWs {
+  FilterWs f;
+  int* list;
+  float* Q;
+  float* theta;
+  float* out_s;
+  int64_t* out_i;
+  int* dummy;
+};
+static FilterRepairWs filter_repair_carve(const FilterWs& f, int D, int k, bool int8, size_t slot_bytes) {
+  char* w = reinterpret_cast<char*>(f.cand);
+  size_t off = 0;
+  auto take = [&](size_t bytes) {
+    char* ptr = w + off;
+    off += align_up(bytes, 256);
+    return ptr;
+  };
+  const size_t q = FILTER_REPAIR_Q;
+  FilterRepairWs r{};
+  r.f.cand = reinterpret_cast<int*>(take(q * FILTER_LIST_CAP * slot_bytes));
+  r.Q = reinterpret_cast<float*>(take(q * D * sizeof(float)));
+  r.f.Qn = reinterpret_cast<float*>(take(q * D * sizeof(float)));
+  if (int8) r.f.Qb8 = reinterpret_cast<signed char*>(take(q * D));
+  else r.f.Qb = reinterpret_cast<uint16_t*>(take(q * D * sizeof(uint16_t)));
+  r.f.count = reinterpret_cast<int*>(take(q * FILTER_COUNT_STRIDE * sizeof(int)));
+  r.out_s = reinterpret_cast<float*>(take(q * k * sizeof(float)));
+  r.out_i = reinterpret_cast<int64_t*>(take(q * k * sizeof(int64_t)));
+  r.list = reinterpret_cast<int*>(take(q * sizeof(int)));
+  r.theta = reinterpret_cast<float*>(take(q * sizeof(float)));
+  r.f.eq = reinterpret_cast<float*>(take(q * sizeof(float)));
+  r.f.eq8 = reinterpret_cast<float*>(take(q * sizeof(float)));
+  r.f.qscale = reinterpret_cast<float*>(take(q * sizeof(float)));
+  r.f.flag = reinterpret_cast<unsigned char*>(take(q));
+  r.dummy = reinterpret_cast<int*>(take(sizeof(int)));
+  r.f.theta = r.theta;
+  r.f.overflow_list = f.overflow_list;
+  r.f.fix_done = f.fix_done;
+  return r;
+}
+
+template <int D>
+static int run_tight_repair(const FilteredArgs& a, const FilterCall& c, const FilterShape& in, const FilterWs& f, FilterThr thr,
+                            const signed char* K8, int* stats, hipStream_t st) {
+  const int64_t B = a.B, N = a.N;
+  const int k = a.k;
+  const FilterLevel& lv = c.level[c.nlev - 1];
+  const size_t slot = c.scored_slots ? sizeof(int2) : sizeof(int);
+  RG_REQUIRE((size_t)(reinterpret_cast<char*>(f.theta) - reinterpret_cast<char*>(f.cand)) >= filter_repair_bytes(D, k, slot),
+             RAGRAPH_EWORKSPACE, "topk_cosine_filtered: the repair's buffers do not fit the idle lists");
+  const FilterRepairWs r = filter_repair_carve(f, D, k, lv.int8, slot);
+  hipLaunchKernelGGL(filter_tight_verdict_kernel, dim3((unsigned)cdiv(B, 256)), dim3(256), 0, st, a.out_scores, a.out_idx, B, k,
+                     in.tight, in.prior, f.flag, f.theta, r.list, stats);
+  RG_CHECK_LAUNCH("topk_cosine_filtered(soft verdict)");
+  hipLaunchKernelGGL(filter_repair_gather_kernel<D>, dim3(FILTER_REPAIR_Q), dim3(64), 0, st, a.Q, f.theta, r.list, r.Q, r.theta, stats);
+  RG_CHECK_LAUNCH("topk_cosine_filtered(repair gather)");
+  hipLaunchKernelGGL((filter_prep_kernel<D, 1>), dim3(FILTER_REPAIR_Q / 4), dim3(256), 0, st, r.Q, (int64_t)FILTER_REPAIR_Q, r.f.Qn,
+                     r.f.eq, r.f.count, r.f.flag, r.dummy, (int*)nullptr, k, r.f.Qb, filter_count_stride(FILTER_REPAIR_Q),
+                     lv.int8 ? r.f.eq8 : nullptr, r.f.qscale, r.f.Qb8, r.f.fix_done, (int*)nullptr, FilterStatsInit{},
+                     (float*)nullptr, 0.f);
+  RG_CHECK_LAUNCH("topk_cosine_filtered(repair prepare)");
+  FilterThr thr2 = thr;
+  thr2.theta = r.theta;
+  thr2.prev_scores = nullptr;
+  thr2.gmax = nullptr;
+  thr2.eq = r.f.eq;
+  thr2.eq8 = r.f.eq8;
+  thr2.qscale = r.f.qscale;
+  thr2.flag = r.f.flag;
+  int rc = run_pass<D>(r.f, a.Kb, K8, FILTER_REPAIR_Q, 0, N, thr2, FILTER_LIST_CAP, 0, lv.int8, c.repair_scored, in.env, in.cus, -1, st,
+                       FilterGate{stats + 22, 1, FILTER_REPAIR_Q});
+  if (rc != RAGRAPH_OK) return rc;
+  rc = run_rescore<D>(r.f, a.Kn, N, FILTER_REPAIR_Q, FILTER_LIST_CAP, k, 0, 0, 0, r.out_s, r.out_i, r.dummy,
+                      rescore_kind(FILTER_REPAIR_Q, k, c.repair_scored, false), thr2, nullptr, st);
+  if (rc != RAGRAPH_OK) return rc;
+  hipLaunchKernelGGL(filter_repair_scatter_kernel, dim3(FILTER_REPAIR_Q), dim3(64), 0, st, r.list, r.out_s, r.out_i, r.f.flag, k,
+                     a.out_scores, a.out_idx, f.flag, stats);
+  RG_CHECK_LAUNCH("topk_cosine_filtered(repair scatter)");
+  thr.theta = f.theta;
+  thr.gmax = nullptr;
+  thr.prev_scores = a.out_scores;
+  rc = run_pass<D>(f, a.Kb, K8, B, 0, N, thr, c.cap, 0, lv.int8, lv.scored, in.env, in.cus, -1, st,
+                   FilterGate{stats + 22, FILTER_REPAIR_Q + 1, INT_MAX});
+  if (rc != RAGRAPH_OK) return rc;
+  return run_rescore<D>(f, a.Kn, N, B, c.cap, k, a.idx_base, 1, 1, a.out_scores, a.out_idx, a.overflow,
+                        rescore_kind(B, k, lv.scored, false), thr, nullptr, st);
+}
+
 template <int D>
 static int run_filtered(const FilteredArgs& a, const FilterCall& c, const FilterShape& in) {
   hipStream_t st = as_stream(a.stream);
@@ -627,7 +731,7 @@
   hipLaunchKernelGGL((filter_prep_kernel<D, R_>), dim3((unsigned)cdiv(B <= FILTER_QB_MAX_B ? (B + 31) / 32 * 32 : B, 4 * (R_))), dim3(256), 0, st, a.Q, B, \
                      f.Qn, f.eq, f.count, f.flag, a.overflow, bound ? f.gmax : nullptr, c.parts, c.bf16_image ? f.Qb : nullptr,         \
                      filter_count_stride(B), c.i8_levels > 0 ? f.eq8 : nullptr, f.qscale, B <= FILTER_QB_MAX_B ? f.Qb8 : nullptr, f.fix_done, \
-                     stats, stats_init, c.spec ? (sharded ? a.theta : f.theta) : nullptr, in.prior)
+                     stats, stats_init, c.spec ? (sharded ? a.theta : f.theta) : nullptr, c.tight ? in.tight : in.prior)
   if (B >= 8192) RG_PREP(4);
   else RG_PREP(1);
 #undef RG_PREP
@@ -702,7 +806,7 @@
     }
     if (rc != RAGRAPH_OK) return rc;
     if (t_prof) t_prof->have = l + 1;
-    rc = run_rescore<D>(f, a.Kn, N, B, c.cap, k, a.idx_base, l > 0, l == c.nlev - 1, out_scores, out_idx, a.overflow,
+    rc = run_rescore<D>(f, a.Kn, N, B, c.cap, k, a.idx_base, l > 0, l == c.level_final, out_scores, out_idx, a.overflow,
                         rescore_kind(B, k, lv.scored, sharded && l > 0), thr, stats + 2 + l, st);
     if (rc != RAGRAPH_OK) return rc;
     if (l + 1 == c.nlev) break;
@@ -713,6 +817,8 @@
       if ((rc = launch_theta(thr, B, 0, f.theta, st)) != RAGRAPH_OK) return rc;
     }
   }
+
+  if (c.tight && (rc = run_tight_repair<D>(a, c, in, f, thr, v8.K8, stats, st)) != RAGRAPH_OK) return rc;
 
   if (c.spec && !sharded) {
     hipLaunchKernelGGL(filter_verify_prior_kernel, dim3((unsigned)cdiv(B, 256)), dim3(256), 0, st, out_scores, B, k, in.prior, 1, f.flag,
@@ -741,7 +847,7 @@
   const FilterSchedule sc_one = filter_schedule(one);
   const size_t need = filter_workspace_bytes(one, sc_one);
   RG_REQUIRE(a.ws_bytes >= need, RAGRAPH_EWORKSPACE, "topk_cosine_filtered: workspace %zu < %zu", a.ws_bytes, need);
-  const FilterShape in{B, N, plan_N, D, k, a.n_shards, a.exchange != nullptr, t_prior, t_max_i8_levels, false, one.env, one.cus};
+  const FilterShape in{B, N, plan_N, D, k, a.n_shards, a.exchange != nullptr, t_prior, t_max_i8_levels, false, one.env, one.cus, t_tight};
   const FilterCall c = filter_call_plan(in, a.exchange && a.n_shards > 1 ? filter_schedule(in) : sc_one);
   if (c.exact_participant) return run_exact_participant(a, c);
   if (D == 256) return run_filtered<256>(a, c, in);
diff --git a/ragraph_amd/csrc/topk_filter_direct.hip b/ragraph_amd/csrc/topk_filter_direct.hip
--- a/ragraph_amd/csrc/topk_filter_direct.hip
+++ b/ragraph_amd/csrc/topk_filter_direct.hip
@@ -37,6 +37,7 @@
   int* gmax;
   int ngroups;
   int qgroups;
+  FilterGate gate;
 };
 
 #ifdef RG_DIRECT_TIMING
@@ -56,6 +57,7 @@
   static_assert(!(I8 && BOUND), "the bound pass runs on the bf16 copy");
   using acc_t = typename std::conditional<I8, i32x4, f32x4>::type;
   RG_DSTAMP(0);
+  if (filter_gate_closed(p.gate)) return;
   extern __shared__ float4 dsmem4[];
   char* smem = reinterpret_cast<char*>(dsmem4);
   const int ngl = QREG ? 0 : p.qgroups;
@@ -418,6 +420,7 @@
   RG_REQUIRE((p.nsub & (p.nsub - 1)) == 0 && p.nsub <= FILTER_COUNT_STRIDE, RAGRAPH_EINVAL, "filter(direct): nsub=%d", p.nsub);
   p.subcap = a.cap / p.nsub;
   p.scored = a.scored;
+  p.gate = a.gate;
   p.qgroups = 2 * (int)cdiv(a.B, 32);
   const int cus = device_cus_multiple_of_8();
   int64_t grid = cdiv(p.nunits, (int64_t)C::WAVES);
@@ -448,6 +451,7 @@
   RG_REQUIRE((p.nsub & (p.nsub - 1)) == 0 && p.nsub <= FILTER_COUNT_STRIDE, RAGRAPH_EINVAL, "filter(direct): nsub=%d", p.nsub);
   p.subcap = a.cap / p.nsub;
   p.gmax = a.gmax_out;
+  p.gate = a.gate;
   p.ngroups = a.bound_groups;
   p.qgroups = 2 * (int)cdiv(a.B, 32);
   const bool bound = a.bound_groups > 0;
diff --git a/ragraph_amd/kernels.py b/ragraph_amd/kernels.py
--- a/ragraph_amd/kernels.py
+++ b/ragraph_amd/kernels.py
@@ -213,6 +213,10 @@
 
 def set_filter_prior(theta_prior) -> float:
     return N.lib().ragraph_topk_cosine_filtered_set_prior(float("nan") if theta_prior is None else float(theta_prior))
+
+
+def set_filter_tight_prior(theta_tight) -> float:
+    return N.lib().ragraph_topk_cosine_filtered_set_tight_prior(float("nan") if theta_tight is None else float(theta_tight))
 
 
 def ord2f(v: int) -> float:
diff --git a/ragraph_amd/kernels_index.py b/ragraph_amd/kernels_index.py
--- a/ragraph_amd/kernels_index.py
+++ b/ragraph_amd/kernels_index.py
@@ -23,6 +23,10 @@
     SPEC_MIN_MARGIN = 0.01
     SPEC_MAX_CANDIDATES = 1.5
     SPEC_HISTORY = 16
+    TIGHT_MIN_BATCH = 2048
+    TIGHT_MARGIN = 0.002
+    TIGHT_MARGIN_MAX = 0.064
+    TIGHT_MAX_SOFT = 32
     DEDUP_MIN_ROWS = 2048
     DEDUP_MAX_UNIQUE = 0.9
     DEDUP_MAX_GROUP = 64
@@ -54,6 +58,8 @@
         self.last_i8_candidates = None
         self._spec = {}
         self.spec_enabled = os.environ.get("RAGRAPH_SPEC", "1") != "0"
+        self.tight_enabled = os.environ.get("RAGRAPH_SPEC_TIGHT", "1") != "0"
+        self.last_tight = None
         self._notes = 0
         self.last_stats = None
         self.last_prior = None
@@ -148,6 +154,7 @@
             return lists_over
         st["used"] += 1
         st["failed"] += failed
+        self._judge_tight(st, words)
         loose = cand is not None and st["cand"] is not None and cand > self.SPEC_MAX_CANDIDATES * max(st["cand"], 32.0)
         if failed or loose or lists_over:
             probed_at = st.get("probed_at")
@@ -158,6 +165,31 @@
                 st["hist"] = []
                 st["queries"] = 0
         return 0
+
+    def _judge_tight(self, st: dict, words):
+        if len(words) < 24 or not words[21]:
+            return
+        st["soft"] = st.get("soft", 0) + words[22]
+        st["tight_used"] = st.get("tight_used", 0) + 1
+        if words[23] == 2:
+            st["tight_off_at"] = self._queries
+        if words[23] == 2 or words[22] > self.TIGHT_MAX_SOFT:
+            st["tight_margin"] = min(2.0 * st.get("tight_margin", self.TIGHT_MARGIN), self.TIGHT_MARGIN_MAX)
+
+    def _tight_for(self, B: int, k: int, prior):
+        if prior is None or not self.tight_enabled or B < self.TIGHT_MIN_BATCH or \
+                getattr(self.ops, "set_filter_tight_prior", None) is None:
+            return None
+        st = self._spec_state(k)
+        off_at = st.get("tight_off_at")
+        if off_at is not None:
+            if self._queries - off_at < self.REPROBE_QUERIES:
+                return None
+            st["tight_off_at"] = None
+        if not st["hist"]:
+            return None
+        t = min(h[0] for h in st["hist"]) - st.get("tight_margin", self.TIGHT_MARGIN)
+        return t if t > prior else None
 
     def _demote(self, what: str):
         if what == "i8":
@@ -346,8 +378,11 @@
             had_i8 = had_i8 and ops.filtered_i8_levels(B, kn.shape[0], D, k) > 0
             stats = None
             prior = self._prior_for(B, k)
+            tight = self._tight_for(B, k, prior)
             if prior is not None:
                 ops.set_filter_prior(prior)
+            if tight is not None:
+                ops.set_filter_tight_prior(tight)
             try:
                 if getattr(ops, "FILTER_STATS", False):
                     s, i, over, stats = ops.topk_cosine_filtered(q, kn, self._bf16, k, idx_base=idx_base,
@@ -359,7 +394,10 @@
                     cap(-1)
                 if prior is not None:
                     ops.set_filter_prior(None)
+                if tight is not None:
+                    ops.set_filter_tight_prior(None)
             self.last_prior = prior
+            self.last_tight = tight
             self._note_overflow(over, B, had_i8, stats, k)
             self.last_stats = stats
             return s, i
```

Measured after the change: 5.372 million, median of 6. 7.4% higher.
